# ethz-asl/ethzasl_brisk

Hardware: AMD Instinct MI355X
Metric: frames/sec detect+describe @1080p (1/2/4/8 GPU); % HBM roofline (higher is better)
Workload: dtype u8

## Files before the change

ethzasl_brisk_amd/csrc/brisk_capi.hip:

```cpp
#include <hip/hip_runtime.h>
#include <math.h>
#include <stdio.h>
#include <stdlib.h>
#include <string.h>

#include <sched.h>
#include <unistd.h>

#include <atomic>
#include <chrono>
#include <mutex>
#include <thread>
#include <string>
#include <vector>

#include "../../include/brisk_hip.h"
#include "../../include/brisk_hip_debug.h"
#include "brisk_common.h"
#include "brisk_kernels.h"
#include "brisk_pattern.h"
#include "brisk_device_describe.h"
#include "brisk_hostmem.h"
#include "brisk_slab_layout.h"
#include "brisk_transfer.h"
// ... 264 lines not shown
  HIPCHK(c, w.pyr.grow((size_t)slots * pyr + 256));
  HIPCHK(c, w.smap.grow(((size_t)slots * pyr + 256) * sizeof(uint16_t)));
  HIPCHK(c, w.cand.grow((size_t)slots * c->cand_cap * sizeof(BriskCand)));
  HIPCHK(c, w.blocks.grow((size_t)slots * c->cand_cap * 64));
  HIPCHK(c, w.tie_idx.grow((size_t)slots * BRISK_MAX_LAYERS * c->tie_cap * sizeof(int)));
  HIPCHK(c, w.keys.grow((size_t)slots * c->cand_cap * 2 * sizeof(unsigned)));
  HIPCHK(c, w.counters.grow((size_t)slots * sizeof(BriskFrameCounters)));
  HIPCHK(c, w.kp_out.grow((size_t)slots * c->kp_cap * sizeof(BriskKeyPoint)));
  HIPCHK(c, w.integral.grow((size_t)slots * ifr * sizeof(uint32_t)));
  HIPCHK(c, w.bandsum.grow((size_t)slots * ((ifr / 64) + 4 * 8192 + 64) * sizeof(uint32_t)));
  HIPCHK(c, w.dkp.grow((size_t)slots * c->kp_cap * sizeof(BriskKeyPoint)));
  HIPCHK(c, w.dscale.grow((size_t)slots * c->kp_cap * sizeof(int)));
  HIPCHK(c, w.dperm.grow((size_t)slots * c->kp_cap * sizeof(int)));
  HIPCHK(c, w.drec.grow(((size_t)slots * c->kp_cap + 4) * sizeof(uint4)));
  c->D.dp_work_stride = brisk_dp_work_ints(c->kp_cap);
  HIPCHK(c, w.dp_work.grow((size_t)slots * c->D.dp_work_stride * sizeof(int)));
  c->D.desc_pitch = c->desc_pitch;
  HIPCHK(c, w.desc.grow((size_t)slots * c->kp_cap * c->D.desc_pitch));
  HIPCHK(c, c->d_kp_in.grow((size_t)slots * c->kp_cap * sizeof(BriskKeyPoint)));
  HIPCHK(c, c->d_n_in.grow((size_t)slots * sizeof(int)));
  c->B.pyr = w.pyr.as<uint8_t>(); c->B.smap = w.smap.as<uint16_t>(); c->B.cand = w.cand.as<BriskCand>(); c->B.blocks = w.blocks.as<uint8_t>();
  c->B.tie_idx = w.tie_idx.as<int>(); c->B.keys = w.keys.as<unsigned>(); c->B.counters = w.counters.as<BriskFrameCounters>();
  c->B.kp_out = w.kp_out.as<BriskKeyPoint>(); c->B.bandsum = w.bandsum.as<uint32_t>();
  c->D.integral = w.integral.as<uint32_t>(); c->D.dkp = w.dkp.as<BriskKeyPoint>(); c->D.dscale = w.dscale.as<int>(); c->D.dperm = w.dperm.as<int>();
  c->D.drec = w.drec.as<uint4>(); c->D.dp_work = w.dp_work.as<int>(); c->D.desc = w.desc.as<uint8_t>();
  HIPCHK(c, hipMemset(c->B.pyr, 0, (size_t)slots * pyr + 256));
  HIPCHK(c, hipMemset(c->B.smap, 0, ((size_t)slots * pyr + 256) * sizeof(uint16_t)));
  HIPCHK(c, hipDeviceSynchronize());
  c->dirty_frames = 0;
  c->slots = slots; c->pyr_elems_alloc = pyr; c->iframe_elems_alloc = ifr;
  c->D.istride = istride;
  c->B.istride = istride;
  c->D.iframe_elems = iframe;
  c->D.ibits = 32;
  return BRISK_HIP_OK;
}

static int ensure_stage(brisk_hip_ctx* c, size_t bytes) {
  if (bytes <= c->d_stage.cap) return BRISK_HIP_OK;
  HIPCHK(c, hipStreamSynchronize(c->stream));
  c->img_cache.valid = false;
  HIPCHK(c, c->d_stage.grow(bytes, 256));
  return BRISK_HIP_OK;
}

static void integral_format(const brisk_hip_ctx* ctx, const brisk_hip_pattern* pat, bool batch_with_detect, int* ibits) {
  static const int env = tuning_env("BRISK_INTEGRAL_BITS") ? atoi(tuning_env("BRISK_INTEGRAL_BITS")) : 0;
  *ibits = 32;
  if (!pat || !pat->dev.int24_ok) return;
  if (env == 32 || (dbg_flags(ctx) & (1 << 18))) return;
  if (env == 24 || (dbg_flags(ctx) & (1 << 24))) { *ibits = 24; return; }
  if (ctx->integral_fmt == BRISK_HIP_INTEGRAL_U32) return;
  if (ctx->integral_fmt == BRISK_HIP_INTEGRAL_U24) { *ibits = 24; return; }
  if (!batch_with_detect) return;
  double density = 0.0;
  if (ctx->h_density.p && ctx->density_mpx > 0.0) {
    const long long wv = __atomic_load_n(ctx->h_density.as<long long>(), __ATOMIC_RELAXED);
    const long long frames = wv >> 40, cands = wv & 0xFFFFFFFFFFll;
    if (frames > 0) density = (double)cands / ((double)frames * ctx->density_mpx);
  }
  if (density <= 3000.0) *ibits = 24;
}
static int check_pattern_device(brisk_hip_ctx* ctx, const brisk_hip_pattern* pat) {
  if (pat && pat->device != ctx->device) {
    char msg[160];
    snprintf(msg, sizeof msg, "pattern handle was created on device %d, the context runs on device %d: create one extractor per GPU",
             pat->device, ctx->device);
    return fail(ctx, BRISK_HIP_ERR_ARG, msg);
  }
  return BRISK_HIP_OK;
}

static hipError_t upload_rows(uint8_t* dst, int pitch, const uint8_t* src, int stride, int w, int h, hipStream_t s) {
  if (pitch == w && stride == w) return hipMemcpyAsync(dst, src, (size_t)w * h, hipMemcpyHostToDevice, s);
  return hipMemcpy2DAsync(dst, pitch, src, stride, w, h, hipMemcpyHostToDevice, s);
}

static int check_detect_args(brisk_hip_ctx* ctx, int w, int h, int threshold, int octaves) {
  if (w <= 0 || h <= 0 || w > 8191 || h > 8191) return fail(ctx, BRISK_HIP_ERR_ARG, "image size must be in [1, 8191]");
  if (octaves < 0 || 2 * octaves > BRISK_MAX_LAYERS) return fail(ctx, BRISK_HIP_ERR_ARG, "octaves must be in [0, 8]");
  if (threshold < 1 || threshold > 255)
    return fail(ctx, BRISK_HIP_ERR_THRESHOLD, "AGAST threshold must be in [1, 255]");
  return BRISK_HIP_OK;
}

static int usable_cpus();

extern "C" {

int brisk_hip_device_count(void) {
  int n = 0;
  if (hipGetDeviceCount(&n) != hipSuccess) return 0;
  return n;
}

int brisk_hip_usable_cpus(void) { return usable_cpus(); }

int brisk_hip_host_register(void* ptr, size_t bytes) {
  if (!ptr || !bytes) return BRISK_HIP_ERR_ARG;
  int n = 0;
  if (hipGetDeviceCount(&n) != hipSuccess || n <= 0) return BRISK_HIP_ERR_NO_DEVICE;
  const hipError_t e = hipHostRegister(ptr, bytes, hipHostRegisterDefault);
  if (e == hipSuccess) return BRISK_HIP_OK;
  (void)hipGetLastError();
  return e == hipErrorHostMemoryAlreadyRegistered ? BRISK_HIP_ERR_ARG : BRISK_HIP_ERR_HIP;
}

int brisk_hip_host_unregister(void* ptr) {
  if (!ptr) return BRISK_HIP_ERR_ARG;
  if (hipHostUnregister(ptr) == hipSuccess) return BRISK_HIP_OK;
  (void)hipGetLastError();
  return BRISK_HIP_ERR_ARG;
}

int brisk_hip_create(int device, brisk_hip_ctx** out) {
  if (!out) return BRISK_HIP_ERR_ARG;
  *out = nullptr;
  int n = 0;
  if (hipGetDeviceCount(&n) != hipSuccess || n <= 0 || device < 0 || device >= n) return BRISK_HIP_ERR_NO_DEVICE;
  if (hipSetDevice(device) != hipSuccess) return BRISK_HIP_ERR_NO_DEVICE;
  brisk_hip_ctx* c = new brisk_hip_ctx();
  c->device = device;
  c->B.band_h = 96;
  if (hipStreamCreateWithFlags(&c->stream, hipStreamNonBlocking) != hipSuccess) {
    delete c;
    return BRISK_HIP_ERR_HIP;
  }
  *out = c;
  return BRISK_HIP_OK;
}

void brisk_hip_destroy(brisk_hip_ctx* c) {
  if (!c) return;
  hipSetDevice(c->device);
  hipDeviceSynchronize();
  if (c->done_ev) hipEventDestroy(c->done_ev);
  if (c->block_ev) hipEventDestroy(c->block_ev);
  for (int i = 0; i < 2; ++i) {
    if (c->copied_ev[i]) hipEventDestroy(c->copied_ev[i]);
    if (c->consumed_ev[i]) hipEventDestroy(c->consumed_ev[i]);
    if (c->pin_ev[i]) hipEventDestroy(c->pin_ev[i]);
  }
  if (c->kin_pin_ev) hipEventDestroy(c->kin_pin_ev);
  if (c->copy_stream) hipStreamDestroy(c->copy_stream);
  c->ex.destroy_events();
  c->mx.destroy_events();
  c->tx.destroy_events();
  if (c->egress) hipStreamDestroy(c->egress);
  brisk_prof_destroy(&c->prof);
  if (c->side) { hipStreamDestroy(c->side); hipEventDestroy(c->side_fork); hipEventDestroy(c->side_join); }
  if (c->sub_created) {
    for (int i = 0; i < 8; ++i) { hipStreamDestroy(c->sub[i]); hipEventDestroy(c->join_ev[i]); }
    hipEventDestroy(c->fork_ev);
  }
  hipStreamDestroy(c->stream);
  delete c;
}

const char* brisk_hip_last_error(const brisk_hip_ctx* ctx) { return ctx ? ctx->err.c_str() : "null context"; }

int brisk_hip_set_capacity(brisk_hip_ctx* ctx, int max_candidates, int max_keypoints) {
  if (!ctx) return BRISK_HIP_ERR_ARG;
  if (max_candidates < 256 || max_keypoints < 16) return fail(ctx, BRISK_HIP_ERR_ARG, "capacity too small");
  if (max_keypoints >= (1 << 23)) return fail(ctx, BRISK_HIP_ERR_ARG, "keypoint capacity must be below 2^23");
  std::lock_guard<std::mutex> lk(ctx->mu);
  ctx->cand_cap = max_candidates;
  ctx->kp_cap = max_keypoints;
  ctx->tie_cap = max_candidates / 4 > 1024 ? max_candidates / 4 : 1024;
  return BRISK_HIP_OK;
}

int brisk_hip_reserve(brisk_hip_ctx* ctx, int min_candidates, int min_keypoints) {
  if (!ctx) return BRISK_HIP_ERR_ARG;
  std::lock_guard<std::mutex> lk(ctx->mu);
  if (min_keypoints >= (1 << 23)) return fail(ctx, BRISK_HIP_ERR_ARG, "keypoint capacity must be below 2^23");
  if (min_candidates > ctx->cand_cap) {
    ctx->cand_cap = min_candidates;
    if (min_candidates / 4 > ctx->tie_cap) ctx->tie_cap = min_candidates / 4;
  }
  if (min_keypoints > ctx->kp_cap) ctx->kp_cap = min_keypoints;
  return BRISK_HIP_OK;
}

static int upload_pattern(brisk_hip_ctx* ctx, brisk_hip_pattern* p) {
  const BriskPatternHost& H = p->host;
  const size_t n = (size_t)H.npoints;
  size_t off = 0;
  auto take = [&](size_t bytes) { size_t o = off; off += (bytes + 255) / 256 * 256; return o; };
  const size_t o_mult = take(64 * n * 4), o_sigma = take(64 * n * 4), o_uv = take((size_t)BRISK_NROT * n * 16);
  const size_t o_scl = take(64 * n * 8), o_tab = take(64 * n * 16);
  const size_t o_thr = take(64 * 4), o_size = take(64 * 4), o_sp = take((size_t)H.nshort * 4), o_lp = take((size_t)H.nlong * 16);
  HIPCHK(ctx, hipSetDevice(ctx->device));
  HIPCHK(ctx, hipMalloc(&p->blob, off));
  char* b = (char*)p->blob;
  HIPCHK(ctx, hipMemcpy(b + o_mult, H.mult.data(), 64 * n * 4, hipMemcpyHostToDevice));
  HIPCHK(ctx, hipMemcpy(b + o_sigma, H.sigma.data(), 64 * n * 4, hipMemcpyHostToDevice));
  HIPCHK(ctx, hipMemcpy(b + o_scl, H.scaling.data(), 64 * n * 8, hipMemcpyHostToDevice));
  {
    std::vector<int> tab(64 * n * 4);
    for (size_t i = 0; i < 64 * n; ++i) {
      memcpy(&tab[4 * i], &H.mult[i], 4);
      memcpy(&tab[4 * i + 1], &H.sigma[i], 4);
      brisk_pack_tab(H.scaling[2 * i], H.scaling[2 * i + 1], &tab[4 * i + 2], &tab[4 * i + 3]);
    }
    HIPCHK(ctx, hipMemcpy(b + o_tab, tab.data(), 64 * n * 16, hipMemcpyHostToDevice));
  }
  HIPCHK(ctx, hipMemcpy(b + o_uv, H.uv.data(), (size_t)BRISK_NROT * n * 16, hipMemcpyHostToDevice));
  HIPCHK(ctx, hipMemcpy(b + o_thr, H.size_thresh.data(), 64 * 4, hipMemcpyHostToDevice));
  HIPCHK(ctx, hipMemcpy(b + o_size, H.size_list.data(), 64 * 4, hipMemcpyHostToDevice));
  HIPCHK(ctx, hipMemcpy(b + o_sp, H.short_pairs.data(), (size_t)H.nshort * 4, hipMemcpyHostToDevice));
  HIPCHK(ctx, hipMemcpy(b + o_lp, H.long_pairs.data(), (size_t)H.nlong * 16, hipMemcpyHostToDevice));
  BriskPatternDev& d = p->dev;
  d.npoints = H.npoints; d.nshort = H.nshort; d.nlong = H.nlong; d.strings = H.strings;
  d.rotation_invariant = 1; d.scale_invariant = 1; d.basicscale = H.basicscale;
  d.has_bilinear = 0;
  d.reg_tables = (H.nlong <= 896 && H.nshort <= 512 && H.npoints <= 128) ? 1 : 0;
  for (int i = 0; i < H.nlong; ++i)
    if (H.long_pairs[4 * i + 2] < -32768 || H.long_pairs[4 * i + 2] > 32767 || H.long_pairs[4 * i + 3] < -32768 || H.long_pairs[4 * i + 3] > 32767) d.reg_tables = 0;
  float sigma_max = 0.f;
  for (float sg : H.sigma) { d.has_bilinear |= (sg < 0.5f) ? 1 : 0; sigma_max = sg > sigma_max ? sg : sigma_max; }
  d.int24_ok = (!d.has_bilinear && sigma_max < 120.0f) ? 1 : 0;
  d.mult = (const float*)(b + o_mult); d.sigma = (const float*)(b + o_sigma); d.uv = (const double*)(b + o_uv);
  d.scaling = (const int*)(b + o_scl);
  d.tab = (const int*)(b + o_tab);
  d.size_thresh = (const float*)(b + o_thr); d.size_list = (const int*)(b + o_size);
  d.short_pairs = (const uint16_t*)(b + o_sp); d.long_pairs = (const int*)(b + o_lp);
  return BRISK_HIP_OK;
}

static int pattern_finish(brisk_hip_ctx* ctx, brisk_hip_pattern* p, bool ok, const std::string& err,
                          brisk_hip_pattern** out) {
  if (!ok) {
    ctx->err = err;
    delete p;
    return BRISK_HIP_ERR_PATTERN;
  }
  p->device = p->true_device = ctx->device;
  p->blob = nullptr;
  const int rc = upload_pattern(ctx, p);
  if (rc != BRISK_HIP_OK) {
    if (p->blob) hipFree(p->blob);
    delete p;
    return rc;
  }
  *out = p;
  return BRISK_HIP_OK;
}

int brisk_hip_pattern_create(brisk_hip_ctx* ctx, int version, float pattern_scale, brisk_hip_pattern** out) {
  if (!ctx || !out) return BRISK_HIP_ERR_ARG;
  *out = nullptr;
  std::lock_guard<std::mutex> lk(ctx->mu);
  brisk_hip_pattern* p = new brisk_hip_pattern();
  std::string err;
  const bool ok = brisk_pattern_build_default(version, pattern_scale, &p->host, &err);
  return pattern_finish(ctx, p, ok, err, out);
}

int brisk_hip_pattern_create_from_text(brisk_hip_ctx* ctx, const char* ptn_text, float pattern_scale,
                                       brisk_hip_pattern** out) {
  if (!ctx || !out || !ptn_text) return BRISK_HIP_ERR_ARG;
  *out = nullptr;
  std::lock_guard<std::mutex> lk(ctx->mu);
  brisk_hip_pattern* p = new brisk_hip_pattern();
  std::string err;
  const bool ok = brisk_pattern_build_from_text(ptn_text, pattern_scale, &p->host, &err);
  return pattern_finish(ctx, p, ok, err, out);
}

void brisk_hip_pattern_destroy(brisk_hip_pattern* p) {
  if (!p) return;
  hipSetDevice(p->true_device);
  if (p->blob) hipFree(p->blob);
  delete p;
}

int brisk_hip_pattern_descriptor_size(const brisk_hip_pattern* p) { return p ? p->host.strings : 0; }
int brisk_hip_pattern_points(const brisk_hip_pattern* p) { return p ? p->host.npoints : 0; }

int brisk_hip_pattern_tables(const brisk_hip_pattern* p, float* scale_list, int* size_list, float* size_thresh) {
  if (!p) return BRISK_HIP_ERR_ARG;
  if (scale_list) memcpy(scale_list, p->host.scale_list.data(), 64 * 4);
  if (size_list) memcpy(size_list, p->host.size_list.data(), 64 * 4);
  if (size_thresh) memcpy(size_thresh, p->host.size_thresh.data(), 64 * 4);
  return BRISK_HIP_OK;
}

struct BatchArgs {
  const brisk_hip_pattern* pat;
  int w, h, threshold, octaves;
  long frame_pitch;
  int row_pitch;
  const uint8_t* d_mask;
  long mask_frame_pitch;
  int mask_row_pitch;
  bool do_detect, do_describe;
  double uni_radius;
  int uni_max;
  int bk_u = 0, bk_v = 0, bk_max = 0;
  bool no_scale_nms = false;
  int lower_threshold = BRISK_LOWER_THRESHOLD;
  bool format_as_full_batch = false;
  bool inplace_ok = true;
};

static int ensure_filter_buffers(brisk_hip_ctx* ctx, int w, int h, int nframes, double uni_radius) {
  size_t need = 0;
  if (uni_radius > 0.0) {
    const float scaling = (float)(15.0 / (float)uni_radius);
    const int oh = (int)(h * ceil(scaling) + 32), ow = (int)(w * ceil(scaling) + 32);
    need = (size_t)(((long)oh * ow + 255) / 256 * 256) * nframes + 64;
  }
  const size_t items = (size_t)ctx->slots * ctx->kp_cap;
  if (need > ctx->d_occ.cap || items * sizeof(BriskKeyPoint) > ctx->d_uni_tmp.cap || items * sizeof(int) > ctx->d_uni_order.cap) {
    HIPCHK(ctx, hipDeviceSynchronize());
    HIPCHK(ctx, ctx->d_occ.grow(need));
    HIPCHK(ctx, ctx->d_uni_tmp.grow(items * sizeof(BriskKeyPoint)));
    HIPCHK(ctx, ctx->d_uni_order.grow(items * sizeof(int)));
  }
  return BRISK_HIP_OK;
}

static int batch_begin(brisk_hip_ctx* ctx, const BatchArgs& A, int nframes, hipStream_t s) {
  int rc = check_detect_args(ctx, A.w, A.h, A.threshold, A.octaves);
  if (rc) return rc;
  HIPCHK(ctx, hipSetDevice(ctx->device));
  make_geometry(A.w, A.h, A.threshold, A.octaves, &ctx->G, &ctx->T);
  ctx->G.debug_flags = dbg_flags(ctx);
  ctx->G.no_scale_nms = (A.no_scale_nms && A.octaves != 0) ? 1 : 0;
  ctx->G.lower_threshold = A.lower_threshold;
  if (A.do_describe && A.pat && A.pat->host.strings > ctx->desc_pitch) ctx->desc_pitch = brisk_align_up(A.pat->host.strings, 16);
  rc = ensure_buffers(ctx, nframes, ctx->G);
  if (rc) return rc;
  integral_format(ctx, A.pat, A.format_as_full_batch || (A.do_detect && A.do_describe), &ctx->D.ibits);
  const bool bucketing = A.do_detect && !(A.uni_radius > 0.0) && A.bk_u > 0;
  if ((A.do_detect && A.uni_radius > 0.0) || bucketing) {
    rc = ensure_filter_buffers(ctx, A.w, A.h, nframes, bucketing ? 0.0 : A.uni_radius);
    if (rc) return rc;
  }
  if (bucketing && (A.bk_u >= A.w || A.bk_v >= A.h))
    return fail(ctx, BRISK_HIP_ERR_ARG, "bucketing: more buckets than pixels (key-point-bucketing-inl.h:82-83)");
  rc = workspace_acquire(ctx, s);
  if (rc) return fail(ctx, rc, "hipStreamWaitEvent failed");
  ctx->img_cache.valid = false;
  brisk_prof_begin_call(&ctx->prof);
  if (A.do_detect) {
    if (ctx->dirty_frames > 0) brisk_launch_smap_clear(ctx->dirtyG, ctx->B, ctx->dirty_frames, s);
    ctx->dirtyG = ctx->G;
    ctx->dirty_frames = nframes;
  }
  return BRISK_HIP_OK;
}

static int batch_slice(brisk_hip_ctx* ctx, const BatchArgs& A, const uint8_t* d_frames, long f0, int nf, hipStream_t si,
                       BriskProfiler* prof, bool overlap_integral) {
  const int nbands = (A.h + ctx->B.band_h - 1) / ctx->B.band_h;
  BriskDetectBuffers Bi = ctx->B;
  Bi.pyr += f0 * ctx->G.pyr_elems;
  Bi.smap += f0 * ctx->G.pyr_elems;
  Bi.cand += f0 * Bi.cand_cap;
  Bi.blocks += f0 * Bi.cand_cap * 64;
  Bi.tie_idx += f0 * BRISK_MAX_LAYERS * Bi.tie_cap;
  Bi.keys += f0 * Bi.cand_cap * 2;
  Bi.counters += f0;
  Bi.kp_out += f0 * Bi.kp_cap;
  Bi.bandsum += f0 * nbands * Bi.istride;
  BriskDescribeBuffers Di = ctx->D;
  Di.ibits = ctx->D.ibits;
  Di.integral += f0 * Di.iframe_elems;
  Di.dkp += f0 * Bi.kp_cap;
  Di.dscale += f0 * Bi.kp_cap;
  Di.dperm += f0 * Bi.kp_cap;
  Di.drec += f0 * Bi.kp_cap;
  Di.dp_work += f0 * Di.dp_work_stride;
  Di.desc += f0 * Bi.kp_cap * Di.desc_pitch;
  BriskOverlap ov{};
  const BriskOverlap* ovp = nullptr;
  if (A.do_detect && A.do_describe && overlap_integral && ctx->overlap && !(dbg_flags(ctx) & 0x10000)) {
    if (!ctx->side) {
      int least = 0, greatest = 0;
      HIPCHK(ctx, hipDeviceGetStreamPriorityRange(&least, &greatest));
      const char* pe = tuning_env("BRISK_SIDE_PRIO");
      HIPCHK(ctx, hipStreamCreateWithPriority(&ctx->side, hipStreamNonBlocking, (pe && atoi(pe) == 0) ? 0 : least));
      HIPCHK(ctx, hipEventCreateWithFlags(&ctx->side_fork, hipEventDisableTiming));
      HIPCHK(ctx, hipEventCreateWithFlags(&ctx->side_join, hipEventDisableTiming));
    }
    ov.side = ctx->side; ov.fork = ctx->side_fork; ov.join = ctx->side_join; ov.Dd = &Di;
    ovp = &ov;
  }
  BriskGeom Gs = ctx->G;
  {
    static const bool inplace_on = !(tuning_env("BRISK_L0_INPLACE") && atoi(tuning_env("BRISK_L0_INPLACE")) == 0);
    const bool ordered = Gs.threshold < BRISK_FAST_PATH_MIN_THRESHOLD || Gs.no_scale_nms || Gs.lower_threshold != BRISK_LOWER_THRESHOLD;
    if (A.do_detect && A.inplace_ok && inplace_on && !ordered && A.row_pitch == Gs.L[0].stride && A.w == Gs.L[0].stride &&
        ((((uintptr_t)d_frames) | (uintptr_t)A.frame_pitch) & 15) == 0) {
      Gs.l0_ext = d_frames;
      Gs.l0_pitch = A.frame_pitch;
      if (f0 == 0) { ctx->last_l0_ext = d_frames; ctx->last_l0_pitch = A.frame_pitch; }
    } else if (f0 == 0) {
      ctx->last_l0_ext = nullptr;
    }
  }
  if (A.do_detect) {
    brisk_launch_detect(Gs, ctx->T, Bi, nf, d_frames, A.frame_pitch, A.row_pitch,
                        A.d_mask ? A.d_mask + f0 * A.mask_frame_pitch : nullptr, A.mask_frame_pitch, A.mask_row_pitch, si, prof, ovp);
  }
  int* const uni_order = ctx->d_uni_order.as<int>();
  BriskKeyPoint* const uni_tmp = ctx->d_uni_tmp.as<BriskKeyPoint>();
  if (A.do_detect && A.uni_radius > 0.0) {
    const float scaling = (float)(15.0 / (float)A.uni_radius);
    const int oh = (int)(A.h * ceil(scaling) + 32), ow = (int)(A.w * ceil(scaling) + 32);
    const long occ_frame = ((long)oh * ow + 255) / 256 * 256;
    brisk_launch_uniformity(Bi.kp_out, Bi.counters, uni_order + f0 * Bi.kp_cap, uni_tmp + f0 * Bi.kp_cap,
                            ctx->d_occ.as<uint8_t>() + f0 * occ_frame, occ_frame, ow, Bi.kp_cap, scaling, A.uni_max, nf, si);
  }
  if (A.do_detect && !(A.uni_radius > 0.0) && A.bk_u > 0) {
    brisk_launch_bucketing(Bi.kp_out, Bi.counters, uni_order + f0 * Bi.kp_cap, uni_tmp + f0 * Bi.kp_cap, Bi.kp_cap,
                           A.h, A.w, A.bk_u, A.bk_v, A.bk_max, nf, si);
  }
  if (A.do_detect) brisk_prof_mark(prof, BRISK_STG_INTEGRAL, si);
  if (A.do_describe) {
    BriskPatternDev P = A.pat->dev;
    brisk_launch_describe(Gs, P, Bi, Di, nf, Bi.kp_out, &Bi.counters[0].nkp, sizeof(BriskFrameCounters), si, prof, ovp);
  }
  return BRISK_HIP_OK;
}

static int batch_end(brisk_hip_ctx* ctx, const BatchArgs& A, int nframes, hipStream_t s) {
  if (A.do_detect && A.do_describe) {
    if (!ctx->h_density.p) {
      HIPCHK(ctx, ctx->h_density.grow(sizeof(long long), 0, hipHostMallocMapped));
      *ctx->h_density.as<long long>() = 0;
    }
    ctx->density_mpx = (double)A.w * (double)A.h / 1e6;
    brisk_launch_batch_density(ctx->B.counters, nframes, ctx->B.cand_cap, ctx->h_density.as<long long>(), s);
  }
  if (ctx->prof.on) ctx->prof.calls++;
  HIPCHK(ctx, hipGetLastError());
  ctx->last_nframes = nframes;
  ctx->last_has_desc = A.do_describe;
  ctx->last_desc_pitch = ctx->D.desc_pitch;
  if (A.do_describe && A.pat) ctx->last_strings = A.pat->host.strings;
  const int rc = workspace_release(ctx, s);
  if (rc) return fail(ctx, rc, "hipEventRecord failed");
  return BRISK_HIP_OK;
}

static int run_batch(brisk_hip_ctx* ctx, const brisk_hip_pattern* pat, const uint8_t* d_frames, int nframes, int w, int h,
                     long frame_pitch, int row_pitch, int threshold, int octaves, const uint8_t* d_mask,
                     long mask_frame_pitch, int mask_row_pitch, hipStream_t s, bool do_detect, bool do_describe,
                     double uni_radius = -1.0, int uni_max = 0, bool no_scale_nms = false,
                     int lower_threshold = BRISK_LOWER_THRESHOLD, const int* bucketing = nullptr) {
  if (!d_frames || nframes <= 0 || row_pitch < w || frame_pitch < (long)row_pitch * (h - 1) + w)
    return fail(ctx, BRISK_HIP_ERR_ARG, "bad frame buffer description");
  if (int rcp = check_pattern_device(ctx, pat)) return rcp;
  const bool full_batch = do_detect && do_describe;
  if (do_detect && do_describe && (dbg_flags(ctx) & (1 << 27)) && ctx->last_nframes >= nframes) do_detect = false;
  BatchArgs A{pat, w, h, threshold, octaves, frame_pitch, row_pitch, d_mask, mask_frame_pitch, mask_row_pitch, do_detect,
              do_describe, uni_radius < 0.0 ? ctx->uni_radius : uni_radius, uni_radius < 0.0 ? ctx->uni_max : uni_max};
  A.no_scale_nms = no_scale_nms;
  A.lower_threshold = lower_threshold;
  A.format_as_full_batch = full_batch;
  if (bucketing) { A.bk_u = bucketing[0]; A.bk_v = bucketing[1]; A.bk_max = bucketing[2]; }
  else if (uni_radius < 0.0) { A.bk_u = ctx->bk_u; A.bk_v = ctx->bk_v; A.bk_max = ctx->bk_max; }
  int rc = batch_begin(ctx, A, nframes, s);
  if (rc) return rc;
  WorkspaceGuard guard(ctx, s);
  int nsub = ctx->nsub;
  if (nsub > 8) nsub = 8;
  if (nframes < 16 * nsub) nsub = nframes >= 32 ? 2 : 1;
  if (nsub > 1 && !ctx->sub_created) {
    for (int i = 0; i < 8; ++i) {
      HIPCHK(ctx, hipStreamCreateWithFlags(&ctx->sub[i], hipStreamNonBlocking));
      HIPCHK(ctx, hipEventCreateWithFlags(&ctx->join_ev[i], hipEventDisableTiming));
    }
    HIPCHK(ctx, hipEventCreateWithFlags(&ctx->fork_ev, hipEventDisableTiming));
    ctx->sub_created = true;
  }
  const int grp = 8 * ((dbg_flags(ctx) >> 20) & 0xF);
  if (grp > 0 && !do_detect && do_describe) {
    if (dbg_flags(ctx) & (1 << 19))
      brisk_launch_integral(ctx->G, ctx->B.pyr, ctx->B.bandsum, ctx->D.integral, ctx->D.istride, ctx->D.iframe_elems, ctx->B.band_h, nframes, s);
    for (long f0 = 0; f0 < nframes; f0 += grp) {
      const int nf = (int)((nframes - f0) < grp ? (nframes - f0) : grp);
      if (f0 == 0) ctx->last_frames_per_launch = nf;
      rc = batch_slice(ctx, A, d_frames + f0 * frame_pitch, f0, nf, s, (f0 == 0) ? &ctx->prof : nullptr, false);
      if (rc) return rc;
    }
    guard.armed = false;
    return batch_end(ctx, A, nframes, s);
  }
  if (nsub > 1) HIPCHK(ctx, hipEventRecord(ctx->fork_ev, s));
  for (int i = 0; i < nsub; ++i) {
    const long f0 = (long)nframes * i / nsub, f1 = (long)nframes * (i + 1) / nsub;
    const int nf = (int)(f1 - f0);
    if (nf <= 0) continue;
    hipStream_t si = s;
    if (nsub > 1) {
      si = ctx->sub[i];
      HIPCHK(ctx, hipStreamWaitEvent(si, ctx->fork_ev, 0));
    }
    if (i == 0) ctx->last_frames_per_launch = nf;
    rc = batch_slice(ctx, A, d_frames + f0 * frame_pitch, f0, nf, si, (i == 0) ? &ctx->prof : nullptr, nsub == 1);
    if (rc) return rc;
    if (nsub > 1) {
      HIPCHK(ctx, hipEventRecord(ctx->join_ev[i], si));
      HIPCHK(ctx, hipStreamWaitEvent(s, ctx->join_ev[i], 0));
    }
  }
  guard.armed = false;
  return batch_end(ctx, A, nframes, s);
}

static int host_slice_frames() {
  static const int v = [] { const char* e = tuning_env("BRISK_HOST_SLICE"); const int n = e ? atoi(e) : 0; return n > 0 ? n : 64; }();
  return v;
}

#define BRISK_STAGED_SLICE 32
static int copy_threads() {
  static const int n = [] {
    const char* e = tuning_env("BRISK_COPY_THREADS");
    int t = e ? atoi(e) : usable_cpus() / 2;
    return t < 1 ? 1 : (t > 8 ? 8 : t);
  }();
  return n;
}
static int upload_frames(brisk_hip_ctx* ctx, uint8_t* d_dst, size_t dframe, int dpitch, const uint8_t* const* ptrs, int nf, int w, int h, int stride,
                         bool staged, int b, hipStream_t cs) {
  if (!staged) {
    for (int f = 0; f < nf; ++f)
      HIPCHK(ctx, hipMemcpy2DAsync(d_dst + (size_t)f * dframe, dpitch, ptrs[f], stride, w, h, hipMemcpyHostToDevice, cs));
    return BRISK_HIP_OK;
  }
  if (ctx->h_pin[0].cap < dframe * BRISK_STAGED_SLICE || ctx->h_pin[1].cap < dframe * BRISK_STAGED_SLICE) {
    for (int i = 0; i < 2; ++i) {
      if (ctx->pin_used[i]) HIPCHK(ctx, hipEventSynchronize(ctx->pin_ev[i]));
      ctx->pin_used[i] = false;
      ctx->h_pin[i].reset();
    }
    for (int i = 0; i < 2; ++i) {
      HIPCHK(ctx, ctx->h_pin[i].grow(dframe * BRISK_STAGED_SLICE, 256));
      if (!ctx->pin_ev[i]) HIPCHK(ctx, hipEventCreateWithFlags(&ctx->pin_ev[i], hipEventDisableTiming));
    }
  }
  if (ctx->pin_used[b]) HIPCHK(ctx, hipEventSynchronize(ctx->pin_ev[b]));
  uint8_t* const pin = ctx->h_pin[b].as<uint8_t>();
  std::atomic<int> next{0};
  const int items = nf * 4;
  auto work = [&]() {
    for (;;) {
      const int i = next.fetch_add(1, std::memory_order_relaxed);
      if (i >= items) break;
      const int f = i >> 2, part = i & 3;
      const int y0 = (int)((long)h * part / 4), y1 = (int)((long)h * (part + 1) / 4);
      if (y1 <= y0) continue;
      uint8_t* d = pin + (size_t)f * dframe;
      const uint8_t* sp = ptrs[f];
      if (stride == dpitch) memcpy(d + (size_t)y0 * dpitch, sp + (size_t)y0 * stride, (size_t)(y1 - y0 - 1) * dpitch + (size_t)w);
      else for (int y = y0; y < y1; ++y) memcpy(d + (size_t)y * dpitch, sp + (size_t)y * stride, (size_t)w);
    }
  };
  const int T = copy_threads() < items ? copy_threads() : items;
  std::vector<std::thread> helpers;
  for (int t = 1; t < T; ++t) helpers.emplace_back(work);
  work();
  for (std::thread& t : helpers) t.join();
  HIPCHK(ctx, hipMemcpyAsync(d_dst, pin, dframe * (size_t)nf, hipMemcpyHostToDevice, cs));
  HIPCHK(ctx, hipEventRecord(ctx->pin_ev[b], cs));
  ctx->pin_used[b] = true;
  return BRISK_HIP_OK;
}
static bool is_pageable(const void* p) {
  void* dev = nullptr;
  return !device_can_write(p, &dev);
}

static int batch_host_locked(brisk_hip_ctx* ctx, const brisk_hip_pattern* pat, const uint8_t* h_frames, int nframes, int w, int h,
                             long frame_pitch, int row_pitch, int threshold, int octaves, const uint8_t* const* frame_ptrs = nullptr,
                             uint8_t* d_resident = nullptr ) {
  if ((!h_frames && !frame_ptrs) || nframes <= 0 || row_pitch < w || (!frame_ptrs && frame_pitch < (long)row_pitch * (h - 1) + w))
    return fail(ctx, BRISK_HIP_ERR_ARG, "bad frame buffer description");
  if (frame_ptrs)
    for (int f = 0; f < nframes; ++f)
      if (!frame_ptrs[f]) return fail(ctx, BRISK_HIP_ERR_ARG, "null image in the list");
  if (int rcp = check_pattern_device(ctx, pat)) return rcp;
  BatchArgs A{pat, w, h, threshold, octaves, 0, 0, nullptr, 0, 0, true, pat != nullptr, ctx->uni_radius, ctx->uni_max};
  A.bk_u = ctx->bk_u; A.bk_v = ctx->bk_v; A.bk_max = ctx->bk_max;
  A.inplace_ok = d_resident != nullptr;
  hipStream_t s = ctx->stream;
  int rc = batch_begin(ctx, A, nframes, s);
  if (rc) return rc;
  WorkspaceGuard guard(ctx, s);
  const bool staged = frame_ptrs && is_pageable(frame_ptrs[0]);
  const int slice_max = staged ? BRISK_STAGED_SLICE : host_slice_frames();
  const int slice = slice_max < nframes ? slice_max : nframes;
  const int dpitch = brisk_align_up(w, 64);
  const size_t dframe = (size_t)dpitch * h;
  bool fresh = false;
  if (!ctx->copy_stream) {
    HIPCHK(ctx, hipStreamCreateWithFlags(&ctx->copy_stream, hipStreamNonBlocking));
    for (int i = 0; i < 2; ++i) {
      HIPCHK(ctx, hipEventCreateWithFlags(&ctx->copied_ev[i], hipEventDisableTiming));
      HIPCHK(ctx, hipEventCreateWithFlags(&ctx->consumed_ev[i], hipEventDisableTiming));
    }
    fresh = true;
  }
  if (!d_resident && (ctx->d_hstage[0].cap < dframe * slice || ctx->d_hstage[1].cap < dframe * slice)) {
    HIPCHK(ctx, hipDeviceSynchronize());
    for (int i = 0; i < 2; ++i) ctx->d_hstage[i].reset();
    for (int i = 0; i < 2; ++i) HIPCHK(ctx, ctx->d_hstage[i].grow(dframe * slice, 256));
    fresh = true;
  }
  A.frame_pitch = (long)dframe;
  A.row_pitch = dpitch;
  if (fresh) {
    HIPCHK(ctx, hipEventRecord(ctx->consumed_ev[0], s));
    HIPCHK(ctx, hipEventRecord(ctx->consumed_ev[1], s));
  }
  int k = 0;
  for (long f0 = 0; f0 < nframes; f0 += slice, ++k) {
    const int nf = (int)((nframes - f0 < slice) ? nframes - f0 : slice);
    const int b = k & 1;
    uint8_t* const dslice = d_resident ? d_resident + (size_t)f0 * dframe : ctx->d_hstage[b].as<uint8_t>();
    if (!d_resident) HIPCHK(ctx, hipStreamWaitEvent(ctx->copy_stream, ctx->consumed_ev[b], 0));
    else if (k == 0 && ctx->done_valid && !ensure_done_event(ctx)) HIPCHK(ctx, hipStreamWaitEvent(ctx->copy_stream, ctx->done_ev, 0));
    const uint8_t* src = frame_ptrs ? nullptr : h_frames + f0 * frame_pitch;
    if (frame_ptrs) {
      rc = upload_frames(ctx, dslice, dframe, dpitch, frame_ptrs + f0, nf, w, h, row_pitch, staged, b, ctx->copy_stream);
      if (rc) return rc;
    } else if (frame_pitch == (long)row_pitch * h) {
      HIPCHK(ctx, hipMemcpy2DAsync(dslice, dpitch, src, row_pitch, w, (size_t)h * nf, hipMemcpyHostToDevice,
                                   ctx->copy_stream));
    } else {
      for (int f = 0; f < nf; ++f)
        HIPCHK(ctx, hipMemcpy2DAsync(dslice + (size_t)f * dframe, dpitch, src + (long)f * frame_pitch, row_pitch, w,
                                     h, hipMemcpyHostToDevice, ctx->copy_stream));
    }
    HIPCHK(ctx, hipEventRecord(ctx->copied_ev[b], ctx->copy_stream));
    HIPCHK(ctx, hipStreamWaitEvent(s, ctx->copied_ev[b], 0));
    if (k == 0) ctx->last_frames_per_launch = nf;
    rc = batch_slice(ctx, A, dslice, f0, nf, s, (k == 0) ? &ctx->prof : nullptr, true);
    if (rc) return rc;
    if (!d_resident) HIPCHK(ctx, hipEventRecord(ctx->consumed_ev[b], s));
  }
  guard.armed = false;
  return batch_end(ctx, A, nframes, s);
}

int brisk_hip_detect_describe_batch_host(brisk_hip_ctx* ctx, const brisk_hip_pattern* pat, const uint8_t* h_frames,
                                         int nframes, int w, int h, long frame_pitch, int row_pitch, int threshold,
                                         int octaves) {
  if (!ctx || !pat) return BRISK_HIP_ERR_ARG;
  std::lock_guard<std::mutex> lk(ctx->mu);
  return batch_host_locked(ctx, pat, h_frames, nframes, w, h, frame_pitch, row_pitch, threshold, octaves);
}

int brisk_hip_detect_describe_batch(brisk_hip_ctx* ctx, const brisk_hip_pattern* pat, const uint8_t* d_frames, int nframes,
                                    int w, int h, long frame_pitch, int row_pitch, int threshold, int octaves,
                                    void* stream) {
  if (!ctx || !pat) return BRISK_HIP_ERR_ARG;
  std::lock_guard<std::mutex> lk(ctx->mu);
  hipStream_t s = stream ? (hipStream_t)stream : ctx->stream;
  return run_batch(ctx, pat, d_frames, nframes, w, h, frame_pitch, row_pitch, threshold, octaves, nullptr, 0, 0, s, true,
                   true);
}

int brisk_hip_detect_batch(brisk_hip_ctx* ctx, const uint8_t* d_frames, int nframes, int w, int h, long frame_pitch,
                           int row_pitch, int threshold, int octaves, void* stream) {
  if (!ctx) return BRISK_HIP_ERR_ARG;
  std::lock_guard<std::mutex> lk(ctx->mu);
  hipStream_t s = stream ? (hipStream_t)stream : ctx->stream;
  return run_batch(ctx, nullptr, d_frames, nframes, w, h, frame_pitch, row_pitch, threshold, octaves, nullptr, 0, 0, s, true,
                   false);
}

int brisk_hip_batch_results(brisk_hip_ctx* ctx, const int** d_detected, const int** d_described, int* count_stride,
                            const brisk_hip_keypoint** d_detected_kps, const brisk_hip_keypoint** d_described_kps,
                            const uint8_t** d_desc, int* kp_cap, int* desc_pitch) {
  if (!ctx) return BRISK_HIP_ERR_ARG;
  std::lock_guard<std::mutex> lk(ctx->mu);
  if (!ctx->B.counters) return fail(ctx, BRISK_HIP_ERR_ARG, "no batch has run");
  if (d_detected) *d_detected = &ctx->B.counters[0].nkp;
  if (d_described) *d_described = &ctx->B.counters[0].ndesc;
  if (count_stride) *count_stride = (int)sizeof(BriskFrameCounters);
  if (d_detected_kps) *d_detected_kps = (const brisk_hip_keypoint*)ctx->B.kp_out;
  if (d_described_kps) *d_described_kps = (const brisk_hip_keypoint*)ctx->D.dkp;
  if (d_desc) *d_desc = ctx->D.desc;
  if (kp_cap) *kp_cap = ctx->B.kp_cap;
  if (desc_pitch) *desc_pitch = ctx->last_desc_pitch ? ctx->last_desc_pitch : ctx->D.desc_pitch;
  return BRISK_HIP_OK;
}

static int overflow_to_rc(brisk_hip_ctx* ctx, int flags) {
  if (flags & 1) return fail(ctx, BRISK_HIP_ERR_CAPACITY, "candidate capacity exceeded (brisk_hip_set_capacity)");
  if (flags & 2) return fail(ctx, BRISK_HIP_ERR_CAPACITY, "tie-candidate capacity exceeded (brisk_hip_set_capacity)");
  if (flags & 4) return fail(ctx, BRISK_HIP_ERR_CAPACITY, "keypoint capacity exceeded (brisk_hip_set_capacity)");
  if (flags & 8) {
    static const char* const site[8] = {"", " (the layer below)", " (a pending tie outside its chunk)", " (a neighbour's decision)",
                                        " (the writer wave)", " (the sorted tie list of the layer below)", "", ""};
    char msg[128];
    snprintf(msg, sizeof(msg), "tie resolution gave up waiting for a decision%s (internal error)", site[(flags >> 8) & 7]);
    return fail(ctx, BRISK_HIP_ERR_HIP, msg);
  }
  if (flags & 16)
    return fail(ctx, BRISK_HIP_ERR_UNSUPPORTED,
                "no defined result in the reference on this input: suppressScaleNonmaxima=false indexes layer 0's point list "
                "past its end or reads outside a score matrix (brisk-scale-space.cc:137), or ComputeScale addresses the maps of "
                "a point in a layer's last rows beyond the image (brisk-layer.cc:110-115)");
  return BRISK_HIP_OK;
}

int brisk_hip_batch_status(brisk_hip_ctx* ctx, int nframes, int* overflow_flags) {
  if (!ctx) return BRISK_HIP_ERR_ARG;
  std::lock_guard<std::mutex> lk(ctx->mu);
  if (nframes <= 0 || nframes > ctx->slots) return fail(ctx, BRISK_HIP_ERR_ARG, "bad frame count");
  HIPCHK(ctx, hipSetDevice(ctx->device));
  HIPCHK(ctx, wait_own_work(ctx));
  std::vector<BriskFrameCounters> c(nframes);
  HIPCHK(ctx, hipMemcpy(c.data(), ctx->B.counters, sizeof(BriskFrameCounters) * nframes, hipMemcpyDeviceToHost));
  int f = 0;
  for (auto& x : c) f |= x.overflow;
  if (overflow_flags) *overflow_flags = f;
  return overflow_to_rc(ctx, f);
}

static int download_locked(brisk_hip_ctx* ctx, int frame, int which, brisk_hip_keypoint* kps, int cap, int* n,
                           uint8_t* desc, int desc_stride, int strings, int dev_pitch = 0) {
  if (!dev_pitch) dev_pitch = ctx->D.desc_pitch;
  if (frame < 0 || frame >= ctx->slots) return fail(ctx, BRISK_HIP_ERR_ARG, "bad frame index");
  HIPCHK(ctx, wait_own_work(ctx));
  BriskFrameCounters c;
  HIPCHK(ctx, hipMemcpy(&c, ctx->B.counters + frame, sizeof(c), hipMemcpyDeviceToHost));
  int rc = overflow_to_rc(ctx, c.overflow);
  if (rc) return rc;
  const int cnt = which ? c.ndesc : c.nkp;
  if (n) *n = cnt;
  if (kps) {
    if (cnt > cap) return fail(ctx, BRISK_HIP_ERR_CAPACITY, "output keypoint buffer too small");
    const BriskKeyPoint* src = (which ? ctx->D.dkp : ctx->B.kp_out) + (size_t)frame * ctx->B.kp_cap;
    if (cnt) HIPCHK(ctx, hipMemcpy(kps, src, sizeof(BriskKeyPoint) * (size_t)cnt, hipMemcpyDeviceToHost));
  }
  if (desc && which && cnt) {
    if (cnt > cap) return fail(ctx, BRISK_HIP_ERR_CAPACITY, "output descriptor buffer too small");
    const uint8_t* src = ctx->D.desc + (size_t)frame * ctx->B.kp_cap * ctx->D.desc_pitch;
    if (dev_pitch == desc_stride && strings == desc_stride)
      HIPCHK(ctx, hipMemcpy(desc, src, (size_t)cnt * strings, hipMemcpyDeviceToHost));
    else
      HIPCHK(ctx, hipMemcpy2D(desc, desc_stride, src, dev_pitch, strings, cnt, hipMemcpyDeviceToHost));
  }
  return BRISK_HIP_OK;
}

static int usable_cpus() {
  static const int n = [] {
    int c = 0;
    cpu_set_t set;
    if (sched_getaffinity(0, sizeof set, &set) == 0) c = CPU_COUNT(&set);
    if (c <= 0) c = (int)sysconf(_SC_NPROCESSORS_ONLN);
    long quota = -1, period = -1;
    if (FILE* f = fopen("/sys/fs/cgroup/cpu.max", "r")) {
      char q[64];
      if (fscanf(f, "%63s %ld", q, &period) == 2 && strcmp(q, "max") != 0) quota = atol(q);
      fclose(f);
    } else {
      if (FILE* g = fopen("/sys/fs/cgroup/cpu/cpu.cfs_quota_us", "r")) { if (fscanf(g, "%ld", &quota) != 1) quota = -1; fclose(g); }
      if (FILE* g = fopen("/sys/fs/cgroup/cpu/cpu.cfs_period_us", "r")) { if (fscanf(g, "%ld", &period) != 1) period = -1; fclose(g); }
    }
    if (quota > 0 && period > 0) {
      const int lim = (int)((quota + period - 1) / period);
      if (lim > 0 && lim < c) c = lim;
    }
    return c > 0 ? c : 1;
// ... 1858 lines not shown
```

ethzasl_brisk_amd/csrc/brisk_describe.hip:

```cpp
#include <hip/hip_runtime.h>
#include <stdlib.h>

#include "brisk_common.h"
#include "brisk_device_describe.h"
#include "brisk_kernels.h"

#define DP_MAXSORT 2048
#ifndef DP_THREADS
#define DP_THREADS 1024
#endif
#define DP_SMALL_N 2048
#define DP_SB DP_THREADS
#define DP_MAXBUCKETS 4096
#define DP_W_HIST 16
#define DP_W_BLK (DP_W_HIST + DP_MAXBUCKETS + 16)
__device__ __forceinline__ unsigned dp_order_key(int x, int y, int sc, int j, int mode) {
  const unsigned low = (unsigned)(j & 0x7FF);
  if (mode == 1) {
    unsigned tx = (unsigned)x >> 6, ty = (unsigned)y >> 6, d = 0;
    for (unsigned s = 64; s > 0; s >>= 1) {
      const unsigned rx = (tx & s) ? 1u : 0u, ry = (ty & s) ? 1u : 0u;
      d += s * s * ((3u * rx) ^ ry);
      if (ry == 0) {
        if (rx == 1) { tx = 127u - tx; ty = 127u - ty; }
        const unsigned t = tx; tx = ty; ty = t;
      }
    }
    return (d << 18) | (((unsigned)x & 63u) << 12) | low;
  }
  if (mode == 2) return ((unsigned)(y >> 7) << 24) | (((unsigned)x & 0x1FFFu) << 11) | low;
  if (mode == 3) return ((unsigned)(y >> 5) << 24) | (((unsigned)x & 0x1FFFu) << 11) | low;
  if (mode == 4) return ((unsigned)(sc >> 4) << 30) | (((unsigned)(y >> 6) & 0x7Fu) << 23) | ((((unsigned)x >> 1) & 0xFFFu) << 11) | low;
  return ((unsigned)(y >> 6) << 24) | (((unsigned)x & 0x1FFFu) << 11) | low;
}

__global__ void __launch_bounds__(DP_THREADS) k_desc_prepare(BriskGeom G, BriskPatternDev P, const BriskKeyPoint* kp_in,
                                                       const int* n_in_ptr, long n_in_stride, BriskFrameCounters* counters,
                                                       BriskKeyPoint* dkp, int* dscale, int* dperm, uint4* drec, int kp_cap,
                                                       int* work, long work_stride) {
  __shared__ int wtot[DP_THREADS / 64];
  __shared__ int base, nest;
  __shared__ __attribute__((aligned(16))) unsigned pkey[DP_MAXSORT + 4];
  BRISK_CHAIN_SETPRIO();
  const int frame = blockIdx.x, tid = threadIdx.x, wave = tid >> 6, lane = tid & 63;
  const int n = min(*(const int*)((const char*)n_in_ptr + (long)frame * n_in_stride), kp_cap);
  const BriskKeyPoint* K = kp_in + (long)frame * kp_cap;
  if (n > DP_SMALL_N) {
    int* wk = work + (long)frame * work_stride;
    for (int q = tid; q < DP_W_BLK; q += DP_THREADS) wk[q] = 0;
    return;
  }
  __shared__ uint4 srec[DP_SMALL_N];
  __shared__ int sborder[BRISK_SCALES];
  __shared__ float sthr[BRISK_SCALES];
  if (tid == 0) { base = 0; nest = 0; }
  if (tid < BRISK_SCALES) { sborder[tid] = P.size_list[tid]; sthr[tid] = P.size_thresh[tid]; }
  __syncthreads();
  for (int i0 = 0; i0 < n; i0 += DP_THREADS) {
    const int i = i0 + tid;
    bool keep = false;
    int sc = 0;
    BriskKeyPoint kp;
    if (i < n) {
      kp = K[i];
      if (!P.scale_invariant) sc = P.basicscale;
      else {
#pragma unroll 8
        for (int q = 1; q < BRISK_SCALES; ++q) sc += (kp.size >= sthr[q]) ? 1 : 0;
      }
      const int border = sborder[sc];
      keep = !((kp.x < (float)border) || (kp.x >= (float)(G.L[0].w - border)) || (kp.y < (float)border) || (kp.y >= (float)(G.L[0].h - border)));
    }
    const unsigned long long bal = __ballot(keep);
    const int before = __popcll(bal & ((1ull << lane) - 1ull));
    if (lane == 0) wtot[wave] = __popcll(bal);
    const unsigned long long bal_e = __ballot(keep && kp.angle == -1.0f);
    if (lane == 0 && bal_e) atomicAdd(&nest, __popcll(bal_e));
    __syncthreads();
    int wbase = 0, total = 0;
#pragma unroll
    for (int k = 0; k < DP_THREADS / 64; ++k) {
      const int t = wtot[k];
      wbase += (k < wave) ? t : 0;
      total += t;
    }
    if (keep) {
      const int j = base + wbase + before;
      dkp[(long)frame * kp_cap + j] = kp;
      if (j < DP_MAXSORT) pkey[j] = dp_order_key((int)kp.x, (int)kp.y, sc, j, (BRISK_DBG_FLAGS(G) >> 4) & 0xF);
      srec[j] = make_uint4(__float_as_uint(kp.x), __float_as_uint(kp.y), __float_as_uint(kp.angle), (unsigned)sc | ((unsigned)j << 8));
    }
    __syncthreads();
    if (tid == 0) base += total;
    __syncthreads();
  }
  if (tid == 0) { counters[frame].ndesc = base; counters[frame].nestimate = nest; counters[frame].desc_ticket = 0; counters[frame].orient_ticket = 0; }
  const int m = base;
  if (tid < 4) pkey[m + tid] = 0xFFFFFFFFu;
  __syncthreads();
  if (((BRISK_DBG_FLAGS(G) >> 4) & 0xF) != 0) {
    for (int j = tid; j < m; j += DP_THREADS) {
      const unsigned kj = pkey[j];
      int r = 0;
      for (int q = 0; q < m; q += 4) {
        const uint4 kk = *reinterpret_cast<const uint4*>(&pkey[q]);
        r += (kk.x < kj ? 1 : 0) + (kk.y < kj ? 1 : 0) + (kk.z < kj ? 1 : 0) + (kk.w < kj ? 1 : 0);
      }
      drec[(long)frame * kp_cap + r] = srec[j];
    }
    return;
  }
  {
    __shared__ int bhead[DP_SB], bstart[DP_SB];
    __shared__ int bnext[DP_SMALL_N];
    const int nbands = ((G.L[0].h - 1) >> 6) + 1;
    int xs = 6;
    while (nbands * (((G.L[0].w - 1) >> xs) + 1) > DP_SB) ++xs;
    const int nbx = ((G.L[0].w - 1) >> xs) + 1;
    auto bucket_of = [&](unsigned key) { return (int)(key >> 24) * nbx + (int)(((key >> 11) & 0x1FFFu) >> xs); };
    for (int b = tid; b < DP_SB; b += DP_THREADS) { bhead[b] = -1; bstart[b] = 0; }
    __syncthreads();
    for (int j = tid; j < m; j += DP_THREADS) {
      const int b = bucket_of(pkey[j]);
      atomicAdd(&bstart[b], 1);
      bnext[j] = atomicExch(&bhead[b], j);
    }
    __syncthreads();
    {
      static_assert(DP_SB == DP_THREADS, "one bucket per thread");
      const int v = bstart[tid];
      int incl = v;
#pragma unroll
      for (int off = 1; off < 64; off <<= 1) {
        const int t = __shfl_up(incl, off, 64);
        if (lane >= off) incl += t;
      }
      __syncthreads();
      if (lane == 63) wtot[wave] = incl;
      __syncthreads();
      int woff = 0;
#pragma unroll
      for (int k = 0; k < DP_THREADS / 64; ++k) woff += (k < wave) ? wtot[k] : 0;
      bstart[tid] = woff + incl - v;
    }
    __syncthreads();
    for (int j = tid; j < m; j += DP_THREADS) {
      const unsigned kj = pkey[j];
      const int b = bucket_of(kj);
      int r = bstart[b];
      for (int q = bhead[b]; q >= 0; q = bnext[q]) r += (pkey[q] < kj) ? 1 : 0;
      drec[(long)frame * kp_cap + r] = srec[j];
    }
  }
}

struct DpTiles { int shift, tiles_x, w, h; };
__device__ __forceinline__ int dp_bucket(const DpTiles& T, float x, float y) {
  const int xi = min(max((int)x, 0), T.w - 1), yi = min(max((int)y, 0), T.h - 1);
  return (yi >> T.shift) * T.tiles_x + (xi >> T.shift);
}
struct DpItem { bool keep; int sc; BriskKeyPoint kp; };
__device__ __forceinline__ DpItem dp_item(const BriskGeom& G, const BriskPatternDev& P, const BriskKeyPoint* K, int i, int n) {
  DpItem it;
  it.keep = false; it.sc = 0;
  if (i < n) {
    it.kp = K[i];
    it.sc = brisk_scale_index(P, it.kp.size);
    it.keep = brisk_inside_border(P, it.sc, it.kp.x, it.kp.y, G.L[0].w, G.L[0].h);
  }
  return it;
}

__global__ void __launch_bounds__(DP_THREADS) k_dp_count(BriskGeom G, BriskPatternDev P, DpTiles T, const BriskKeyPoint* kp_in,
                                                          const int* n_in_ptr, long n_in_stride, int kp_cap, int* work, long work_stride) {
  __shared__ int wtot[DP_THREADS / 64];
  const int frame = blockIdx.y, tid = threadIdx.x, wave = tid >> 6, lane = tid & 63;
  const int n = min(*(const int*)((const char*)n_in_ptr + (long)frame * n_in_stride), kp_cap);
  if (n <= DP_SMALL_N) return;
  int* wk = work + (long)frame * work_stride;
  for (int blk = blockIdx.x; blk * DP_THREADS < n; blk += gridDim.x) {
    const DpItem it = dp_item(G, P, kp_in + (long)frame * kp_cap, blk * DP_THREADS + tid, n);
    const unsigned long long bal = __ballot(it.keep);
    if (lane == 0) wtot[wave] = __popcll(bal);
    const unsigned long long bal_e = __ballot(it.keep && it.kp.angle == -1.0f);
    if (lane == 0 && bal_e) atomicAdd(&wk[0], __popcll(bal_e));
    if (it.keep) atomicAdd(&wk[DP_W_HIST + dp_bucket(T, it.kp.x, it.kp.y)], 1);
    __syncthreads();
    if (tid == 0) {
      int t = 0;
#pragma unroll
      for (int k = 0; k < DP_THREADS / 64; ++k) t += wtot[k];
      wk[DP_W_BLK + blk] = t;
    }
    __syncthreads();
  }
}

__device__ __forceinline__ int dp_scan_inplace(int* v, int n, int* sh) {
  const int tid = threadIdx.x, wave = tid >> 6, lane = tid & 63;
  int carry = 0;
  for (int i0 = 0; i0 < n; i0 += DP_THREADS) {
    const int i = i0 + tid;
    const int x = i < n ? v[i] : 0;
    int incl = x;
#pragma unroll
    for (int off = 1; off < 64; off <<= 1) {
      const int t = __shfl_up(incl, off, 64);
      if (lane >= off) incl += t;
    }
    if (lane == 63) sh[wave] = incl;
    __syncthreads();
    int woff = 0, tot = 0;
#pragma unroll
    for (int k = 0; k < DP_THREADS / 64; ++k) { const int t = sh[k]; woff += (k < wave) ? t : 0; tot += t; }
    if (i < n) v[i] = carry + woff + incl - x;
    carry += tot;
    __syncthreads();
  }
  return carry;
}

__global__ void __launch_bounds__(DP_THREADS) k_dp_scan(const int* n_in_ptr, long n_in_stride, int kp_cap, int nbuckets,
                                                         BriskFrameCounters* counters, int* work, long work_stride) {
  __shared__ int sh[DP_THREADS / 64 + 1];
  const int frame = blockIdx.x;
  const int n = min(*(const int*)((const char*)n_in_ptr + (long)frame * n_in_stride), kp_cap);
  if (n <= DP_SMALL_N) return;
  int* wk = work + (long)frame * work_stride;
  const int m = dp_scan_inplace(wk + DP_W_BLK, (n + DP_THREADS - 1) / DP_THREADS, sh);
  (void)dp_scan_inplace(wk + DP_W_HIST, nbuckets, sh);
  if (threadIdx.x == 0) {
    counters[frame].ndesc = m; counters[frame].nestimate = wk[0]; counters[frame].desc_ticket = 0; counters[frame].orient_ticket = 0;
  }
}

__global__ void __launch_bounds__(DP_THREADS) k_dp_scatter(BriskGeom G, BriskPatternDev P, DpTiles T, const BriskKeyPoint* kp_in,
                                                            const int* n_in_ptr, long n_in_stride, int kp_cap, int* work,
                                                            long work_stride, BriskKeyPoint* dkp, uint4* drec) {
  __shared__ int wtot[DP_THREADS / 64];
  const int frame = blockIdx.y, tid = threadIdx.x, wave = tid >> 6, lane = tid & 63;
  const int n = min(*(const int*)((const char*)n_in_ptr + (long)frame * n_in_stride), kp_cap);
  if (n <= DP_SMALL_N) return;
  int* wk = work + (long)frame * work_stride;
  for (int blk = blockIdx.x; blk * DP_THREADS < n; blk += gridDim.x) {
    const DpItem it = dp_item(G, P, kp_in + (long)frame * kp_cap, blk * DP_THREADS + tid, n);
    const unsigned long long bal = __ballot(it.keep);
    if (lane == 0) wtot[wave] = __popcll(bal);
    __syncthreads();
    if (it.keep) {
      int j = wk[DP_W_BLK + blk] + __popcll(bal & ((1ull << lane) - 1ull));
#pragma unroll
      for (int k = 0; k < DP_THREADS / 64; ++k) j += (k < wave) ? wtot[k] : 0;
      dkp[(long)frame * kp_cap + j] = it.kp;
      const int pos = atomicAdd(&wk[DP_W_HIST + dp_bucket(T, it.kp.x, it.kp.y)], 1);
      drec[(long)frame * kp_cap + pos] = make_uint4(__float_as_uint(it.kp.x), __float_as_uint(it.kp.y), __float_as_uint(it.kp.angle),
                                                    (unsigned)it.sc | ((unsigned)j << 8));
    }
    __syncthreads();
  }
}

#ifndef DS_WAVES
#define DS_WAVES 2
#endif
#define DS_MAXRUN 8
#define DS_MAXQ 256
#ifndef DS_BLOCKS_PER_CU
#define DS_BLOCKS_PER_CU 3
#endif
#define DS_LP_LDS 1024
#define DS_REG_LONG 14
#define DS_REG_SHORT 8
#define DS_GETREG_XCC_ID (20 | (3 << 11))

typedef uint32_t __attribute__((ext_vector_type(2))) ds_u32x2;

__device__ __forceinline__ int ds_wave_sum(int v) {
  v += __builtin_amdgcn_update_dpp(0, v, 0x111, 0xf, 0xf, false);
  v += __builtin_amdgcn_update_dpp(0, v, 0x112, 0xf, 0xf, false);
  v += __builtin_amdgcn_update_dpp(0, v, 0x114, 0xf, 0xf, false);
  v += __builtin_amdgcn_update_dpp(0, v, 0x118, 0xf, 0xf, false);
  v += __builtin_amdgcn_update_dpp(0, v, 0x142, 0xa, 0xf, false);
  v += __builtin_amdgcn_update_dpp(0, v, 0x143, 0xc, 0xf, false);
  return __builtin_amdgcn_readlane(v, 63);
}

struct DsLane {
  float kx, ky;
  int4 tab;
  int ti;
  double2 uv;
  int slot;
};
typedef BriskBoxPrep DsPrep;
typedef uint32_t __attribute__((ext_vector_type(3))) ds_u32x3;
struct DsRaw {
  ds_u32x2 p00, p02, p10, p12, p30, p32, ql, qr;
  ds_u32x3 p20, p22;
  unsigned br, bl;
};
__device__ __forceinline__ DsPrep ds_prep(float xf, float yf, float sigma_half, int tab_z, int tab_w) {
  return brisk_box_prep(xf, yf, sigma_half, tab_z, tab_w);
}
template <bool I24>
__device__ __forceinline__ void ds_load(DsRaw& r, const DsPrep& p, __amdgpu_buffer_rsrc_t rs_img, int stride, int cols,
                                        __amdgpu_buffer_rsrc_t rs_int, int istride) {
  constexpr int ES = I24 ? 3 : 4;
  const int rowb = istride * ES;
  const int o_t = p.y_top * rowb, o_b = p.y_bottom * rowb;
  const int o_tl = o_t + p.x_left * ES, o_tr = o_t + p.x_right * ES, o_bl = o_b + p.x_left * ES, o_br = o_b + p.x_right * ES;
  r.p00 = __builtin_amdgcn_raw_buffer_load_b64(rs_int, o_tl, 0, 0);
  r.p02 = __builtin_amdgcn_raw_buffer_load_b64(rs_int, o_tr, 0, 0);
  r.p10 = __builtin_amdgcn_raw_buffer_load_b64(rs_int, o_tl, rowb, 0);
  r.p12 = __builtin_amdgcn_raw_buffer_load_b64(rs_int, o_tr, rowb, 0);
  r.ql = __builtin_amdgcn_raw_buffer_load_b64(rs_int, o_bl - rowb + ES, 0, 0);
  r.qr = __builtin_amdgcn_raw_buffer_load_b64(rs_int, o_br - rowb + ES, 0, 0);
  r.p20 = __builtin_amdgcn_raw_buffer_load_b96(rs_int, o_bl, 0, 0);
  r.p22 = __builtin_amdgcn_raw_buffer_load_b96(rs_int, o_br, 0, 0);
  r.p30 = __builtin_amdgcn_raw_buffer_load_b64(rs_int, o_bl, rowb, 0);
  r.p32 = __builtin_amdgcn_raw_buffer_load_b64(rs_int, o_br, rowb, 0);
  r.br = 0; r.bl = 0;
  const bool wrap = p.quirk && (p.x_right + 1 >= cols || p.x_left + 1 >= cols);
  if (__builtin_expect(wrap, 0)) {
    const int qy = max(p.y_bottom - 1, 0), xr = p.x_right + 1, xl = p.x_left + 1, o_q = qy * stride, wr = stride - cols;
    r.br = __builtin_amdgcn_raw_buffer_load_b8(rs_img, o_q + xr + (xr >= cols ? wr : 0), 0, 0);
    r.bl = __builtin_amdgcn_raw_buffer_load_b8(rs_img, o_q + xl + (xl >= cols ? wr : 0), 0, 0);
    r.br |= 0x100u; r.bl |= 0x100u;
  }
}
__device__ __forceinline__ void ds_unpack2(ds_u32x2 v, uint32_t& a, uint32_t& b) {
  a = v.x;
  b = __builtin_amdgcn_alignbit(v.y, v.x, 24);
}
template <bool I24>
__device__ __forceinline__ int ds_combine(const DsPrep& p, const DsRaw& r) {
  uint32_t i00, i01, i02, i03, i10, i11, i12, i13, i20, i21, i2x, i22, i23, i2y, i30, i31, i32, i33, ql0, ql1, qr0, qr1;
  if (I24) {
    ds_unpack2(r.p00, i00, i01); ds_unpack2(r.p02, i02, i03); ds_unpack2(r.p10, i10, i11); ds_unpack2(r.p12, i12, i13);
    ds_unpack2(ds_u32x2{r.p20.x, r.p20.y}, i20, i21); i2x = __builtin_amdgcn_alignbit(r.p20.z, r.p20.y, 16);
    ds_unpack2(ds_u32x2{r.p22.x, r.p22.y}, i22, i23); i2y = __builtin_amdgcn_alignbit(r.p22.z, r.p22.y, 16);
    ds_unpack2(r.p30, i30, i31); ds_unpack2(r.p32, i32, i33); ds_unpack2(r.ql, ql0, ql1); ds_unpack2(r.qr, qr0, qr1);
  } else {
    i00 = r.p00.x; i01 = r.p00.y; i02 = r.p02.x; i03 = r.p02.y; i10 = r.p10.x; i11 = r.p10.y; i12 = r.p12.x; i13 = r.p12.y;
    i20 = r.p20.x; i21 = r.p20.y; i2x = r.p20.z; i22 = r.p22.x; i23 = r.p22.y; i2y = r.p22.z;
    i30 = r.p30.x; i31 = r.p30.y; i32 = r.p32.x; i33 = r.p32.y; ql0 = r.ql.x; ql1 = r.ql.y; qr0 = r.qr.x; qr1 = r.qr.y;
  }
  constexpr uint32_t mask = I24 ? 0xFFFFFFu : 0xFFFFFFFFu;
  unsigned qbr = (i2y - i23 - qr1 + qr0) & mask;
  unsigned qbl = (i2x - i21 - ql1 + ql0) & mask;
  if (r.br & 0x100u) { qbr = r.br & 0xFFu; qbl = r.bl & 0xFFu; }
  const uint32_t acc = brisk_box_acc(p, i00, i01, i02, i03, i10, i11, i12, i13, i20, i21, i22, i23, i30, i31, i32, i33, qbr, qbl, mask);
  if (__any(p.shift < 0)) return brisk_box_divide(p, acc);
  return brisk_div_by_magic((int)acc, p.magic, p.shift);
}
__device__ __forceinline__ int ds_dpp_even(int v) { return __builtin_amdgcn_update_dpp(0, v, 0xA0, 0xf, 0xf, false); }
__device__ __forceinline__ int ds_dpp_odd(int v) { return __builtin_amdgcn_update_dpp(0, v, 0xF5, 0xf, 0xf, false); }
__device__ __forceinline__ int ds_dpp_partner(int v) { return __builtin_amdgcn_update_dpp(0, v, 0xB1, 0xf, 0xf, false); }
struct DsRawPair {
  ds_u32x2 at0, at1, aq, ab1, bt0, bt1, bq, bb1;
  ds_u32x3 ab0, bb0;
  unsigned br, bl;
  bool a_quirk, b_quirk;
};
template <bool I24>
__device__ __forceinline__ void ds_load_pair(DsRawPair& r, const DsPrep& p, bool odd, bool pair_valid, bool valid, __amdgpu_buffer_rsrc_t rs_img,
                                             int stride, int cols, __amdgpu_buffer_rsrc_t rs_int, int istride) {
  constexpr int ES = I24 ? 3 : 4;
  const int rowb = istride * ES;
  const int o_t = p.y_top * rowb, o_b = p.y_bottom * rowb;
  const int o_tl = o_t + p.x_left * ES, o_tr = o_t + p.x_right * ES, o_bl = o_b + p.x_left * ES, o_br = o_b + p.x_right * ES;
  const int e_tr = ds_dpp_even(o_tr), o_tl_ = ds_dpp_odd(o_tl), e_br = ds_dpp_even(o_br), o_bl_ = ds_dpp_odd(o_bl);
  const int qk = p.quirk ? 1 : 0;
  const int e_qk = ds_dpp_even(qk), o_qk = ds_dpp_odd(qk);
  r.a_quirk = e_qk != 0; r.b_quirk = o_qk != 0;
  const int a_top = odd ? e_tr : o_tl, b_top = odd ? o_tr : o_tl_;
  const int a_bot = odd ? e_br : o_bl, b_bot = odd ? o_br : o_bl_;
  if (pair_valid) {
    r.at0 = __builtin_amdgcn_raw_buffer_load_b64(rs_int, a_top, 0, 0);
    r.bt0 = __builtin_amdgcn_raw_buffer_load_b64(rs_int, b_top, 0, 0);
    r.at1 = __builtin_amdgcn_raw_buffer_load_b64(rs_int, a_top, rowb, 0);
    r.bt1 = __builtin_amdgcn_raw_buffer_load_b64(rs_int, b_top, rowb, 0);
    r.aq = __builtin_amdgcn_raw_buffer_load_b64(rs_int, a_bot - rowb + ES, 0, 0);
    r.bq = __builtin_amdgcn_raw_buffer_load_b64(rs_int, b_bot - rowb + ES, 0, 0);
    r.ab0 = __builtin_amdgcn_raw_buffer_load_b96(rs_int, a_bot, 0, 0);
    r.bb0 = __builtin_amdgcn_raw_buffer_load_b96(rs_int, b_bot, 0, 0);
    r.ab1 = __builtin_amdgcn_raw_buffer_load_b64(rs_int, a_bot, rowb, 0);
    r.bb1 = __builtin_amdgcn_raw_buffer_load_b64(rs_int, b_bot, rowb, 0);
  }
  r.br = 0; r.bl = 0;
  const bool wrap = valid && p.quirk && (p.x_right + 1 >= cols || p.x_left + 1 >= cols);
  if (__builtin_expect(wrap, 0)) {
    const int qy = max(p.y_bottom - 1, 0), xr = p.x_right + 1, xl = p.x_left + 1, o_q = qy * stride, wr = stride - cols;
    r.br = __builtin_amdgcn_raw_buffer_load_b8(rs_img, o_q + xr + (xr >= cols ? wr : 0), 0, 0);
    r.bl = __builtin_amdgcn_raw_buffer_load_b8(rs_img, o_q + xl + (xl >= cols ? wr : 0), 0, 0);
    r.br |= 0x100u; r.bl |= 0x100u;
  }
}
template <bool I24>
__device__ __forceinline__ BriskBoxSide ds_side(ds_u32x2 t0, ds_u32x2 t1, ds_u32x2 q, ds_u32x3 b0, ds_u32x2 b1, bool quirk, bool right) {
  uint32_t t0x, t0y, t1x, t1y, qx, qy, b0x, b0y, b0z, b1x, b1y;
  if (I24) {
    ds_unpack2(t0, t0x, t0y); ds_unpack2(t1, t1x, t1y); ds_unpack2(q, qx, qy); ds_unpack2(ds_u32x2{b0.x, b0.y}, b0x, b0y); ds_unpack2(b1, b1x, b1y);
    b0z = __builtin_amdgcn_alignbit(b0.z, b0.y, 16);
  } else {
    t0x = t0.x; t0y = t0.y; t1x = t1.x; t1y = t1.y; qx = q.x; qy = q.y; b0x = b0.x; b0y = b0.y; b0z = b0.z; b1x = b1.x; b1y = b1.y;
  }
  return brisk_box_side(t0x, t0y, t1x, t1y, qx, qy, b0x, b0y, b0z, b1x, b1y, quirk, right, I24 ? 0xFFFFFFu : 0xFFFFFFFFu);
}
template <bool I24>
__device__ __forceinline__ int ds_combine_pair(const DsPrep& p, const DsRawPair& r, bool odd) {
  constexpr uint32_t mask = I24 ? 0xFFFFFFu : 0xFFFFFFFFu;
  const BriskBoxSide sa = ds_side<I24>(r.at0, r.at1, r.aq, r.ab0, r.ab1, r.a_quirk, odd);
  const BriskBoxSide sb = ds_side<I24>(r.bt0, r.bt1, r.bq, r.bb0, r.bb1, r.b_quirk, odd);
  BriskBoxSide own, par;
#define DS_X(f) own.f = odd ? sb.f : sa.f; par.f = (uint32_t)ds_dpp_partner((int)(odd ? sa.f : sb.f));
  DS_X(ct) DS_X(cb) DS_X(st) DS_X(dt) DS_X(db) DS_X(dm)
#undef DS_X
  if (r.br & 0x100u) {
    const unsigned pbl = r.bl & 0xFFu, pbr = r.br & 0xFFu;
    own.cb = odd ? pbr : pbl;
    par.cb = odd ? pbl : pbr;
  }
  const uint32_t acc = brisk_box_acc_pair(p, own, par, odd, mask);
  if (__any(p.shift < 0)) return brisk_box_divide(p, acc);
  return brisk_div_by_magic((int)acc, p.magic, p.shift);
}
struct DsFrame {
  const uint8_t* img;
  const uint32_t* integ;
  __amdgpu_buffer_rsrc_t rs_img, rs_int;
};
struct DsSide {
  int t;
  uint4 rec;
};
struct DsTicket {
  int frame, k0, cnt, total;
  bool ok;
};

template <int RUN, bool GENERIC, bool REGTAB, bool I24>
__global__ void __launch_bounds__(DS_WAVES * 64) k_describe(BriskGeom G, BriskPatternDev P, const uint8_t* __restrict__ pyr,
                                                            const uint32_t* __restrict__ integral, int istride,
                                                            long iframe_elems, BriskFrameCounters* counters,
                                                            BriskKeyPoint* dkp, uint4* __restrict__ drec,
                                                            uint8_t* desc, int kp_cap, int desc_pitch, int nframes, int run_fixed) {
  extern __shared__ __attribute__((aligned(16))) unsigned char ds_lds[];
  const int np = P.npoints;
  const bool lp_in_lds = !REGTAB && P.nlong <= DS_LP_LDS;
  int4* lp_s = reinterpret_cast<int4*>(ds_lds);
  unsigned* sp_s = reinterpret_cast<unsigned*>(lp_s + (lp_in_lds ? P.nlong : 0));
  const int wave = threadIdx.x >> 6, lane = threadIdx.x & 63;
  const int table_bytes = REGTAB ? 0 : ((lp_in_lds ? P.nlong * 16 : 0) + ((P.nshort * 4 + 15) & ~15));
  const int vals_bytes = (RUN * np * 4 + 15) & ~15;
  const int per_wave = 2 * RUN * 16 + ((RUN * 4 + 15) & ~15) + vals_bytes + 2 * DS_MAXQ * 4;
  unsigned char* wbase = ds_lds + table_bytes + wave * per_wave;
  uint4* krec2 = reinterpret_cast<uint4*>(wbase);
  int* kth = reinterpret_cast<int*>(wbase + 2 * RUN * 16);
  int* vals = reinterpret_cast<int*>(wbase + 2 * RUN * 16 + ((RUN * 4 + 15) & ~15));
  int* cum = reinterpret_cast<int*>(reinterpret_cast<unsigned char*>(vals) + vals_bytes);
  int* cnt_q = cum + DS_MAXQ;
  unsigned lp_ij[DS_REG_LONG], lp_w[DS_REG_LONG], sp_ij[DS_REG_SHORT];
  if (REGTAB) {
#pragma unroll
    for (int t = 0; t < DS_REG_LONG; ++t) {
      const int p = t * 64 + lane;
      lp_ij[t] = 0; lp_w[t] = 0;
      if (p < P.nlong) {
        const int4 q = reinterpret_cast<const int4*>(P.long_pairs)[p];
        lp_ij[t] = (unsigned)q.x | ((unsigned)q.y << 8);
        lp_w[t] = ((unsigned)q.z & 0xFFFFu) | ((unsigned)q.w << 16);
      }
    }
#pragma unroll
    for (int t = 0; t < DS_REG_SHORT; ++t) {
      const int p = t * 64 + lane;
      sp_ij[t] = 0xFFFFFFFFu;
      if (p < P.nshort) sp_ij[t] = (unsigned)P.short_pairs[2 * p] | ((unsigned)P.short_pairs[2 * p + 1] << 16);
    }
  } else {
    if (lp_in_lds)
      for (int p = threadIdx.x; p < P.nlong; p += DS_WAVES * 64) lp_s[p] = reinterpret_cast<const int4*>(P.long_pairs)[p];
    for (int p = threadIdx.x; p < P.nshort; p += DS_WAVES * 64) sp_s[p] = (unsigned)P.short_pairs[2 * p] | ((unsigned)P.short_pairs[2 * p + 1] << 16);
    __syncthreads();
  }

  const int xcc = (int)(__builtin_amdgcn_s_getreg(DS_GETREG_XCC_ID) & 7);
#ifdef DS_TIMING
  unsigned dt_acc[6] = {0, 0, 0, 0, 0, 0};
  unsigned long long dt_last = 0;
#define DS_T0() do { dt_last = __builtin_amdgcn_s_memtime(); asm volatile("s_waitcnt lgkmcnt(0)" ::: "memory"); } while (0)
#define DS_T(i) do { const unsigned long long t_ = __builtin_amdgcn_s_memtime(); asm volatile("s_waitcnt lgkmcnt(0)" ::: "memory"); dt_acc[i] += (unsigned)(t_ - dt_last); dt_last = t_; } while (0)
#else
#define DS_T0() do { } while (0)
#define DS_T(i) do { } while (0)
#endif
  const int stride = G.L[0].stride, cols = G.L[0].w;
  const int img_bytes = (G.L[0].h - 1) * stride + cols;
  const unsigned inv20 = (1u << 20) / (unsigned)np + 1u;
  const int nwords = P.strings / 8;
  const int4* tab4 = reinterpret_cast<const int4*>(P.tab);
  const double2* uv2 = reinterpret_cast<const double2*>(P.uv);

  auto wave_sync = [&]() {
    __builtin_amdgcn_fence(__ATOMIC_RELEASE, "wavefront");
    __builtin_amdgcn_wave_barrier();
    __builtin_amdgcn_fence(__ATOMIC_ACQUIRE, "wavefront");
  };
  auto fetch = [&](const uint4* krec, int total, int s, bool rotated) {
    DsLane L;
    const int sc = min(s, total - 1);
    const int kq = (int)(((unsigned)sc * inv20) >> 20);
    const int pt = sc - kq * np;
    const uint4 rec = krec[kq];
    const int theta = rotated ? kth[kq] : 0;
    L.kx = __uint_as_float(rec.x); L.ky = __uint_as_float(rec.y);
    L.ti = (int)(rec.w & 0xFF) * np + pt;
    L.tab = tab4[L.ti];
    L.uv = uv2[theta * np + pt];
    L.slot = sc;
    return L;
  };
  auto pass = [&](const DsFrame& F, const uint4* krec, int total, bool rotated, bool use_first, DsLane first, bool side,
                  auto&& take_fn, const uint4* nsrc, int ncnt) {
    DsSide out;
    out.t = 0; out.rec = make_uint4(0, 0, 0, 0);
    DsLane Lc = first;
    if (!use_first) Lc = fetch(krec, total, lane, rotated);
    for (int s0 = 0; s0 < total; s0 += 64) {
      const bool valid = s0 + lane < total;
      DsLane Ln = Lc;
      if (s0 + 64 < total) Ln = fetch(krec, total, s0 + 64 + lane, rotated);
      const double mm = (double)__int_as_float(Lc.tab.x);
      const float sigma = __int_as_float(Lc.tab.y);
      const float xf = (float)(mm * Lc.uv.x) + Lc.kx, yf = (float)(mm * Lc.uv.y) + Lc.ky;
      int value;
      if (GENERIC) {
        BriskSamplePoint sp;
        sp.x = (float)(mm * Lc.uv.x); sp.y = (float)(mm * Lc.uv.y); sp.sigma = sigma;
        sp.scaling = P.scaling[2 * Lc.ti]; sp.scaling2 = P.scaling[2 * Lc.ti + 1];
        value = valid ? brisk_smoothed_intensity(F.img, stride, cols, F.integ, istride, Lc.kx, Lc.ky, sp) : 0;
      } else {
        const DsPrep pr = ds_prep(xf, yf, sigma, Lc.tab.z, Lc.tab.w);
        if (side && s0 == 0) {
          out.t = take_fn();
          if (lane < ncnt) out.rec = nsrc[lane];
        }
#ifdef DS_NO_PAIRS
        constexpr bool pairs = false;
#else
        constexpr bool pairs = I24;
#endif
        if (!pairs) {
          DsRaw raw;
          __builtin_amdgcn_s_setprio(1);
          if (valid) ds_load<I24>(raw, pr, F.rs_img, stride, cols, F.rs_int, istride);
          __builtin_amdgcn_s_setprio(0);
          value = ds_combine<I24>(pr, raw);
        } else {
          DsRawPair raw;
          const bool odd = lane & 1;
          __builtin_amdgcn_s_setprio(1);
          ds_load_pair<I24>(raw, pr, odd, s0 + (lane & ~1) < total, valid, F.rs_img, stride, cols, F.rs_int, istride);
          __builtin_amdgcn_s_setprio(0);
          value = ds_combine_pair<I24>(pr, raw, odd);
        }
      }
      if (valid) vals[Lc.slot] = value;
      Lc = Ln;
    }
    if (GENERIC && side) {
      out.t = take_fn();
      if (lane < ncnt) out.rec = nsrc[lane];
    }
    wave_sync();
    return out;
  };
  auto frame_of = [&](int frame) {
    DsFrame F;
    F.img = brisk_layer_img(G, pyr, frame, 0);
    F.integ = integral + (long)frame * iframe_elems;
    F.rs_img = __builtin_amdgcn_make_buffer_rsrc(const_cast<uint8_t*>(F.img), 0, (BRISK_DBG_FLAGS(G) & (1 << 30)) ? 0 : img_bytes, 0x00020000);
    F.rs_int = __builtin_amdgcn_make_buffer_rsrc(const_cast<uint32_t*>(F.integ), 0, (BRISK_DBG_FLAGS(G) & (1 << 29)) ? 0 : (int)(iframe_elems * 4), 0x00020000);
    return F;
  };

  const int ngroups = nframes < 8 ? 1 : (nframes <= 8 * DS_MAXQ ? 8 : (nframes + DS_MAXQ - 1) / DS_MAXQ);
  for (int gi = 0; gi < ngroups; ++gi) {
    const int g = (xcc + gi) % ngroups;
    if (g >= nframes) continue;
    const int m = (nframes - 1 - g) / ngroups + 1;
    __builtin_amdgcn_wave_barrier();
    int carry = 0;
    for (int j0 = 0; j0 < m; j0 += 64) {
      const int j = j0 + lane;
      const int nkp = j < m ? counters[g + (m - 1 - j) * ngroups].ndesc : 0;
      int runf = run_fixed;
      if (runf == 0) {
        const long density = (long)nkp * (1 << 20) / ((long)cols * G.L[0].h);
        runf = density < 1500 ? 3 : density < 6000 ? 4 : 8;
        const int waves_serving = (int)(gridDim.x * DS_WAVES) / ngroups;
        runf = min(runf, max(1, nkp / max(waves_serving, 1)));
      }
      runf = min(max(runf, 1), RUN);
      int r = (nkp + runf - 1) / runf;
      for (int off = 1; off < 64; off <<= 1) {
        const int t = __shfl_up(r, off, 64);
        if (lane >= off) r += t;
      }
      if (j < m) { cum[j] = carry + r; cnt_q[j] = nkp | (runf << 24); }
      carry += __shfl(r, 63, 64);
    }
    wave_sync();
    const int total_runs = __builtin_amdgcn_readfirstlane(carry);
    int* ticket = &counters[g].desc_ticket;
    int qj = 0;
    auto decode = [&](int tk) {
      DsTicket T;
      T.ok = tk < total_runs;
      T.frame = 0; T.k0 = 0; T.cnt = 0; T.total = 0;
      if (T.ok) {
        while (tk >= cum[qj]) ++qj;
        qj = __builtin_amdgcn_readfirstlane(qj);
        T.frame = g + (m - 1 - qj) * ngroups;
        const int run = __builtin_amdgcn_readfirstlane(tk - (qj ? cum[qj - 1] : 0));
        const int cq = __builtin_amdgcn_readfirstlane(cnt_q[qj]);
        const int runf = cq >> 24;
        T.k0 = run * runf;
        T.cnt = min(runf, (cq & 0xFFFFFF) - T.k0);
        T.total = T.cnt * np;
      }
      return T;
    };
    const bool static_deal = ngroups == 1;
    int static_next = (int)(blockIdx.x * DS_WAVES + wave);
    typedef __attribute__((address_space(1))) int* ds_gptr;
    ds_gptr ticket_opaque = (ds_gptr)ticket;
    asm volatile("" : "+v"(ticket_opaque));
    auto take = [&]() {
      int t = total_runs;
      if (static_deal) {
        t = min(static_next, total_runs);
        static_next += (int)(gridDim.x * DS_WAVES);
      } else if (lane == 0) {
        t = __hip_atomic_fetch_add(ticket_opaque, 1, __ATOMIC_RELAXED, __HIP_MEMORY_SCOPE_AGENT);
      }
      return t;
    };
    if (gi > 0 && __builtin_amdgcn_readfirstlane(__hip_atomic_load(ticket, __ATOMIC_RELAXED, __HIP_MEMORY_SCOPE_AGENT)) >= total_runs) continue;
    const int t1 = take();
    const int t2 = take();
    DsTicket cur = decode(__builtin_amdgcn_readfirstlane(t1));
    DsTicket nxt = decode(__builtin_amdgcn_readfirstlane(t2));
    int kb = 0;
    uint4 myrec = make_uint4(0, 0, 0, 0);
    if (lane < cur.cnt) myrec = (drec + (long)cur.frame * kp_cap)[cur.k0 + lane];
    if (lane < cur.cnt) krec2[lane] = myrec;
    bool have_first = false;
    DsLane first;
    first.kx = 0.f; first.ky = 0.f; first.tab = make_int4(0, 0, 0, 0); first.ti = 0; first.uv = make_double2(0., 0.); first.slot = 0;
    DS_T0();
    while (cur.ok) {
      uint4* krec = krec2 + kb * RUN;
      const uint4* nsrc = drec + (long)nxt.frame * kp_cap + nxt.k0;
      const DsFrame F = frame_of(cur.frame);
      const bool estimate = P.rotation_invariant && lane < cur.cnt && __uint_as_float(myrec.z) == -1.0f;
      int theta = 0;
      DsSide side;
      side.t = 0; side.rec = make_uint4(0, 0, 0, 0);
      const bool two_passes = __any(estimate);
      DS_T(0);
      if (two_passes) {
        wave_sync();
        side = pass(F, krec, cur.total, false, have_first, first, true, take, nsrc, nxt.cnt);
        DS_T(1);
        int md0 = 0, md1 = 0;
        for (int kq = 0; kq < cur.cnt; ++kq) {
          const int* v = vals + kq * np;
          int d0 = 0, d1 = 0;
          if (REGTAB) {
            int va[DS_REG_LONG], vb[DS_REG_LONG];
#pragma unroll
            for (int t = 0; t < DS_REG_LONG; ++t) { va[t] = v[lp_ij[t] & 0xFF]; vb[t] = v[(lp_ij[t] >> 8) & 0xFF]; }
#pragma unroll
            for (int t = 0; t < DS_REG_LONG; ++t) {
              const int delta_t = va[t] - vb[t];
              d0 += delta_t * (int)(short)(lp_w[t] & 0xFFFFu) / 1024;
              d1 += delta_t * ((int)lp_w[t] >> 16) / 1024;
            }
          } else if (lp_in_lds) {
            for (int p = lane; p < P.nlong; p += 64) {
              const int4 q = lp_s[p];
              const int delta_t = v[q.x] - v[q.y];
              d0 += delta_t * q.z / 1024;
              d1 += delta_t * q.w / 1024;
            }
          } else {
            for (int p = lane; p < P.nlong; p += 64) {
              int a, b;
              brisk_long_pair(v, P.long_pairs + 4 * p, &a, &b);
              d0 += a;
              d1 += b;
            }
          }
          d0 = ds_wave_sum(d0);
          d1 = ds_wave_sum(d1);
          if (lane == kq) { md0 = d0; md1 = d1; }
        }
        if (estimate) {
          const float ang = brisk_angle_from_direction(md0, md1);
          dkp[(long)cur.frame * kp_cap + (int)(myrec.w >> 8)].angle = ang;
          theta = brisk_theta_from_angle(ang, true);
        }
        __builtin_amdgcn_wave_barrier();
      }
      if (P.rotation_invariant && !estimate) theta = brisk_theta_from_angle(__uint_as_float(myrec.z), false);
      if (lane < cur.cnt) kth[lane] = theta;
      wave_sync();
      DS_T(2);
      {
        const DsSide s2 = pass(F, krec, cur.total, true, false, first, !two_passes, take, nsrc, nxt.cnt);
        if (!two_passes) side = s2;
      }
      DS_T(3);
      const int t3 = side.t;
      const uint4 nrec = side.rec;
      const DsTicket nn = decode(__builtin_amdgcn_readfirstlane(t3));
      uint4* krec_n = krec2 + (kb ^ 1) * RUN;
      if (lane < nxt.cnt) krec_n[lane] = nrec;
      const bool est_n = P.rotation_invariant && lane < nxt.cnt && __uint_as_float(nrec.z) == -1.0f;
      have_first = nxt.ok && __any(est_n);
      for (int kq = 0; kq < cur.cnt; ++kq) {
        const int* v = vals + kq * np;
        const int k = (int)((unsigned)__builtin_amdgcn_readfirstlane((int)krec[kq].w) >> 8);
        unsigned long long mine = 0;
        if (REGTAB) {
          int va[DS_REG_SHORT], vb[DS_REG_SHORT];
#pragma unroll
          for (int w = 0; w < DS_REG_SHORT; ++w) { va[w] = v[sp_ij[w] & 0xFF]; vb[w] = v[(sp_ij[w] >> 16) & 0xFF]; }
#pragma unroll
          for (int w = 0; w < DS_REG_SHORT; ++w) {
            const unsigned long long mk = __ballot(sp_ij[w] != 0xFFFFFFFFu && va[w] > vb[w]);
            if (lane == w) mine = mk;
          }
        } else {
          for (int w = 0; w < nwords; ++w) {
            const int p = w * 64 + lane;
            bool bit = false;
            if (p < P.nshort) { const unsigned q = sp_s[p]; bit = v[q & 0xFFFF] > v[q >> 16]; }
            const unsigned long long mk = __ballot(bit);
            if (lane == w) mine = mk;
          }
        }
        if (lane < nwords)
          *reinterpret_cast<unsigned long long*>(desc + ((long)cur.frame * kp_cap + k) * desc_pitch + lane * 8) = mine;
      }
      if (have_first) {
        wave_sync();
        first = fetch(krec_n, nxt.total, lane, false);
      }
      __builtin_amdgcn_wave_barrier();
      cur = nxt;
      nxt = nn;
      myrec = nrec;
      kb ^= 1;
      DS_T(4);
#ifdef DS_TIMING
      dt_acc[5] += 1;
#endif
    }
  }
#ifdef DS_TIMING
  if (lane == 0)
    for (int k = 0; k < 6; ++k) atomicAdd(&counters[0].dphase[k], (int)(dt_acc[k] >> (k < 5 ? 4 : 0)));
#endif
}

long brisk_dp_work_ints(int kp_cap) { return DP_W_BLK + (kp_cap + DP_THREADS - 1) / DP_THREADS + 16; }

static size_t describe_lds_bytes(const BriskPatternDev& P, int run, bool regtab) {
  const size_t table = regtab ? 0 : (P.nlong <= DS_LP_LDS ? (size_t)P.nlong * 16 : 0) + (((size_t)P.nshort * 4 + 15) & ~(size_t)15);
  const size_t per_wave = 2 * (size_t)run * 16 + (((size_t)run * 4 + 15) & ~(size_t)15) + (((size_t)run * P.npoints * 4 + 15) & ~(size_t)15) + 2 * DS_MAXQ * 4;
  return table + DS_WAVES * per_wave;
}

typedef void (*ds_kernel_t)(BriskGeom, BriskPatternDev, const uint8_t*, const uint32_t*, int, long, BriskFrameCounters*, BriskKeyPoint*, uint4*,
                            uint8_t*, int, int, int, int);

void brisk_launch_describe(const BriskGeom& G, const BriskPatternDev& P, const BriskDetectBuffers& B,
                           const BriskDescribeBuffers& Dd, int nframes, const BriskKeyPoint* kp_in, const int* n_in,
                           long n_in_stride, hipStream_t s, BriskProfiler* prof, const BriskOverlap* ov, int n_in_max) {
  brisk_prof_mark(prof, BRISK_STG_INTEGRAL, s);
  if (!ov && !((BRISK_DBG_FLAGS(G) & (1 << 19)) && (BRISK_DBG_FLAGS(G) & (1 << 27))))
    brisk_launch_integral(G, B.pyr, B.bandsum, Dd.integral, Dd.istride, Dd.iframe_elems, B.band_h, nframes, s, Dd.ibits, B.counters);
  brisk_prof_mark(prof, BRISK_STG_DESC_PREPARE, s);
  hipLaunchKernelGGL(k_desc_prepare, dim3(nframes), dim3(DP_THREADS), 0, s, G, P, kp_in, n_in, n_in_stride, B.counters, Dd.dkp,
                     Dd.dscale, Dd.dperm, Dd.drec, B.kp_cap, Dd.dp_work, Dd.dp_work_stride);
  if (B.kp_cap > DP_SMALL_N && (n_in_max < 0 || n_in_max > DP_SMALL_N)) {
    DpTiles T;
    T.w = G.L[0].w; T.h = G.L[0].h; T.shift = 6;
    while ((((T.w - 1) >> T.shift) + 1) * (((T.h - 1) >> T.shift) + 1) > DP_MAXBUCKETS) ++T.shift;
    T.tiles_x = ((T.w - 1) >> T.shift) + 1;
    const int nbuckets = T.tiles_x * (((T.h - 1) >> T.shift) + 1);
    const int dp_blocks = min((B.kp_cap + DP_THREADS - 1) / DP_THREADS, max(1, 512 / nframes));
    const dim3 grid(dp_blocks, nframes);
    hipLaunchKernelGGL(k_dp_count, grid, dim3(DP_THREADS), 0, s, G, P, T, kp_in, n_in, n_in_stride, B.kp_cap, Dd.dp_work, Dd.dp_work_stride);
    hipLaunchKernelGGL(k_dp_scan, dim3(nframes), dim3(DP_THREADS), 0, s, n_in, n_in_stride, B.kp_cap, nbuckets, B.counters, Dd.dp_work,
                       Dd.dp_work_stride);
    hipLaunchKernelGGL(k_dp_scatter, grid, dim3(DP_THREADS), 0, s, G, P, T, kp_in, n_in, n_in_stride, B.kp_cap, Dd.dp_work,
                       Dd.dp_work_stride, Dd.dkp, Dd.drec);
  }
  if (ov) (void)hipStreamWaitEvent(s, ov->join, 0);
  brisk_prof_mark(prof, BRISK_STG_DESCRIBE, s);
  {
    const int ncu = brisk_device_cus();
    int run_fixed = (BRISK_DBG_FLAGS(G) >> 8) & 0xF;
    if (P.has_bilinear) run_fixed = 1;
    if (run_fixed > DS_MAXRUN) run_fixed = DS_MAXRUN;
    int bpc = (BRISK_DBG_FLAGS(G) >> 12) & 0xF;
    if (!bpc) bpc = DS_BLOCKS_PER_CU;
    const bool regtab = P.reg_tables && !P.has_bilinear;
    const int run_max = P.has_bilinear ? 1 : DS_MAXRUN;
    size_t lds = describe_lds_bytes(P, run_max, regtab);
    const size_t lds_limit = 160 * 1024 / (size_t)(bpc + 1) + 512;
    if (lds < lds_limit && !(BRISK_DBG_FLAGS(G) & (1 << 28))) lds = lds_limit;
    const bool i24 = Dd.ibits == 24;
    ds_kernel_t fn = regtab ? (i24 ? k_describe<DS_MAXRUN, false, true, true> : k_describe<DS_MAXRUN, false, true, false>)
                            : (i24 ? k_describe<DS_MAXRUN, false, false, true> : k_describe<DS_MAXRUN, false, false, false>);
    if (P.has_bilinear) fn = k_describe<1, true, false, false>;
    (void)hipFuncSetAttribute((const void*)fn, hipFuncAttributeMaxDynamicSharedMemorySize, (int)lds);
    hipLaunchKernelGGL(fn, dim3(ncu * bpc), dim3(DS_WAVES * 64), lds, s, G, P, B.pyr, Dd.integral, Dd.istride, Dd.iframe_elems,
                       B.counters, Dd.dkp, Dd.drec, Dd.desc, B.kp_cap, Dd.desc_pitch, nframes, run_fixed);
  }
  brisk_prof_mark(prof, BRISK_STG_DESCRIBE + 1, s);
}
```

ethzasl_brisk_amd/csrc/brisk_kernels.h:

```cpp
#pragma once
#include <hip/hip_runtime.h>

#include "brisk_common.h"
#include "brisk_match_gate.h"
#include "brisk_match_epiline.h"
#include "brisk_match_guide.h"
#include "brisk_match_select.h"
#include "brisk_pair_verify.h"
#include "brisk_pair_refit.h"
#include "brisk_pair_epipolar.h"
#include "brisk_pair_epipolar_refit.h"
#include "brisk_track_link.h"
#include "brisk_track_points.h"

#define BRISK_DETECT_TILE_W 64
#ifndef BRISK_DETECT_ROWS_PER_THREAD
#define BRISK_DETECT_ROWS_PER_THREAD 4
#endif
#define BRISK_DETECT_TILE_H (16 * BRISK_DETECT_ROWS_PER_THREAD)

struct BriskTileTable {
  int first_tile[BRISK_MAX_LAYERS + 1];
  int tiles_x[BRISK_MAX_LAYERS];
  int total_tiles;
};

struct BriskDetectBuffers {
  uint8_t* pyr;
  uint16_t* smap;
  BriskCand* cand;
  uint8_t* blocks;
  int* tie_idx;
  unsigned* keys;
  BriskFrameCounters* counters;
  BriskKeyPoint* kp_out;
  uint32_t* bandsum;
  int band_h;
  int istride;
  int cand_cap, tie_cap, kp_cap;
};

struct BriskDescribeBuffers {
  uint32_t* integral;
  int istride;
  int ibits;
  long iframe_elems;
  BriskKeyPoint* dkp;
  int* dscale;
  int* dperm;
  uint4* drec;
  uint8_t* desc;
  int desc_pitch;
  int* dp_work;
  long dp_work_stride;
};
long brisk_dp_work_ints(int kp_cap);

#define BRISK_PROF_STAGES 9
#define BRISK_PROF_MAX_CALLS 64
struct BriskProfiler {
  bool on = false;
  int calls = 0;
  hipEvent_t ev[BRISK_PROF_MAX_CALLS][BRISK_PROF_STAGES + 1] = {};
  bool used[BRISK_PROF_MAX_CALLS][BRISK_PROF_STAGES + 1] = {};
  hipEvent_t side_ev[BRISK_PROF_MAX_CALLS][2] = {};
  bool side_used[BRISK_PROF_MAX_CALLS] = {};
  bool created = false;
};
enum { BRISK_STG_PYRAMID = 0, BRISK_STG_DETECT, BRISK_STG_CLASSIFY, BRISK_STG_TIES, BRISK_STG_FINALIZE,
       BRISK_STG_POSTFILTER ,
       BRISK_STG_INTEGRAL, BRISK_STG_DESC_PREPARE, BRISK_STG_DESCRIBE };
const char* brisk_stage_name(int i);
void brisk_prof_begin_call(BriskProfiler* P);
void brisk_prof_mark(BriskProfiler* P, int slot, hipStream_t s);
void brisk_prof_mark_side(BriskProfiler* P, int which, hipStream_t side);
void brisk_prof_destroy(BriskProfiler* P);

struct BriskOverlap {
  hipStream_t side;
  hipEvent_t fork, join;
  const BriskDescribeBuffers* Dd;
};
int brisk_device_cus();
void brisk_launch_detect(const BriskGeom& G, const BriskTileTable& T, const BriskDetectBuffers& B, int nframes,
                         const uint8_t* frames, long frame_pitch, int row_pitch, const uint8_t* mask,
                         long mask_frame_pitch, int mask_row_pitch, hipStream_t s, BriskProfiler* prof,
                         const BriskOverlap* ov = nullptr);
void brisk_launch_smap_clear(const BriskGeom& Gprev, const BriskDetectBuffers& B, int nframes, hipStream_t s);
void brisk_launch_compute_scale(const BriskGeom& G, const BriskDetectBuffers& B, const uint8_t* frame, int row_pitch,
                                const BriskKeyPoint* d_in, int n_in, int suppress, hipStream_t s);
void brisk_launch_layer0_only(const BriskGeom& G, const BriskDetectBuffers& B, int nframes, const uint8_t* frames,
                              long frame_pitch, int row_pitch, hipStream_t s);
void brisk_launch_integral(const BriskGeom& G, const uint8_t* pyr, const uint32_t* bandsum, uint32_t* integral, int istride,
                           long iframe_elems, int band_h, int nframes, hipStream_t s, int ibits = 32,
                           BriskFrameCounters* counters = nullptr);
void brisk_launch_publish_single(const BriskFrameCounters* counters, const BriskKeyPoint* kps, const uint8_t* desc, int which, int max_kp,
                                 int dev_pitch, int expect, uint8_t* host, unsigned o_cnt, unsigned o_kp, unsigned o_desc, int* done,
                                 unsigned seq, hipStream_t s);
void brisk_launch_batch_density(const BriskFrameCounters* counters, int nframes, int cand_cap, long long* host_word, hipStream_t s);
void brisk_launch_describe(const BriskGeom& G, const BriskPatternDev& P, const BriskDetectBuffers& B,
                           const BriskDescribeBuffers& Dd, int nframes, const BriskKeyPoint* kp_in, const int* n_in,
                           long n_in_stride, hipStream_t s, BriskProfiler* prof, const BriskOverlap* ov = nullptr,
                           int n_in_max = -1 );

struct BriskExportSlab {
  int* counts;
  int* flags;
  long long* offsets;
  uint32_t* kps;
  uint32_t* desc;
};
void brisk_launch_export_pack(const BriskFrameCounters* counters, const BriskKeyPoint* kps, const uint8_t* desc, int kp_cap, int dev_pitch,
                              int strings, int nframes, int which, long long rows_cap, int desc_stride, int cut_flag,
                              const BriskExportSlab& S, hipStream_t s);
void brisk_launch_export_egress(const BriskExportSlab& S, int nframes, int desc_stride, int* h_counts, int* h_flags, long long* h_offsets,
                                void* h_kps, void* h_desc, hipStream_t s);

void brisk_launch_stream_probe(const void* a, void* b, size_t bytes, int mode, hipStream_t s);

struct BriskDMatch {
  int queryIdx, trainIdx, imgIdx;
  float distance;
};
void brisk_launch_match_dist(const uint8_t* query, int q_pitch, int q0, int nqb, const uint8_t* train, int t_pitch, int nt,
                             int words, const uint8_t* mask, long mask_pitch, uint16_t* dist, long dist_pitch,
                             hipStream_t s);
void brisk_launch_match_masked_out(const uint8_t* mask, long mask_pitch, int q0, int nqb, const int* img_start,
                                   const int* has_mask, int nimg, int* masked, hipStream_t s);
void brisk_launch_match_knn(const uint16_t* dist, long dist_pitch, int q0, int nqb, int nt, const int* img_start, int nimg,
                            const int* masked, int k, BriskDMatch* out, int* out_count, hipStream_t s);
void brisk_launch_match_radius(const uint16_t* dist, long dist_pitch, int q0, int nqb, int nt, const int* img_start,
                               int nimg, const int* masked, float max_distance, int cap, BriskDMatch* out, int* out_count,
                               int dim_bytes, hipStream_t s);
bool brisk_launch_match_knn_fused(const uint8_t* query, int q_pitch, int nq, const uint8_t* train, int t_pitch, int nt,
                                  int words32, int k, BriskDMatch* out, int* out_count, hipStream_t s);

struct BriskDescSet {
  const uint8_t* desc;
  const int* counts;
  int count_stride;
  long frame_pitch;
  int row_pitch;
  int frames;
};
struct BriskPairSpec {
  int npairs, query_first, query_step, train_first, train_step;
  const int* pairs;
};
bool brisk_launch_match_knn_pairs(const BriskDescSet& Q, const BriskDescSet& T, const BriskPairSpec& P, int words32, int k, bool cross,
                                  int rows_cap, BriskDMatch* out, int* out_count, int* pair_rows, hipStream_t s);

bool brisk_launch_match_radius_pairs(const BriskDescSet& Q, const BriskDescSet& T, const BriskPairSpec& P, int words32, float max_distance,
                                     int cap, int rows_cap, BriskDMatch* out, int* out_count, int* pair_rows, hipStream_t s);
bool brisk_launch_match_radius_fused(const uint8_t* query, int q_pitch, int nq, const uint8_t* train, int t_pitch, int nt, int words32,
                                     float max_distance, int cap, BriskDMatch* out, int* out_count, hipStream_t s);

struct BriskKpSet {
  const char* kps;
  long frame_pitch;
};
bool brisk_launch_match_knn_pairs_gated(const BriskDescSet& Q, const BriskDescSet& T, const BriskKpSet& QK, const BriskKpSet& TK,
                                        const BriskMatchGate& gate, const BriskPairSpec& P, int words32, int k, bool cross, int rows_cap,
                                        BriskDMatch* out, int* out_count, int* pair_rows, hipStream_t s);
bool brisk_launch_match_radius_pairs_gated(const BriskDescSet& Q, const BriskDescSet& T, const BriskKpSet& QK, const BriskKpSet& TK,
                                           const BriskMatchGate& gate, const BriskPairSpec& P, int words32, float max_distance, int cap,
                                           int rows_cap, BriskDMatch* out, int* out_count, int* pair_rows, hipStream_t s);

bool brisk_launch_match_knn_pairs_guided(const BriskDescSet& Q, const BriskDescSet& T, const BriskKpSet& QK, const BriskKpSet& TK,
                                         const BriskPairModel* models, const BriskMatchGuide& guide, const BriskPairSpec& P, int words32, int k,
                                         int rows_cap, BriskDMatch* out, int* out_count, int* pair_rows, hipStream_t s);
bool brisk_launch_match_radius_pairs_guided(const BriskDescSet& Q, const BriskDescSet& T, const BriskKpSet& QK, const BriskKpSet& TK,
                                            const BriskPairModel* models, const BriskMatchGuide& guide, const BriskPairSpec& P, int words32,
                                            float max_distance, int cap, int rows_cap, BriskDMatch* out, int* out_count, int* pair_rows,
                                            hipStream_t s);

bool brisk_launch_match_knn_pairs_epiline(const BriskDescSet& Q, const BriskDescSet& T, const BriskKpSet& QK, const BriskKpSet& TK,
                                          const BriskPairEpipolarModel* models, const BriskMatchEpiGuide& guide, const BriskPairSpec& P,
                                          int words32, int k, int rows_cap, BriskDMatch* out, int* out_count, int* pair_rows, hipStream_t s);
bool brisk_launch_match_radius_pairs_epiline(const BriskDescSet& Q, const BriskDescSet& T, const BriskKpSet& QK, const BriskKpSet& TK,
                                             const BriskPairEpipolarModel* models, const BriskMatchEpiGuide& guide, const BriskPairSpec& P,
                                             int words32, float max_distance, int cap, int rows_cap, BriskDMatch* out, int* out_count,
                                             int* pair_rows, hipStream_t s);

bool brisk_launch_match_mutual_pairs_guided(const BriskDescSet& Q, const BriskDescSet& T, const BriskKpSet& QK, const BriskKpSet& TK,
                                            const BriskPairModel* models, const BriskMatchGuide& guide, const BriskPairSpec& P, int words32,
                                            int rows_cap, BriskDMatch* out, int* out_count, int* pair_rows, hipStream_t s);
bool brisk_launch_match_mutual_pairs_epiline(const BriskDescSet& Q, const BriskDescSet& T, const BriskKpSet& QK, const BriskKpSet& TK,
                                             const BriskPairEpipolarModel* models, const BriskMatchEpiGuide& guide, const BriskPairSpec& P,
                                             int words32, int rows_cap, BriskDMatch* out, int* out_count, int* pair_rows, hipStream_t s);

enum { BRISK_PAIR_ROWS_CUT = 1, BRISK_PAIR_BAD = 2, BRISK_PAIR_ENTRIES_CUT = 4, BRISK_PAIR_NO_MODEL = 8, BRISK_PAIR_REFIT = 0x10, BRISK_PAIR_MATCHES_CUT = 0x100 };
int brisk_match_export_blocks_per_pair(int rows_cap);
void brisk_launch_pair_select(const BriskDMatch* out, const int* out_count, const int* pair_rows, int npairs, int rows_cap, int per_row,
                              const BriskMatchSelect& sel, long long* blk, int* blk_over, long long matches_cap, int* counts, int* flags,
                              long long* offsets, BriskDMatch* matches, int* rows_copy, hipStream_t s);
void brisk_launch_pair_select_egress(const int* s_rows, const int* s_counts, const int* s_flags, const long long* s_offsets,
                                     const BriskDMatch* s_matches, int npairs, int* h_rows, int* h_counts, int* h_flags, long long* h_offsets,
                                     void* h_matches, hipStream_t s);

void brisk_launch_pair_verify(const BriskDescSet& Q, const BriskDescSet& T, const BriskKpSet& QK, const BriskKpSet& TK, const BriskPairSpec& P,
                              int rows_cap, const long long* offsets, const BriskDMatch* matches, long long in_cap, const BriskPairVerify& V,
                              unsigned char* keep, long long* kept, long long out_cap, BriskPairModel* models, int* counts, int* flags,
                              long long* out_offsets, BriskDMatch* out, hipStream_t s);
void brisk_launch_pair_epipolar(const BriskDescSet& Q, const BriskDescSet& T, const BriskKpSet& QK, const BriskKpSet& TK, const BriskPairSpec& P,
                                int rows_cap, const long long* offsets, const BriskDMatch* matches, long long in_cap, const BriskPairVerify& V,
                                unsigned char* keep, long long* kept, long long out_cap, BriskPairEpipolarModel* models, int* counts, int* flags,
                                long long* out_offsets, BriskDMatch* out, hipStream_t s);
void brisk_launch_pair_refit(const BriskDescSet& Q, const BriskDescSet& T, const BriskKpSet& QK, const BriskKpSet& TK, const BriskPairSpec& P,
                             int rows_cap, const long long* offsets, const BriskDMatch* matches, long long in_cap,
                             const BriskPairModel* in_models, const BriskPairRefit& R, unsigned char* keep, long long* kept, long long out_cap,
                             BriskPairModel* models, int* counts, int* flags, long long* out_offsets, BriskDMatch* out, hipStream_t s);
void brisk_launch_pair_epipolar_refit(const BriskDescSet& Q, const BriskDescSet& T, const BriskKpSet& QK, const BriskKpSet& TK,
                                      const BriskPairSpec& P, int rows_cap, const long long* offsets, const BriskDMatch* matches, long long in_cap,
                                      const BriskPairEpipolarModel* in_models, const BriskPairEpipolarRefit& R, unsigned char* keep,
                                      long long* kept, long long out_cap, BriskPairEpipolarModel* models, int* counts, int* flags,
                                      long long* out_offsets, BriskDMatch* out, hipStream_t s);

enum { BRISK_TRACK_C_LINKS = 0, BRISK_TRACK_C_LOST = 1, BRISK_TRACK_C_IGNORED = 2, BRISK_TRACK_COUNTERS = 4 };
enum { BRISK_TRACK_LIST_CUT = 1 };
int brisk_track_blocks_per_node(int rows_cap);
void brisk_launch_track_link(const int* node_rows, long long stride, int nodes, int rows_cap, const long long* offsets, const BriskDMatch* matches,
                             const long long* seed_track, const int* seed_age, long long first_new, const long long* d_first_new,
                             unsigned long long* claims, long long* blk, unsigned long long* counters, long long* words, int* prev,
                             long long* track, int* age, long long* summary, hipStream_t s);
void brisk_launch_track_list(const int* node_rows, long long stride, int nodes, int rows_cap, const int* prev, const long long* track,
                             const int* age, int min_len, long long tracks_cap, long long obs_cap, int* next, int* len, long long* piece,
                             long long* blk_pieces, long long* blk_obs, long long* words, long long* list_track, int* list_len,
                             long long* list_offsets, void* list_obs, long long* summary, hipStream_t s);

void brisk_launch_tracklist_points(const int* node_rows, long long stride, int nodes, int rows_cap, const long long* list_offsets,
                                   const void* list_obs, const long long* list_summary, long long obs_cap, const void* kps, long long frame_pitch,
                                   int kp_first, int kp_step, void* points, hipStream_t s);
void brisk_launch_tracklist_egress(const long long* s_summary, const long long* s_track, const int* s_len, const long long* s_offsets,
                                   const void* s_points, long long tracks_cap, long long points_cap, long long* h_summary, long long* h_track,
                                   int* h_len, long long* h_offsets, void* h_points, hipStream_t s);

void brisk_launch_bucketing(BriskKeyPoint* kp, BriskFrameCounters* counters, int* order, BriskKeyPoint* tmp, int kp_cap, int rows,
                            int cols, int nbu, int nbv, int max_keypoints, int nframes, hipStream_t s);
void brisk_launch_uniformity(BriskKeyPoint* kp, BriskFrameCounters* counters, int* order, BriskKeyPoint* tmp, uint8_t* occ,
                             long occ_frame, int ow, int kp_cap, float scaling, int max_keypoints, int nframes, hipStream_t s);

void brisk_launch_halfsample16(const uint16_t* src, int sstride, int w, int h, uint16_t* dst, int dstride, hipStream_t s);
void brisk_launch_twothirdsample16(const uint16_t* src, int sstride, int w, int h, uint16_t* dst, int dstride, hipStream_t s);
void brisk_launch_integral16(const uint16_t* src, int sstride, int w, int h, float* rowsum, float* out, int ostride, hipStream_t s);
```

ethzasl_brisk_amd/csrc/brisk_kernels.hip:

```cpp
#include <hip/hip_runtime.h>
#include <stdlib.h>

#include "brisk_common.h"
#include "brisk_device_detect.h"
#include "brisk_kernels.h"

#ifdef BRISK_HIP_TUNING
static int env_knob(const char* name, int dflt) {
  const char* v = getenv(name);
  return (v && *v) ? atoi(v) : dflt;
}
#else
#define env_knob(name, dflt) (dflt)
#endif


__device__ __forceinline__ BriskLayerView make_view(const BriskGeom& G, uint8_t* pyr, uint16_t* smap, int frame,
                                                    int l) {
  BriskLayerView v;
  const long base = (long)frame * G.pyr_elems + G.L[l].off;
  v.img = brisk_layer_img(G, pyr, frame, l);
  v.smap = smap + base;
  v.w = G.L[l].w;
  v.h = G.L[l].h;
// ... 736 lines not shown
                                                                BriskFrameCounters* counters, int* tie_idx, int cand_cap,
                                                                int tie_cap) {
  const int frame = blockIdx.y;
  if (counters[frame].nredo == 0 || counters[frame].low_score) return;
  const int n = min(counters[frame].ncand, cand_cap);
  for (int i = blockIdx.x * blockDim.x + threadIdx.x; i < n; i += gridDim.x * blockDim.x) {
    BriskCand* c = &cand[(long)frame * cand_cap + i];
    if (c->status != 0xFF) continue;
    const int l = c->layer, x = c->x, y = c->y, D = c->D;
    const bool has_above = !G.single_layer && (l + 1 < G.nlayers);
    const bool has_below = !G.single_layer && (l > 0);
    const BriskLayerView Lo = make_view(G, pyr, smap, frame, l);
    const BriskLayerView La = make_view(G, pyr, smap, frame, has_above ? l + 1 : l);
    const BriskLayerView Lb = make_view(G, pyr, smap, frame, has_below ? l - 1 : l);
    int nprobed = 0;
    unsigned flags = 0;
    BriskKeyPoint kp;
    kp.x = kp.y = kp.size = kp.response = 0.f;
    BriskTouch touch;
    touch.on = false; touch.mask = 0; touch.x0 = 0; touch.y0 = 0;
    bool e5 = false;
    const unsigned status = brisk_classify<true>(Lo, x, y, D, &nprobed);
    if (status != BRISK_ST_REJ && brisk_refine<true>(G, Lb, Lo, La, l, x, y, &kp, &e5, &touch)) flags |= 1;
    unsigned bits = ((unsigned)nprobed << 8) | (status << 12);
    if (e5) { flags |= 2; bits |= BRISK_SM_E5; }
    if (flags & 1) { c->kx = kp.x; c->ky = kp.y; c->ksize = kp.size; c->kresp = kp.response; }
    c->fp_x0 = (int16_t)touch.x0; c->fp_y0 = (int16_t)touch.y0; c->fp_mask = (uint16_t)touch.mask;
    c->status = (uint8_t)status;
    c->flags = (uint8_t)flags;
    if (status == BRISK_ST_PASS && touch.mask) {
      for (int b = 0; b < 16; ++b)
        if (touch.mask & (1u << b)) smap_or(La.smap, (long)(touch.y0 + (b >> 2)) * La.stride + touch.x0 + (b & 3), BRISK_SM_TOUCH);
    }
    if (status == BRISK_ST_TIE) {
      const int j = atomicAdd(&counters[frame].ntie[l], 1);
      if (j < tie_cap) tie_idx[((long)frame * BRISK_MAX_LAYERS + l) * tie_cap + j] = i;
      else atomicOr(&counters[frame].overflow, 2);
    }
    smap_or(Lo.smap, (long)y * Lo.stride + x, bits);
  }
}

#define OC_THREADS 256
__global__ void __launch_bounds__(OC_THREADS) k_order_candidates(BriskGeom G, const BriskCand* cand, BriskFrameCounters* counters,
                                                                 unsigned* order_scratch, int* row_scratch, long row_scratch_stride,
                                                                 int cand_cap, int only_flagged) {
  const int frame = blockIdx.x, tid = threadIdx.x;
  if (only_flagged && !counters[frame].low_score) return;
  const int n = min(counters[frame].ncand, cand_cap);
  const BriskCand* C = cand + (long)frame * cand_cap;
  unsigned* order = order_scratch + (long)frame * cand_cap * 2;
  int* rows = row_scratch + (long)frame * row_scratch_stride;
  __shared__ int rbase[BRISK_MAX_LAYERS + 1];
  if (tid == 0) {
    int acc = 0;
    for (int l = 0; l < G.nlayers; ++l) { rbase[l] = acc; acc += G.L[l].h; }
    rbase[G.nlayers] = acc;
  }
  __syncthreads();
  const int R = rbase[G.nlayers];
  if (2 * R + 2 > row_scratch_stride) {
    if (tid == 0) atomicOr(&counters[frame].overflow, 8);
    return;
  }
  for (int r = tid; r < 2 * R + 2; r += OC_THREADS) rows[r] = 0;
  __threadfence_block();
  __syncthreads();
  for (int i = tid; i < n; i += OC_THREADS) atomicAdd(&rows[rbase[C[i].layer] + C[i].y + 1], 1);
  __threadfence_block();
  __syncthreads();
  if (tid == 0) {
    int acc = 0;
    for (int r = 1; r <= R; ++r) { acc += rows[r]; rows[r] = acc; }
  }
  __threadfence_block();
  __syncthreads();
  int* fill = rows + R + 1;
  for (int i = tid; i < n; i += OC_THREADS) {
    const int b = rbase[C[i].layer] + C[i].y;
    order[rows[b] + atomicAdd(&fill[b], 1)] = (unsigned)i;
  }
  __threadfence_block();
  __syncthreads();
  for (int b = tid; b < R; b += OC_THREADS) {
    const int lo = rows[b], hi = rows[b + 1];
    for (int i = lo + 1; i < hi; ++i) {
      const unsigned v = order[i];
      const int xv = C[v].x;
      int j = i - 1;
      while (j >= lo && C[order[j]].x > xv) { order[j + 1] = order[j]; --j; }
      order[j + 1] = v;
    }
  }
}

__global__ void __launch_bounds__(64) k_ordered_keypoints(BriskGeom G, uint8_t* pyr, uint16_t* smap, const BriskCand* cand,
                                                           BriskFrameCounters* counters, const unsigned* order_scratch,
                                                           BriskKeyPoint* kp_out, int cand_cap, int kp_cap, const uint8_t* mask,
                                                           long mask_pitch_frame, int mask_row_pitch, int no_scale_nms, int only_flagged) {
  if (threadIdx.x != 0) return;
  const int frame = blockIdx.x;
  if (only_flagged && !counters[frame].low_score) return;
  const int n = min(counters[frame].ncand, cand_cap);
  counters[frame].full_clear = 1;
  if (counters[frame].overflow & 1) return;
  BriskOrderedOut out;
  out.kp = kp_out + (long)frame * kp_cap;
  out.cap = kp_cap;
  out.n = 0;
  out.mask = mask ? mask + (long)frame * mask_pitch_frame : nullptr;
  out.mask_row_pitch = mask_row_pitch;
  const bool undefined = brisk_ordered_walk(G, pyr + (long)frame * G.pyr_elems, smap + (long)frame * G.pyr_elems,
                                            cand + (long)frame * cand_cap, order_scratch + (long)frame * cand_cap * 2, n,
                                            no_scale_nms != 0, &out);
  if (undefined) atomicOr(&counters[frame].overflow, 16);
  counters[frame].nkp = min(out.n, kp_cap);
  if (out.n > kp_cap) atomicOr(&counters[frame].overflow, 4);
}

#define CS_THREADS 256
__global__ void __launch_bounds__(CS_THREADS) k_cs_admit(BriskGeom G, uint8_t* pyr, uint16_t* smap, const BriskKeyPoint* in, int n_in,
                                                          BriskFrameCounters* counters, int* adm) {
  __shared__ int wtot[CS_THREADS / 64];
  __shared__ int base;
  const int l = blockIdx.x, tid = threadIdx.x, wave = tid >> 6, lane = tid & 63;
  if (tid == 0) base = 0;
  __syncthreads();
  for (int k0 = 0; k0 < n_in; k0 += CS_THREADS) {
    const int k = k0 + tid;
    float kx = 0.f, ky = 0.f;
    const bool ok = k < n_in && brisk_provided_on_layer(G, l, in[k], &kx, &ky);
    const unsigned long long bal = __ballot(ok);
    if (lane == 0) wtot[wave] = __popcll(bal);
    __syncthreads();
    int wbase = 0, total = 0;
#pragma unroll
    for (int q = 0; q < CS_THREADS / 64; ++q) { wbase += (q < wave) ? wtot[q] : 0; total += wtot[q]; }
    if (ok) {
      adm[(long)l * n_in + base + wbase + __popcll(bal & ((1ull << lane) - 1ull))] = k;
      brisk_cs_touch(G, pyr, smap, l, kx, ky);
    }
    __syncthreads();
    if (tid == 0) base += total;
    __syncthreads();
  }
  if (tid == 0) {
    counters[0].ntie[l] = base;
    counters[0].full_clear = 1;
    if (base == 0) atomicOr(&counters[0].pad[0], 1);
  }
}

__global__ void __launch_bounds__(CS_THREADS) k_cs_scores(BriskGeom G, uint8_t* pyr, uint16_t* smap, const BriskKeyPoint* in, int n_in,
                                                           BriskFrameCounters* counters, const int* adm) {
  if (counters[0].pad[0]) return;
  const int l = blockIdx.y, j = blockIdx.x * CS_THREADS + threadIdx.x;
  if (j >= counters[0].ntie[l]) return;
  float kx, ky;
  (void)brisk_provided_on_layer(G, l, in[adm[(long)l * n_in + j]], &kx, &ky);
  if (brisk_cs_score(G, pyr, smap, l, kx, ky)) atomicOr(&counters[0].overflow, 16);
}

__global__ void __launch_bounds__(64) k_cs_refine(BriskGeom G, uint8_t* pyr, uint16_t* smap, const BriskKeyPoint* in, int n_in, int suppress,
                                                   BriskFrameCounters* counters, const int* adm, unsigned* tmp) {
  if (counters[0].pad[0] || (counters[0].overflow & 16)) return;
  const int l = blockIdx.y, j = blockIdx.x * 64 + threadIdx.x;
  const int cnt = counters[0].ntie[l];
  const bool flat = !suppress && !G.single_layer;
  if (flat && cnt > counters[0].ntie[0]) {
    if (j == 0) atomicOr(&counters[0].overflow, 16);
    return;
  }
  if (j >= cnt) return;
  BriskKeyPoint kp;
  bool valid = true;
  float kx, ky;
  if (flat) {
    const BriskKeyPoint src0 = in[adm[j]];
    (void)brisk_provided_on_layer(G, 0, src0, &kx, &ky);
    brisk_cs_flat(G, pyr, smap, l, src0, kx, ky, &kp);
  } else {
    const BriskKeyPoint src = in[adm[(long)l * n_in + j]];
    (void)brisk_provided_on_layer(G, l, src, &kx, &ky);
    valid = brisk_cs_refine(G, pyr, smap, l, src, kx, ky, &kp);
  }
  unsigned* t = tmp + ((long)l * n_in + j) * 8;
  t[7] = valid ? 1u : 0u;
  if (valid) {
    t[0] = __float_as_uint(kp.x); t[1] = __float_as_uint(kp.y); t[2] = __float_as_uint(kp.size); t[3] = __float_as_uint(kp.angle);
    t[4] = __float_as_uint(kp.response); t[5] = (unsigned)kp.octave; t[6] = (unsigned)kp.class_id;
  }
}

__global__ void __launch_bounds__(1024) k_cs_emit(BriskGeom G, BriskFrameCounters* counters, const unsigned* tmp, int n_in,
                                                   BriskKeyPoint* kp_out, int kp_cap) {
  if (counters[0].pad[0] || (counters[0].overflow & 16)) return;
  __shared__ int wtot[16];
  __shared__ int base;
  const int tid = threadIdx.x, wave = tid >> 6, lane = tid & 63;
  if (tid == 0) base = 0;
  __syncthreads();
  for (int l = 0; l < G.nlayers; ++l) {
    const int cnt = counters[0].ntie[l];
    for (int j0 = 0; j0 < cnt; j0 += 1024) {
      const int j = j0 + tid;
      const unsigned* t = tmp + ((long)l * n_in + j) * 8;
      const bool ok = j < cnt && t[7] != 0;
      const unsigned long long bal = __ballot(ok);
      if (lane == 0) wtot[wave] = __popcll(bal);
      __syncthreads();
      int wbase = 0, total = 0;
#pragma unroll
      for (int q = 0; q < 16; ++q) { wbase += (q < wave) ? wtot[q] : 0; total += wtot[q]; }
      const int pos = base + wbase + __popcll(bal & ((1ull << lane) - 1ull));
      if (ok && pos < kp_cap) {
        BriskKeyPoint kp;
        kp.x = __uint_as_float(t[0]); kp.y = __uint_as_float(t[1]); kp.size = __uint_as_float(t[2]); kp.angle = __uint_as_float(t[3]);
        kp.response = __uint_as_float(t[4]); kp.octave = (int)t[5]; kp.class_id = (int)t[6];
        kp_out[pos] = kp;
      }
      __syncthreads();
      if (tid == 0) base += total;
      __syncthreads();
    }
  }
  if (tid == 0) {
    counters[0].nkp = min(base, kp_cap);
    if (base > kp_cap) atomicOr(&counters[0].overflow, 4);
  }
}

__global__ void __launch_bounds__(64) k_compute_scale(BriskGeom G, uint8_t* pyr, uint16_t* smap, const BriskKeyPoint* in, int n_in,
                                                       int suppress, BriskFrameCounters* counters, unsigned* det_scratch,
                                                       int det_cap, BriskKeyPoint* kp_out, int kp_cap, int always) {
  if (threadIdx.x != 0 || blockIdx.x != 0) return;
  if (!always && !counters[0].pad[0]) return;
  counters[0].full_clear = 1;
  BriskOrderedOut out;
  out.kp = kp_out; out.cap = kp_cap; out.n = 0; out.mask = nullptr; out.mask_row_pitch = 0;
  bool cap_exceeded = false;
  const bool undefined = brisk_compute_scale_walk(G, pyr, smap, in, n_in, suppress != 0, det_scratch, det_cap, &out, &cap_exceeded);
  if (undefined) atomicOr(&counters[0].overflow, 16);
  if (cap_exceeded) atomicOr(&counters[0].overflow, 1);
  counters[0].nkp = min(out.n, kp_cap);
  if (out.n > kp_cap) atomicOr(&counters[0].overflow, 4);
}

#ifndef TR_WAVES
#define TR_WAVES 16
#endif
#define TR_THREADS (TR_WAVES * 64)
#define TR_WIN 9
#ifndef TR_CHUNK
#define TR_CHUNK 3072
#endif
#define TR_PROG_DONE 0x7FFFFFFF
#define TR_DONE_BIT 4
#define TR_BM_WORDS 512
#ifdef TR_TIMING
#define TR_T(i) { const long long now_ = (long long)wall_clock64(); tacc[i] += (int)(now_ - tlast); tlast = now_; }
#else
#define TR_T(i)
#endif
#ifdef TR_TIMELINE
#define TR_STAMP(c_, l_, k_) if (c_) counters[frame].tl[(l_) * 8 + (k_)] = (int)wall_clock64();
#else
#define TR_STAMP(c_, l_, k_)
#endif


static_assert(TR_WIN == BRISK_TIE_WIN, "brisk_state_static_list walks the tie kernel's window");
#define TR_KERNEL_NAME k_tie_resolve
#define TR_SORT_NAME tie_sort_large
#define TR_KERNEL_MASKS 0
#define TR_KERNEL_PAIR 0
#define TR_KERNEL_LIST 1
#include "brisk_tie_kernel.inc"
#undef TR_KERNEL_NAME
#undef TR_KERNEL_MASKS
#undef TR_KERNEL_LIST
#undef TR_SORT_NAME
#define TR_KERNEL_NAME k_tie_resolve_small
#define TR_SORT_NAME tie_sort_large_small
#define TR_KERNEL_MASKS 1
#define TR_KERNEL_LIST 0
#include "brisk_tie_kernel.inc"
#undef TR_KERNEL_NAME
#undef TR_SORT_NAME
#undef TR_KERNEL_PAIR
#define TR_KERNEL_NAME k_tie_resolve_pair
#define TR_SORT_NAME tie_sort_large_pair
#define TR_KERNEL_PAIR 1
#include "brisk_tie_kernel.inc"
#undef TR_KERNEL_NAME
#undef TR_KERNEL_PAIR
#undef TR_KERNEL_MASKS

#ifndef FN_THREADS
#define FN_THREADS 512
#endif
#define FN_BUCKETS 2048
#define FN_SMALL 3072
#define FN_SB 1024
__global__ void __launch_bounds__(FN_THREADS) k_finalize(BriskGeom G, const BriskCand* cand, BriskFrameCounters* counters,
                                                          unsigned* keys_scratch, BriskKeyPoint* kp_out, int cand_cap,
                                                          int kp_cap, const uint8_t* mask, long mask_pitch_frame,
                                                          int mask_row_pitch) {
  __shared__ int nvalid;
  __shared__ unsigned skey[FN_SMALL];
  __shared__ unsigned sidx[FN_SMALL];
  BRISK_CHAIN_SETPRIO();
  const int frame = blockIdx.x, tid = threadIdx.x;
  if (counters[frame].low_score) return;
  const int n = min(counters[frame].ncand, cand_cap);
  const BriskCand* C = cand + (long)frame * cand_cap;
  unsigned* keys = keys_scratch + (long)frame * cand_cap * 2;
  if (tid == 0) nvalid = 0;
  __syncthreads();
  constexpr int FN_U = 4;
  for (int i0 = tid; i0 < n; i0 += FN_U * FN_THREADS) {
    unsigned sw[FN_U], ck[FN_U];
#pragma unroll
    for (int u = 0; u < FN_U; ++u) {
      const int i = min(i0 + u * FN_THREADS, n - 1);
      sw[u] = *reinterpret_cast<const unsigned*>(reinterpret_cast<const uint8_t*>(&C[i]) + 4);
      ck[u] = C[i].key;
    }
#pragma unroll
    for (int u = 0; u < FN_U; ++u) {
      const int i = i0 + u * FN_THREADS;
      bool valid = i < n && ((sw[u] >> 16) & 0xFFu) == BRISK_ST_PASS && ((sw[u] >> 24) & 1u);
      if (valid && mask) {
        const BriskCand& c = C[i];
        const uint8_t* m = mask + (long)frame * mask_pitch_frame;
        valid = m[(long)(int)(c.ky + 0.5f) * mask_row_pitch + (int)(c.kx + 0.5f)] != 0;
      }
      if (valid) {
        const int j = atomicAdd(&nvalid, 1);
        keys[2 * j] = ck[u];
        keys[2 * j + 1] = (unsigned)i;
        if (j < FN_SMALL) { skey[j] = ck[u]; sidx[j] = (unsigned)i; }
      }
    }
  }
  __threadfence_block();
  __syncthreads();
  const int nv = nvalid;
  if (nv > FN_SMALL) {
    if (tid == 0) counters[frame].nvalid_large = nv;
    return;
  }
  {
    __shared__ int rbase[BRISK_MAX_LAYERS + 1];
    __shared__ int bhead[FN_SB];
    __shared__ int bstart[FN_SB];
    __shared__ int bnext[FN_SMALL];
    __shared__ int wsum[FN_THREADS / 64];
    if (tid == 0) {
      int acc = 0;
      for (int l = 0; l < G.nlayers; ++l) { rbase[l] = acc; acc += G.L[l].h; }
      rbase[G.nlayers] = acc;
    }
    for (int b = tid; b < FN_SB; b += FN_THREADS) { bhead[b] = -1; bstart[b] = 0; }
    __syncthreads();
    int shift = 0;
    while ((rbase[G.nlayers] >> shift) >= FN_SB) ++shift;
    auto bucket_of = [&](unsigned key) { return (rbase[key >> 26] + (int)((key >> 13) & 0x1FFF)) >> shift; };
    for (int j = tid; j < nv; j += FN_THREADS) {
      const int b = bucket_of(skey[j]);
      atomicAdd(&bstart[b], 1);
      bnext[j] = atomicExch(&bhead[b], j);
    }
    __syncthreads();
    {
      constexpr int PER = FN_SB / FN_THREADS;
      int loc[PER], sum = 0;
#pragma unroll
      for (int q = 0; q < PER; ++q) { loc[q] = bstart[tid * PER + q]; sum += loc[q]; }
      const int incl = wave_inclusive_scan(sum);
      const int lane = tid & 63, wave = tid >> 6;
      if (lane == 63) wsum[wave] = incl;
      __syncthreads();
      int woff = 0;
#pragma unroll
      for (int q = 0; q < FN_THREADS / 64; ++q) woff += (q < wave) ? wsum[q] : 0;
      int run = woff + incl - sum;
#pragma unroll
      for (int q = 0; q < PER; ++q) { bstart[tid * PER + q] = run; run += loc[q]; }
    }
    __syncthreads();
    for (int j = tid; j < nv; j += FN_THREADS) {
      const unsigned k = skey[j];
      const BriskCand& c = C[sidx[j]];
      const float4 r = *reinterpret_cast<const float4*>(&c.kx);
      const int lyr = c.layer;
      const int b = bucket_of(k);
      int rank = bstart[b];
      for (int q = bhead[b]; q >= 0; q = bnext[q]) rank += (skey[q] < k) ? 1 : 0;
      if (rank < kp_cap) {
        BriskKeyPoint kp;
        kp.x = r.x; kp.y = r.y; kp.size = r.z; kp.angle = -1.0f; kp.response = r.w;
        kp.octave = G.single_layer ? 0 : lyr; kp.class_id = -1;
        kp_out[(long)frame * kp_cap + rank] = kp;
      }
    }
  }
  if (tid == 0) {
    counters[frame].nkp = min(nv, kp_cap);
    if (nv > kp_cap) atomicOr(&counters[frame].overflow, 4);
  }
}

__global__ void __launch_bounds__(FN_THREADS) k_finalize_large(BriskGeom G, const BriskCand* cand, BriskFrameCounters* counters,
                                                                const unsigned* keys_scratch, unsigned* scratch2,
                                                                long scratch2_stride, BriskKeyPoint* kp_out, int cand_cap,
                                                                int kp_cap) {
  const int frame = blockIdx.x, tid = threadIdx.x;
  const int nv = counters[frame].nvalid_large;
  if (nv <= 0) return;
  __shared__ int bstart[FN_BUCKETS + 1];
  __shared__ int bfill[FN_BUCKETS];
  __shared__ int rbase[BRISK_MAX_LAYERS + 1];
  __shared__ int wsum[FN_THREADS / 64];
  const BriskCand* C = cand + (long)frame * cand_cap;
  const unsigned* keys = keys_scratch + (long)frame * cand_cap * 2;
  unsigned* tmp = scratch2 + (long)frame * scratch2_stride;
  if (tid == 0) {
    int acc = 0;
    for (int l = 0; l < G.nlayers; ++l) { rbase[l] = acc; acc += G.L[l].h; }
    rbase[G.nlayers] = acc;
  }
  for (int b = tid; b < FN_BUCKETS; b += FN_THREADS) { bstart[b] = 0; bfill[b] = 0; }
  __syncthreads();
  int shift = 0;
  while ((rbase[G.nlayers] >> shift) >= FN_BUCKETS) ++shift;
  for (int j = tid; j < nv; j += FN_THREADS) {
    const unsigned key = keys[2 * j];
    atomicAdd(&bstart[(rbase[key >> 26] + (int)((key >> 13) & 0x1FFF)) >> shift], 1);
  }
  __syncthreads();
  {
    constexpr int PER = FN_BUCKETS / FN_THREADS;
    int loc[PER], sum = 0;
#pragma unroll
    for (int q = 0; q < PER; ++q) { loc[q] = bstart[tid * PER + q]; sum += loc[q]; }
    int incl = sum;
    const int lane = tid & 63, wave = tid >> 6;
#pragma unroll
    for (int off = 1; off < 64; off <<= 1) {
      const int v = __shfl_up(incl, off, 64);
      if (lane >= off) incl += v;
    }
    if (lane == 63) wsum[wave] = incl;
    __syncthreads();
    int woff = 0;
#pragma unroll
    for (int q = 0; q < FN_THREADS / 64; ++q) woff += (q < wave) ? wsum[q] : 0;
    int run = woff + incl - sum;
#pragma unroll
    for (int q = 0; q < PER; ++q) { bstart[tid * PER + q] = run; run += loc[q]; }
    if (tid == FN_THREADS - 1) bstart[FN_BUCKETS] = run;
  }
  __syncthreads();
  for (int j = tid; j < nv; j += FN_THREADS) {
    const unsigned key = keys[2 * j];
    const int b = (rbase[key >> 26] + (int)((key >> 13) & 0x1FFF)) >> shift;
    const int pos = bstart[b] + atomicAdd(&bfill[b], 1);
    tmp[2 * pos] = key;
    tmp[2 * pos + 1] = keys[2 * j + 1];
  }
  __threadfence();
  __syncthreads();
  for (int pos = tid; pos < nv; pos += FN_THREADS) {
    const unsigned key = tmp[2 * pos];
    const int b = (rbase[key >> 26] + (int)((key >> 13) & 0x1FFF)) >> shift;
    int rank = bstart[b];
    for (int q = bstart[b]; q < bstart[b + 1]; ++q) rank += (tmp[2 * q] < key) ? 1 : 0;
    if (rank < kp_cap) {
      const BriskCand& c = C[tmp[2 * pos + 1]];
      BriskKeyPoint kp;
      kp.x = c.kx; kp.y = c.ky; kp.size = c.ksize; kp.angle = -1.0f; kp.response = c.kresp;
      kp.octave = G.single_layer ? 0 : c.layer; kp.class_id = -1;
      kp_out[(long)frame * kp_cap + rank] = kp;
    }
  }
  if (tid == 0) {
    counters[frame].nkp = min(nv, kp_cap);
    if (nv > kp_cap) atomicOr(&counters[frame].overflow, 4);
  }
}

#define II_THREADS 512
#define II_BAND 64
#define II_CHUNK (II_THREADS * 4)

__device__ __forceinline__ unsigned ii_wg_scan(unsigned total, unsigned (*wave_tot)[II_THREADS / 64], int buf, unsigned* wg_total) {
  const int lane = threadIdx.x & 63, wave = threadIdx.x >> 6;
  const unsigned incl = (unsigned)wave_inclusive_scan((int)total);
  if (lane == 63) wave_tot[buf][wave] = incl;
  __syncthreads();
  unsigned woff = 0, tot = 0;
#pragma unroll
  for (int q = 0; q < II_THREADS / 64; ++q) {
    const unsigned v = wave_tot[buf][q];
    woff += (q < wave) ? v : 0;
    tot += v;
  }
  *wg_total = tot;
  return woff + incl - total;
}

#ifndef II_ROWS
#define II_ROWS 3
#endif
#define II_MAXCHUNKS 4
__device__ __forceinline__ uint2 ii_fetch(const uint8_t* row, int stride, int c0 ) {
  const int a = min(max(c0 - 4, 0), stride - 4), b = min(c0, stride - 4);
  return make_uint2(*reinterpret_cast<const unsigned*>(row + a), *reinterpret_cast<const unsigned*>(row + b));
}
__device__ __forceinline__ void ii_unpack(uint2 raw, int stride, int w, int c0, unsigned* px) {
  const unsigned prev = (c0 >= 4 && c0 - 4 < stride) ? raw.x : 0u, cur = (c0 < stride) ? raw.y : 0u;
  px[0] = (c0 - 1 >= 0 && c0 - 1 < w) ? (prev >> 24) : 0;
  px[1] = (c0 < w) ? (cur & 0xFF) : 0;
  px[2] = (c0 + 1 < w) ? ((cur >> 8) & 0xFF) : 0;
  px[3] = (c0 + 2 < w) ? ((cur >> 16) & 0xFF) : 0;
}

typedef uint32_t __attribute__((ext_vector_type(3))) ii_u32x3;
__device__ __forceinline__ void ii_store4(bool b24, uint32_t* out, long row, int istride, int c0, unsigned a0, unsigned a1, unsigned a2, unsigned a3) {
  if (b24) {
    ii_u32x3 v;
    v.x = (a0 & 0xFFFFFFu) | (a1 << 24);
    v.y = ((a1 >> 8) & 0xFFFFu) | (a2 << 16);
    v.z = ((a2 >> 16) & 0xFFu) | (a3 << 8);
    *reinterpret_cast<ii_u32x3*>(reinterpret_cast<uint8_t*>(out) + (row * istride + c0) * 3) = v;
  } else {
    *reinterpret_cast<uint4*>(out + row * istride + c0) = make_uint4(a0, a1, a2, a3);
  }
}
template <int NCH, bool B24, bool SUB>
__global__ void __launch_bounds__(II_THREADS) k_integral_final(BriskGeom G, const uint8_t* __restrict__ pyr,
                                                               const uint32_t* __restrict__ bandsum,
                                                               uint32_t* __restrict__ integral, int istride, long iframe_elems,
                                                               int nbands, int band_h, BriskFrameCounters* counters, int nsub, int sub_h) {
  __shared__ unsigned wave_tot[2][II_THREADS / 64];
  const int frame = blockIdx.y, band = SUB ? (int)blockIdx.x / nsub : (int)blockIdx.x;
  const int sub = SUB ? (int)blockIdx.x - band * nsub : 0;
  constexpr bool b24 = B24;
  if (counters && blockIdx.x == 0 && threadIdx.x == 0) counters[frame].i24 = b24 ? 1 : 0;
  const int w = G.L[0].w, h = G.L[0].h, stride = G.L[0].stride;
  const uint8_t* img = brisk_layer_img(G, pyr, frame, 0);
  uint32_t* out = integral + (long)frame * iframe_elems;
  const int yb = band * band_h;
  const int y0 = SUB ? yb + sub * sub_h : yb;
  const int y1 = SUB ? min(min(h, yb + band_h), y0 + sub_h) : min(h, y0 + band_h);
  if (SUB && y0 >= y1) return;
  int buf = 0;
  unsigned acc[NCH][4];
  uint2 raw[NCH];
#pragma unroll
  for (int ch = 0; ch < NCH; ++ch) raw[ch] = ii_fetch(img + (long)min(y0, h - 1) * stride, stride, ch * II_CHUNK + threadIdx.x * 4);
  {
    unsigned carry = 0;
#pragma unroll
    for (int ch = 0; ch < NCH; ++ch) {
      const int c0 = ch * II_CHUNK + threadIdx.x * 4;
      uint4 C = make_uint4(0, 0, 0, 0);
      if (c0 <= w)
        for (int b = 0; b < band; ++b) {
          const uint4 v = *reinterpret_cast<const uint4*>(bandsum + ((long)frame * nbands + b) * istride + c0);
          C.x += v.x; C.y += v.y; C.z += v.z; C.w += v.w;
        }
      if (SUB && c0 <= w) {
        for (int r0 = yb; r0 < y0; r0 += 6) {
          uint2 rr[6];
#pragma unroll
          for (int k = 0; k < 6; ++k) rr[k] = ii_fetch(img + (long)min(r0 + k, y0 - 1) * stride, stride, c0);
#pragma unroll
          for (int k = 0; k < 6; ++k) {
            unsigned px[4];
            ii_unpack(rr[k], stride, w, c0, px);
            if (r0 + k < y0) { C.x += px[0]; C.y += px[1]; C.z += px[2]; C.w += px[3]; }
          }
        }
      }
      if (c0 + 1 > w) C.y = 0;
      if (c0 + 2 > w) C.z = 0;
      if (c0 + 3 > w) C.w = 0;
      const unsigned s0 = C.x, s1 = s0 + C.y, s2 = s1 + C.z, s3 = s2 + C.w;
      unsigned tot;
      const unsigned o = ii_wg_scan(s3, wave_tot, buf, &tot) + carry;
      buf ^= 1;
      carry += tot;
      acc[ch][0] = o + s0; acc[ch][1] = o + s1; acc[ch][2] = o + s2; acc[ch][3] = o + s3;
      if (band == 0 && sub == 0 && c0 <= w) ii_store4(b24, out, 0, istride, c0, 0, 0, 0, 0);
    }
  }
  __shared__ unsigned wave_totr[2][II_THREADS / 64][II_ROWS];
  uint2 rawr[II_ROWS][NCH];
#pragma unroll
  for (int k = 0; k < II_ROWS; ++k)
#pragma unroll
    for (int ch = 0; ch < NCH; ++ch)
      rawr[k][ch] = (k == 0) ? raw[ch] : ii_fetch(img + (long)min(y0 + k, h - 1) * stride, stride, ch * II_CHUNK + threadIdx.x * 4);
  const int lane = threadIdx.x & 63, wave = threadIdx.x >> 6;
  for (int y = y0; y < y1; y += II_ROWS) {
    uint2 nxt[II_ROWS][NCH];
#pragma unroll
    for (int k = 0; k < II_ROWS; ++k) {
      const int yn = min(y + II_ROWS + k, y1 - 1);
#pragma unroll
      for (int ch = 0; ch < NCH; ++ch) nxt[k][ch] = ii_fetch(img + (long)yn * stride, stride, ch * II_CHUNK + threadIdx.x * 4);
    }
    unsigned carry[II_ROWS];
#pragma unroll
    for (int k = 0; k < II_ROWS; ++k) carry[k] = 0;
#pragma unroll
    for (int ch = 0; ch < NCH; ++ch) {
      const int c0 = ch * II_CHUNK + threadIdx.x * 4;
      unsigned s[II_ROWS][4], incl[II_ROWS];
#pragma unroll
      for (int k = 0; k < II_ROWS; ++k) {
        unsigned px[4] = {0, 0, 0, 0};
        if (c0 <= w && y + k < y1) ii_unpack(rawr[k][ch], stride, w, c0, px);
        s[k][0] = px[0]; s[k][1] = s[k][0] + px[1]; s[k][2] = s[k][1] + px[2]; s[k][3] = s[k][2] + px[3];
        incl[k] = (unsigned)wave_inclusive_scan((int)s[k][3]);
        if (lane == 63) wave_totr[buf][wave][k] = incl[k];
      }
      __syncthreads();
#pragma unroll
      for (int k = 0; k < II_ROWS; ++k) {
        unsigned wo = 0, tot = 0;
#pragma unroll
        for (int q = 0; q < II_THREADS / 64; ++q) {
          const unsigned v = wave_totr[buf][q][k];
          wo += (q < wave) ? v : 0;
          tot += v;
        }
        const unsigned o = wo + incl[k] - s[k][3] + carry[k];
        carry[k] += tot;
        acc[ch][0] += o + s[k][0]; acc[ch][1] += o + s[k][1]; acc[ch][2] += o + s[k][2]; acc[ch][3] += o + s[k][3];
        if (c0 <= w && y + k < y1) ii_store4(b24, out, (long)(y + k + 1), istride, c0, acc[ch][0], acc[ch][1], acc[ch][2], acc[ch][3]);
      }
      buf ^= 1;
    }
#pragma unroll
    for (int k = 0; k < II_ROWS; ++k)
#pragma unroll
      for (int ch = 0; ch < NCH; ++ch) rawr[k][ch] = nxt[k][ch];
  }
}

void brisk_launch_integral(const BriskGeom& G, const uint8_t* pyr, const uint32_t* bandsum, uint32_t* integral, int istride,
                            long iframe_elems, int band_h, int nframes, hipStream_t s, int ibits, BriskFrameCounters* counters) {
  const int nbands = (G.L[0].h + band_h - 1) / band_h;
  const int nchunks = (G.L[0].w + 1 + II_CHUNK - 1) / II_CHUNK;
  static const int sub_knob = env_knob("BRISK_II_SUB", -1);
  const int sub_h = ((sub_knob > 0 ? sub_knob : (band_h >= 96 ? 18 : 15)) + II_ROWS - 1) / II_ROWS * II_ROWS;
  const bool sub = sub_knob != 0 && nframes <= 4 && sub_h < band_h;
  const int nsub = sub ? (band_h + sub_h - 1) / sub_h : 1;
  const dim3 grid(nbands * nsub, nframes), block(II_THREADS);
  static const int pad_lds = env_knob("BRISK_II_LDS", 0);
  const bool b24 = ibits == 24 && counters;
#define II_LAUNCH1(NCH, LDS, B24_, SUB_)                                                                                                   \
  hipLaunchKernelGGL((k_integral_final<NCH, B24_, SUB_>), grid, block, LDS, s, G, pyr, bandsum, integral, istride, iframe_elems, nbands,   \
                     band_h, counters, nsub, sub_h);
#define II_LAUNCH(NCH, LDS)                                                                                                                  \
  if (b24) { if (sub) { II_LAUNCH1(NCH, LDS, true, true) } else { II_LAUNCH1(NCH, LDS, true, false) } }                                      \
  else { if (sub) { II_LAUNCH1(NCH, LDS, false, true) } else { II_LAUNCH1(NCH, LDS, false, false) } }
  if (nchunks <= 1) { II_LAUNCH(1, pad_lds) }
  else if (nchunks == 2) { II_LAUNCH(2, 0) }
  else { II_LAUNCH(II_MAXCHUNKS, 0) }
#undef II_LAUNCH
#undef II_LAUNCH1
}

__global__ void __launch_bounds__(256) k_batch_density(const BriskFrameCounters* __restrict__ counters, int nframes, int cand_cap,
                                                       long long* __restrict__ host_word) {
  __shared__ long long part[4];
  long long sum = 0;
  for (int f = threadIdx.x; f < nframes; f += 256) sum += min(counters[f].ncand, cand_cap);
  for (int off = 32; off > 0; off >>= 1) sum += __shfl_xor(sum, off, 64);
  if ((threadIdx.x & 63) == 0) part[threadIdx.x >> 6] = sum;
  __syncthreads();
  if (threadIdx.x == 0) {
    const long long total = part[0] + part[1] + part[2] + part[3];
    __hip_atomic_store(host_word, (total & 0xFFFFFFFFFFll) | ((long long)nframes << 40), __ATOMIC_RELAXED, __HIP_MEMORY_SCOPE_SYSTEM);
  }
}
void brisk_launch_batch_density(const BriskFrameCounters* counters, int nframes, int cand_cap, long long* host_word, hipStream_t s) {
  hipLaunchKernelGGL(k_batch_density, dim3(1), dim3(256), 0, s, counters, nframes, cand_cap, host_word);
}

__global__ void __launch_bounds__(256) k_publish_single(const BriskFrameCounters* __restrict__ counters, const BriskKeyPoint* __restrict__ kps,
                                                        const uint8_t* __restrict__ desc, int which, int max_kp, int dev_pitch,
                                                        uint8_t* host, unsigned o_cnt, unsigned o_kp, unsigned o_desc, int* done, unsigned seq) {
  const int tid = threadIdx.x, gt = blockIdx.x * blockDim.x + tid, gn = gridDim.x * blockDim.x;
  const int cnt = (counters[0].overflow & 7) ? 0 : (which ? counters[0].ndesc : counters[0].nkp);
  const bool fits = cnt <= max_kp;
  const int n = fits ? cnt : 0;
  if (blockIdx.x == 0)
    for (int i = tid; i < (int)(sizeof(BriskFrameCounters) / 4); i += blockDim.x)
      reinterpret_cast<int*>(host + o_cnt)[i] = reinterpret_cast<const int*>(counters)[i];
  {
    const int* src = reinterpret_cast<const int*>(kps);
    int* dst = reinterpret_cast<int*>(host + o_kp);
    const int nd = n * (int)(sizeof(BriskKeyPoint) / 4);
    for (int i = gt; i < nd; i += gn) dst[i] = src[i];
  }
  if (desc) {
    const uint2* src = reinterpret_cast<const uint2*>(desc);
    uint2* dst = reinterpret_cast<uint2*>(host + o_desc);
    const long nd = (long)n * dev_pitch / 8;
    for (long i = gt; i < nd; i += gn) dst[i] = src[i];
  }
  __threadfence_system();
  __syncthreads();
  if (tid == 0) {
    const int old = __hip_atomic_fetch_add(done, 1, __ATOMIC_ACQ_REL, __HIP_MEMORY_SCOPE_AGENT);
    if (old == (int)gridDim.x - 1) {
      __hip_atomic_store(done, 0, __ATOMIC_RELAXED, __HIP_MEMORY_SCOPE_AGENT);
      __threadfence_system();
      __hip_atomic_store(reinterpret_cast<unsigned*>(host), seq | (fits ? 0u : 0x80000000u), __ATOMIC_RELEASE, __HIP_MEMORY_SCOPE_SYSTEM);
    }
  }
}
void brisk_launch_publish_single(const BriskFrameCounters* counters, const BriskKeyPoint* kps, const uint8_t* desc, int which, int max_kp,
                                 int dev_pitch, int expect, uint8_t* host, unsigned o_cnt, unsigned o_kp, unsigned o_desc, int* done,
                                 unsigned seq, hipStream_t s) {
  const long bytes = (long)expect * ((long)sizeof(BriskKeyPoint) + (desc ? dev_pitch : 0));
  int grid = (int)((bytes + 16383) / 16384);
  grid = grid < 1 ? 1 : (grid > 32 ? 32 : grid);
  hipLaunchKernelGGL(k_publish_single, dim3(grid), dim3(256), 0, s, counters, kps, desc, which, max_kp, dev_pitch, host, o_cnt, o_kp, o_desc,
                     done, seq);
}

int brisk_device_cus() {
  static int cus[64] = {};
  int dev = 0;
  if (hipGetDevice(&dev) != hipSuccess || dev < 0 || dev >= 64) return 256;
  int v = __atomic_load_n(&cus[dev], __ATOMIC_RELAXED);
  if (!v) {
    hipDeviceProp_t prop;
    v = (hipGetDeviceProperties(&prop, dev) == hipSuccess && prop.multiProcessorCount > 0) ? prop.multiProcessorCount : 256;
    __atomic_store_n(&cus[dev], v, __ATOMIC_RELAXED);
  }
  return v;
}

static inline int grid_for(long items, int per_block, int cap) {
  long b = (items + per_block - 1) / per_block;
  if (b < 1) b = 1;
  if (b > cap) b = cap;
  return (int)b;
}

const char* brisk_stage_name(int i) {
  static const char* n[BRISK_PROF_STAGES] = {"k_pyramid", "k_detect", "k_classify_refine", "k_tie_resolve", "k_finalize",
                                             "k_postfilter", "k_integral_final", "k_desc_prepare", "k_describe"};
  return (i >= 0 && i < BRISK_PROF_STAGES) ? n[i] : "?";
}

void brisk_prof_begin_call(BriskProfiler* P) {
  if (!P || !P->on) return;
  if (!P->created) {
    for (int c = 0; c < BRISK_PROF_MAX_CALLS; ++c)
      for (int k = 0; k <= BRISK_PROF_STAGES; ++k) (void)hipEventCreate(&P->ev[c][k]);
    for (int c = 0; c < BRISK_PROF_MAX_CALLS; ++c)
      for (int k = 0; k < 2; ++k) (void)hipEventCreate(&P->side_ev[c][k]);
    P->created = true;
  }
  const int c = P->calls % BRISK_PROF_MAX_CALLS;
  for (int k = 0; k <= BRISK_PROF_STAGES; ++k) P->used[c][k] = false;
  P->side_used[c] = false;
}

void brisk_prof_mark_side(BriskProfiler* P, int which, hipStream_t side) {
  if (!P || !P->on) return;
  const int c = P->calls % BRISK_PROF_MAX_CALLS;
  (void)hipEventRecord(P->side_ev[c][which], side);
  if (which == 1) P->side_used[c] = true;
}

void brisk_prof_destroy(BriskProfiler* P) {
  if (!P || !P->created) return;
  for (int c = 0; c < BRISK_PROF_MAX_CALLS; ++c) {
    for (int k = 0; k <= BRISK_PROF_STAGES; ++k) (void)hipEventDestroy(P->ev[c][k]);
    for (int k = 0; k < 2; ++k) (void)hipEventDestroy(P->side_ev[c][k]);
  }
  P->created = false;
}

void brisk_prof_mark(BriskProfiler* P, int slot, hipStream_t s) {
  if (!P || !P->on) return;
  const int c = P->calls % BRISK_PROF_MAX_CALLS;
  (void)hipEventRecord(P->ev[c][slot], s);
  P->used[c][slot] = true;
}

__global__ void __launch_bounds__(256) k_stream_copy(const float4* __restrict__ in, float4* __restrict__ out, long n) {
  for (long i = (long)blockIdx.x * blockDim.x + threadIdx.x; i < n; i += (long)gridDim.x * blockDim.x) out[i] = in[i];
}
__global__ void __launch_bounds__(256) k_stream_read(const float4* __restrict__ in, float* __restrict__ out, long n) {
  float s = 0;
  for (long i = (long)blockIdx.x * blockDim.x + threadIdx.x; i < n; i += (long)gridDim.x * blockDim.x) {
    const float4 v = in[i];
    s += v.x + v.y + v.z + v.w;
  }
  if (s == 1.2345f) out[0] = s;
}
void brisk_launch_stream_probe(const void* a, void* b, size_t bytes, int mode, hipStream_t s) {
  const long n = (long)(bytes / 16);
  if (mode == 0) hipLaunchKernelGGL(k_stream_copy, dim3(4096), dim3(256), 0, s, (const float4*)a, (float4*)b, n);
  else hipLaunchKernelGGL(k_stream_read, dim3(4096), dim3(256), 0, s, (const float4*)a, (float*)b, n);
}

void brisk_launch_smap_clear(const BriskGeom& Gprev, const BriskDetectBuffers& B, int nframes, hipStream_t s) {
  if (nframes > 0) hipLaunchKernelGGL(k_smap_clear, dim3(16, nframes), dim3(256), 0, s, Gprev, B.smap, B.cand, B.counters, B.cand_cap);
}

static void launch_pyramid(const BriskGeom& G, const BriskDetectBuffers& B, int nframes, const uint8_t* frames, long frame_pitch,
                           int row_pitch, hipStream_t s) {
  {
    const int even_levels = G.nlayers >= 7 ? 3 : G.nlayers >= 5 ? 2 : G.nlayers >= 3 ? 1 : 0;
    const int odd_levels = G.nlayers >= 8 ? 3 : G.nlayers >= 6 ? 2 : G.nlayers >= 4 ? 1 : G.nlayers >= 2 ? 0 : -1;
    const int ftx = (G.L[0].stride + 95) / 96, fty = (G.L[0].h + PF_BAND - 1) / PF_BAND;
    hipLaunchKernelGGL(k_pyramid_fused, dim3(ftx * fty, nframes), dim3(256), 0, s, G, frames, frame_pitch, row_pitch, B.pyr,
                       even_levels, odd_levels, ftx, fty, B.bandsum, B.istride);
    for (int l = 8; l < G.nlayers; ++l) {
      const long items = (long)(G.L[l].stride / 4) * G.L[l].h;
      hipLaunchKernelGGL(k_pyramid_level, dim3(grid_for(items, 256, 2048), nframes), dim3(256), 0, s, G, B.pyr, l - 2, l, 0);
    }
  }
}

void brisk_launch_detect(const BriskGeom& G, const BriskTileTable& T, const BriskDetectBuffers& B, int nframes,
                         const uint8_t* frames, long frame_pitch, int row_pitch, const uint8_t* mask,
                         long mask_frame_pitch, int mask_row_pitch, hipStream_t s, BriskProfiler* prof,
                         const BriskOverlap* ov) {
  (void)hipMemsetAsync(B.counters, 0, sizeof(BriskFrameCounters) * (size_t)nframes, s);
  brisk_prof_mark(prof, BRISK_STG_PYRAMID, s);
  const int probe_stop = env_knob("BRISK_DETECT_PROBE", 0);
  if (probe_stop != 2) launch_pyramid(G, B, nframes, frames, frame_pitch, row_pitch, s);
  static const int fork_at = env_knob("BRISK_INTEGRAL_FORK", 0);
  auto fork_integral = [&]() {
    (void)hipEventRecord(ov->fork, s);
    (void)hipStreamWaitEvent(ov->side, ov->fork, 0);
    brisk_prof_mark_side(prof, 0, ov->side);
    brisk_launch_integral(G, B.pyr, B.bandsum, ov->Dd->integral, ov->Dd->istride, ov->Dd->iframe_elems, B.band_h, nframes, ov->side,
                          ov->Dd->ibits, B.counters);
    brisk_prof_mark_side(prof, 1, ov->side);
    (void)hipEventRecord(ov->join, ov->side);
  };
  if (ov && fork_at == 1) fork_integral();
  brisk_prof_mark(prof, BRISK_STG_DETECT, s);
  hipLaunchKernelGGL(k_detect, dim3((T.total_tiles + 7) / 8 * 8, nframes), dim3(256), 0, s, G, T, B.pyr, B.smap, B.cand, B.counters,
                     B.cand_cap);
  if (probe_stop) return;
  if (ov && fork_at == 2) fork_integral();
  brisk_prof_mark(prof, BRISK_STG_CLASSIFY, s);
  const bool ordered_all = G.no_scale_nms || G.lower_threshold != BRISK_LOWER_THRESHOLD;
  const bool ordered_some = !ordered_all && G.threshold < BRISK_FAST_PATH_MIN_THRESHOLD;
  auto launch_ordered = [&](int only_flagged) {
    const long row_stride = (long)BRISK_MAX_LAYERS * B.tie_cap;
    hipLaunchKernelGGL(k_order_candidates, dim3(nframes), dim3(OC_THREADS), 0, s, G, B.cand, B.counters, B.keys, B.tie_idx,
                       row_stride, B.cand_cap, only_flagged);
    hipLaunchKernelGGL(k_ordered_keypoints, dim3(nframes), dim3(64), 0, s, G, B.pyr, B.smap, B.cand, B.counters, B.keys, B.kp_out,
                       B.cand_cap, B.kp_cap, mask, mask_frame_pitch, mask_row_pitch, G.no_scale_nms, only_flagged);
  };
  if (ordered_all) {
    brisk_prof_mark(prof, BRISK_STG_TIES, s);
    if (ov && fork_at != 1 && fork_at != 2) fork_integral();
    launch_ordered(0);
    brisk_prof_mark(prof, BRISK_STG_FINALIZE, s);
    brisk_prof_mark(prof, BRISK_STG_POSTFILTER, s);
    return;
  }
  static const int sb_knob = env_knob("BRISK_SB_BLOCKS", 0), cr_knob = env_knob("BRISK_CR_BLOCKS", 0);
  const int sb_blocks = sb_knob ? sb_knob : (nframes > 64 ? (nframes >= 256 ? 32 : 64) : 256), cr_blocks = cr_knob ? cr_knob : (nframes >= 64 ? 24 : 64);
  {
    const int sb_bpf = grid_for(B.cand_cap, SB_WAVES * SB_PER_WAVE, sb_blocks), cr_bpf = grid_for(B.cand_cap, 64, cr_blocks);
    hipLaunchKernelGGL(k_score_blocks, dim3(xcd_grid(nframes, sb_bpf)), dim3(SB_WAVES * 64), 0, s, G, B.pyr, B.smap, B.cand,
                       B.counters, B.blocks, B.cand_cap, nframes, sb_bpf);
    hipLaunchKernelGGL(k_classify_refine, dim3(xcd_grid(nframes, cr_bpf)), dim3(64), 0, s, G, B.pyr, B.smap, B.cand, B.counters,
                       B.blocks, B.tie_idx, B.cand_cap, B.tie_cap, nframes, cr_bpf);
  }
  hipLaunchKernelGGL(k_classify_refine_direct, dim3(8, nframes), dim3(64), 0, s, G, B.pyr, B.smap, B.cand, B.counters,
                     B.tie_idx, B.cand_cap, B.tie_cap);
  brisk_prof_mark(prof, BRISK_STG_TIES, s);
  if (ov && fork_at == 0) fork_integral();
  {
    static const int lpw_knob = env_knob("BRISK_TR_LPW", 0);
    const int per_wg = G.nlayers > 8 ? 192 : 256;
    int lpw_auto = G.nlayers;
    for (int c = 1; c <= G.nlayers; ++c)
      if (nframes * ((G.nlayers + c - 1) / c) <= per_wg) { lpw_auto = c; break; }
    const int lpw = lpw_knob ? min(lpw_knob, G.nlayers) : (nframes * G.nlayers <= 512 ? 1 : lpw_auto);
    int tr_grid = (nframes >= 8 ? (nframes + 7) / 8 * 8 : nframes) * ((G.nlayers + lpw - 1) / lpw);
    static const int persist_knob = env_knob("BRISK_TR_PERSIST", -1), pgrid_env = env_knob("BRISK_TR_PGRID", 0);
    const int pgrid_knob = pgrid_env > 0 ? pgrid_env : brisk_device_cus();
    const int persist = persist_knob >= 0 ? persist_knob : (tr_grid > pgrid_knob ? 1 : 0);
    if (persist && tr_grid > pgrid_knob) tr_grid = pgrid_knob;
    static const int waves_knob = env_knob("BRISK_TR_WAVES", 0);
    const int tr_waves = waves_knob ? min(max(waves_knob, 2), TR_WAVES) : ((!persist && lpw >= G.nlayers && nframes >= 192) ? 12 : TR_WAVES);
    static const int pair_knob = env_knob("BRISK_TR_PAIR", 1);
    static const int pair_min_knob = env_knob("BRISK_TR_PAIR_MIN", 0);
    static const int pair_mode_knob = env_knob("BRISK_TR_PAIR_MODE", 1);
    const int pair_min = (pair_min_knob ? pair_min_knob : 4 * (tr_waves - 1)) | (pair_mode_knob << 16);
    static const int bands_knob = env_knob("BRISK_TR_BANDS", 0);
    int bands = 1;
    if (lpw == 1 && !persist) {
      bands = bands_knob ? min(max(bands_knob, 1), BRISK_TIE_MAX_BANDS) : (tr_grid * 8 <= pgrid_knob ? 8 : tr_grid * 4 <= pgrid_knob ? 4 : tr_grid * 2 <= pgrid_knob ? 2 : 1);
      if (tr_grid * bands > pgrid_knob) bands = 1;
    }
    if ((nframes <= 64 && pair_knob) || pair_knob == 2)
      hipLaunchKernelGGL(k_tie_resolve_pair, dim3(tr_grid * bands), dim3(tr_waves * 64), 0, s, G, B.pyr, B.smap, B.cand, B.counters, B.tie_idx,
                         B.blocks, B.keys, B.cand_cap, B.tie_cap, nframes, lpw, persist, pair_min, bands);
    else if (nframes < 32)
      hipLaunchKernelGGL(k_tie_resolve_small, dim3(tr_grid), dim3(tr_waves * 64), 0, s, G, B.pyr, B.smap, B.cand, B.counters, B.tie_idx,
                         B.blocks, B.keys, B.cand_cap, B.tie_cap, nframes, lpw, persist, 0, 1);
    else
      hipLaunchKernelGGL(k_tie_resolve, dim3(tr_grid), dim3(tr_waves * 64), 0, s, G, B.pyr, B.smap, B.cand, B.counters, B.tie_idx,
                         B.blocks, B.keys, B.cand_cap, B.tie_cap, nframes, lpw, persist, 0, 1);
  }
  brisk_prof_mark(prof, BRISK_STG_FINALIZE, s);
  hipLaunchKernelGGL(k_finalize, dim3(nframes), dim3(FN_THREADS), 0, s, G, B.cand, B.counters, B.keys, B.kp_out, B.cand_cap,
                     B.kp_cap, mask, mask_frame_pitch, mask_row_pitch);
  hipLaunchKernelGGL(k_finalize_large, dim3(nframes), dim3(FN_THREADS), 0, s, G, B.cand, B.counters, B.keys,
                     reinterpret_cast<unsigned*>(B.tie_idx), (long)BRISK_MAX_LAYERS * B.tie_cap, B.kp_out, B.cand_cap, B.kp_cap);
  if (ordered_some) launch_ordered(1);
  brisk_prof_mark(prof, BRISK_STG_POSTFILTER, s);
}

void brisk_launch_compute_scale(const BriskGeom& G, const BriskDetectBuffers& B, const uint8_t* frame, int row_pitch,
                                const BriskKeyPoint* d_in, int n_in, int suppress, hipStream_t s) {
  (void)hipMemsetAsync(B.counters, 0, sizeof(BriskFrameCounters), s);
  launch_pyramid(G, B, 1, frame, 0, row_pitch, s);
  static const int seq_knob = env_knob("BRISK_CS_SEQUENTIAL", 0);
  const bool parallel = !seq_knob && (long)G.nlayers * n_in <= 2L * B.cand_cap;
  if (parallel) {
    int* adm = reinterpret_cast<int*>(B.keys);
    unsigned* tmp = reinterpret_cast<unsigned*>(B.blocks);
    hipLaunchKernelGGL(k_cs_admit, dim3(G.nlayers), dim3(CS_THREADS), 0, s, G, B.pyr, B.smap, d_in, n_in, B.counters, adm);
    hipLaunchKernelGGL(k_cs_scores, dim3((n_in + CS_THREADS - 1) / CS_THREADS, G.nlayers), dim3(CS_THREADS), 0, s, G, B.pyr, B.smap, d_in,
                       n_in, B.counters, adm);
    hipLaunchKernelGGL(k_cs_refine, dim3((n_in + 63) / 64, G.nlayers), dim3(64), 0, s, G, B.pyr, B.smap, d_in, n_in, suppress, B.counters,
                       adm, tmp);
    hipLaunchKernelGGL(k_cs_emit, dim3(1), dim3(1024), 0, s, G, B.counters, tmp, n_in, B.kp_out, B.kp_cap);
  }
  hipLaunchKernelGGL(k_compute_scale, dim3(1), dim3(64), 0, s, G, B.pyr, B.smap, d_in, n_in, suppress, B.counters, B.keys,
                     2 * B.cand_cap, B.kp_out, B.kp_cap, parallel ? 0 : 1);
}

void brisk_launch_layer0_only(const BriskGeom& G, const BriskDetectBuffers& B, int nframes, const uint8_t* frames,
                              long frame_pitch, int row_pitch, hipStream_t s) {
  const int etx = (G.L[0].stride + 63) / 64, ety = (G.L[0].h + 63) / 64;
  hipLaunchKernelGGL(k_pyramid_even, dim3(etx * ety, nframes), dim3(256), 0, s, G, frames, frame_pitch, row_pitch, B.pyr, 0,
                     etx, ety, B.bandsum, B.istride);
}
```

Before: 80740.

## Fuse finalize_large into finalize, inline desc-prepare phases, overlap smap clear and density

Merges k_finalize_large into k_finalize so large-candidate frames are handled in the same launch. It adds a single-block path in k_desc_prepare that runs count, scan and scatter in one kernel when dp_alone is set. For single-slice batches, the smap clear moves into the detect launch and the batch density kernel moves onto the side stream after the integral, removing separate launches from the main stream. This cuts launch count and serialization on small batches, but the large-frame path now shares the finalize kernel's shared-memory footprint and a single block per frame.

```diff
diff --git a/ethzasl_brisk_amd/csrc/brisk_capi.hip b/ethzasl_brisk_amd/csrc/brisk_capi.hip
--- a/ethzasl_brisk_amd/csrc/brisk_capi.hip
+++ b/ethzasl_brisk_amd/csrc/brisk_capi.hip
@@ -590,7 +590,12 @@
   int lower_threshold = BRISK_LOWER_THRESHOLD;
   bool format_as_full_batch = false;
   bool inplace_ok = true;
+  bool one_slice = false;
 };
+
+static bool slice_overlaps(const brisk_hip_ctx* ctx, const BatchArgs& A, bool overlap_integral) {
+  return A.do_detect && A.do_describe && overlap_integral && ctx->overlap && !(dbg_flags(ctx) & 0x10000);
+}
 
 static int ensure_filter_buffers(brisk_hip_ctx* ctx, int w, int h, int nframes, double uni_radius) {
   size_t need = 0;
@@ -632,7 +637,7 @@
   if (rc) return fail(ctx, rc, "hipStreamWaitEvent failed");
   ctx->img_cache.valid = false;
   brisk_prof_begin_call(&ctx->prof);
-  if (A.do_detect) {
+  if (A.do_detect && !A.one_slice) {
     if (ctx->dirty_frames > 0) brisk_launch_smap_clear(ctx->dirtyG, ctx->B, ctx->dirty_frames, s);
     ctx->dirtyG = ctx->G;
     ctx->dirty_frames = nframes;
@@ -664,7 +669,7 @@
   Di.desc += f0 * Bi.kp_cap * Di.desc_pitch;
   BriskOverlap ov{};
   const BriskOverlap* ovp = nullptr;
-  if (A.do_detect && A.do_describe && overlap_integral && ctx->overlap && !(dbg_flags(ctx) & 0x10000)) {
+  if (slice_overlaps(ctx, A, overlap_integral)) {
     if (!ctx->side) {
       int least = 0, greatest = 0;
       HIPCHK(ctx, hipDeviceGetStreamPriorityRange(&least, &greatest));
@@ -675,6 +680,23 @@
     }
     ov.side = ctx->side; ov.fork = ctx->side_fork; ov.join = ctx->side_join; ov.Dd = &Di;
     ovp = &ov;
+  }
+  BriskGeom Gprev;
+  if (A.do_detect && A.one_slice) {
+    Gprev = ctx->dirtyG;
+    if (ovp) {
+      ov.clear_G = &Gprev;
+      ov.clear_frames = ctx->dirty_frames;
+      if (!ctx->h_density.p) {
+        HIPCHK(ctx, ctx->h_density.grow(sizeof(long long), 0, hipHostMallocMapped));
+        *ctx->h_density.as<long long>() = 0;
+      }
+      ov.density_word = ctx->h_density.as<long long>();
+    } else if (ctx->dirty_frames > 0) {
+      brisk_launch_smap_clear(Gprev, ctx->B, ctx->dirty_frames, si);
+    }
+    ctx->dirtyG = ctx->G;
+    ctx->dirty_frames = nf;
   }
   BriskGeom Gs = ctx->G;
   {
@@ -716,12 +738,14 @@
 
 static int batch_end(brisk_hip_ctx* ctx, const BatchArgs& A, int nframes, hipStream_t s) {
   if (A.do_detect && A.do_describe) {
-    if (!ctx->h_density.p) {
-      HIPCHK(ctx, ctx->h_density.grow(sizeof(long long), 0, hipHostMallocMapped));
-      *ctx->h_density.as<long long>() = 0;
+    ctx->density_mpx = (double)A.w * (double)A.h / 1e6;
+    if (!(A.one_slice && slice_overlaps(ctx, A, true))) {
+      if (!ctx->h_density.p) {
+        HIPCHK(ctx, ctx->h_density.grow(sizeof(long long), 0, hipHostMallocMapped));
+        *ctx->h_density.as<long long>() = 0;
+      }
+      brisk_launch_batch_density(ctx->B.counters, nframes, ctx->B.cand_cap, ctx->h_density.as<long long>(), s);
     }
-    ctx->density_mpx = (double)A.w * (double)A.h / 1e6;
-    brisk_launch_batch_density(ctx->B.counters, nframes, ctx->B.cand_cap, ctx->h_density.as<long long>(), s);
   }
   if (ctx->prof.on) ctx->prof.calls++;
   HIPCHK(ctx, hipGetLastError());
@@ -751,12 +775,13 @@
   A.format_as_full_batch = full_batch;
   if (bucketing) { A.bk_u = bucketing[0]; A.bk_v = bucketing[1]; A.bk_max = bucketing[2]; }
   else if (uni_radius < 0.0) { A.bk_u = ctx->bk_u; A.bk_v = ctx->bk_v; A.bk_max = ctx->bk_max; }
+  int nsub = ctx->nsub;
+  if (nsub > 8) nsub = 8;
+  if (nframes < 16 * nsub) nsub = nframes >= 32 ? 2 : 1;
+  A.one_slice = nsub == 1;
   int rc = batch_begin(ctx, A, nframes, s);
   if (rc) return rc;
   WorkspaceGuard guard(ctx, s);
-  int nsub = ctx->nsub;
-  if (nsub > 8) nsub = 8;
-  if (nframes < 16 * nsub) nsub = nframes >= 32 ? 2 : 1;
   if (nsub > 1 && !ctx->sub_created) {
     for (int i = 0; i < 8; ++i) {
       HIPCHK(ctx, hipStreamCreateWithFlags(&ctx->sub[i], hipStreamNonBlocking));
diff --git a/ethzasl_brisk_amd/csrc/brisk_describe.hip b/ethzasl_brisk_amd/csrc/brisk_describe.hip
--- a/ethzasl_brisk_amd/csrc/brisk_describe.hip
+++ b/ethzasl_brisk_amd/csrc/brisk_describe.hip
@@ -34,10 +34,139 @@
   return ((unsigned)(y >> 6) << 24) | (((unsigned)x & 0x1FFFu) << 11) | low;
 }
 
+struct DpTiles { int shift, tiles_x, w, h; };
+__device__ __forceinline__ int dp_bucket(const DpTiles& T, float x, float y) {
+  const int xi = min(max((int)x, 0), T.w - 1), yi = min(max((int)y, 0), T.h - 1);
+  return (yi >> T.shift) * T.tiles_x + (xi >> T.shift);
+}
+struct DpItem { bool keep; int sc; BriskKeyPoint kp; };
+__device__ __forceinline__ DpItem dp_item(const BriskGeom& G, const BriskPatternDev& P, const BriskKeyPoint* K, int i, int n) {
+  DpItem it;
+  it.keep = false; it.sc = 0;
+  if (i < n) {
+    it.kp = K[i];
+    it.sc = brisk_scale_index(P, it.kp.size);
+    it.keep = brisk_inside_border(P, it.sc, it.kp.x, it.kp.y, G.L[0].w, G.L[0].h);
+  }
+  return it;
+}
+
+__device__ __forceinline__ void dp_count(const BriskGeom& G, const BriskPatternDev& P, const DpTiles& T, const BriskKeyPoint* K, int n,
+                                         int* wk, int part, int nparts, int* wtot) {
+  const int tid = threadIdx.x, wave = tid >> 6, lane = tid & 63;
+  for (int blk = part; blk * DP_THREADS < n; blk += nparts) {
+    const DpItem it = dp_item(G, P, K, blk * DP_THREADS + tid, n);
+    const unsigned long long bal = __ballot(it.keep);
+    if (lane == 0) wtot[wave] = __popcll(bal);
+    const unsigned long long bal_e = __ballot(it.keep && it.kp.angle == -1.0f);
+    if (lane == 0 && bal_e) atomicAdd(&wk[0], __popcll(bal_e));
+    if (it.keep) atomicAdd(&wk[DP_W_HIST + dp_bucket(T, it.kp.x, it.kp.y)], 1);
+    __syncthreads();
+    if (tid == 0) {
+      int t = 0;
+#pragma unroll
+      for (int k = 0; k < DP_THREADS / 64; ++k) t += wtot[k];
+      wk[DP_W_BLK + blk] = t;
+    }
+    __syncthreads();
+  }
+}
+__global__ void __launch_bounds__(DP_THREADS) k_dp_count(BriskGeom G, BriskPatternDev P, DpTiles T, const BriskKeyPoint* kp_in,
+                                                          const int* n_in_ptr, long n_in_stride, int kp_cap, int* work, long work_stride) {
+  __shared__ int wtot[DP_THREADS / 64];
+  const int frame = blockIdx.y;
+  const int n = min(*(const int*)((const char*)n_in_ptr + (long)frame * n_in_stride), kp_cap);
+  if (n <= DP_SMALL_N) return;
+  dp_count(G, P, T, kp_in + (long)frame * kp_cap, n, work + (long)frame * work_stride, blockIdx.x, gridDim.x, wtot);
+}
+
+__device__ __forceinline__ int dp_scan_inplace(int* v, int n, int* sh) {
+  const int tid = threadIdx.x, wave = tid >> 6, lane = tid & 63;
+  int carry = 0;
+  for (int i0 = 0; i0 < n; i0 += DP_THREADS) {
+    const int i = i0 + tid;
+    const int x = i < n ? v[i] : 0;
+    int incl = x;
+#pragma unroll
+    for (int off = 1; off < 64; off <<= 1) {
+      const int t = __shfl_up(incl, off, 64);
+      if (lane >= off) incl += t;
+    }
+    if (lane == 63) sh[wave] = incl;
+    __syncthreads();
+    int woff = 0, tot = 0;
+#pragma unroll
+    for (int k = 0; k < DP_THREADS / 64; ++k) { const int t = sh[k]; woff += (k < wave) ? t : 0; tot += t; }
+    if (i < n) v[i] = carry + woff + incl - x;
+    carry += tot;
+    __syncthreads();
+  }
+  return carry;
+}
+
+__device__ __forceinline__ void dp_scan(int n, int nbuckets, BriskFrameCounters* fc, int* wk, int* sh) {
+  const int m = dp_scan_inplace(wk + DP_W_BLK, (n + DP_THREADS - 1) / DP_THREADS, sh);
+  (void)dp_scan_inplace(wk + DP_W_HIST, nbuckets, sh);
+  if (threadIdx.x == 0) { fc->ndesc = m; fc->nestimate = wk[0]; fc->desc_ticket = 0; fc->orient_ticket = 0; }
+}
+__global__ void __launch_bounds__(DP_THREADS) k_dp_scan(const int* n_in_ptr, long n_in_stride, int kp_cap, int nbuckets,
+                                                         BriskFrameCounters* counters, int* work, long work_stride) {
+  __shared__ int sh[DP_THREADS / 64 + 1];
+  const int frame = blockIdx.x;
+  const int n = min(*(const int*)((const char*)n_in_ptr + (long)frame * n_in_stride), kp_cap);
+  if (n <= DP_SMALL_N) return;
+  dp_scan(n, nbuckets, &counters[frame], work + (long)frame * work_stride, sh);
+}
+
+__device__ __forceinline__ void dp_scatter(const BriskGeom& G, const BriskPatternDev& P, const DpTiles& T, const BriskKeyPoint* K, int n,
+                                           int* wk, int part, int nparts, BriskKeyPoint* dkp, uint4* drec, int* wtot) {
+  const int tid = threadIdx.x, wave = tid >> 6, lane = tid & 63;
+  for (int blk = part; blk * DP_THREADS < n; blk += nparts) {
+    const DpItem it = dp_item(G, P, K, blk * DP_THREADS + tid, n);
+    const unsigned long long bal = __ballot(it.keep);
+    if (lane == 0) wtot[wave] = __popcll(bal);
+    __syncthreads();
+    if (it.keep) {
+      int j = wk[DP_W_BLK + blk] + __popcll(bal & ((1ull << lane) - 1ull));
+#pragma unroll
+      for (int k = 0; k < DP_THREADS / 64; ++k) j += (k < wave) ? wtot[k] : 0;
+      dkp[j] = it.kp;
+      const int pos = atomicAdd(&wk[DP_W_HIST + dp_bucket(T, it.kp.x, it.kp.y)], 1);
+      drec[pos] = make_uint4(__float_as_uint(it.kp.x), __float_as_uint(it.kp.y), __float_as_uint(it.kp.angle),
+                             (unsigned)it.sc | ((unsigned)j << 8));
+    }
+    __syncthreads();
+  }
+}
+__global__ void __launch_bounds__(DP_THREADS) k_dp_scatter(BriskGeom G, BriskPatternDev P, DpTiles T, const BriskKeyPoint* kp_in,
+                                                            const int* n_in_ptr, long n_in_stride, int kp_cap, int* work,
+                                                            long work_stride, BriskKeyPoint* dkp, uint4* drec) {
+  __shared__ int wtot[DP_THREADS / 64];
+  const int frame = blockIdx.y;
+  const int n = min(*(const int*)((const char*)n_in_ptr + (long)frame * n_in_stride), kp_cap);
+  if (n <= DP_SMALL_N) return;
+  dp_scatter(G, P, T, kp_in + (long)frame * kp_cap, n, work + (long)frame * work_stride, blockIdx.x, gridDim.x,
+             dkp + (long)frame * kp_cap, drec + (long)frame * kp_cap, wtot);
+}
+
+__device__ __forceinline__ void dp_frame_alone(const BriskGeom& G, const BriskPatternDev& P, const DpTiles& T, int nbuckets,
+                                               const BriskKeyPoint* K, int n, BriskFrameCounters* fc, int* wk, BriskKeyPoint* dkp,
+                                               uint4* drec, int* sh) {
+  __threadfence_block();
+  __syncthreads();
+  dp_count(G, P, T, K, n, wk, 0, 1, sh);
+  __threadfence_block();
+  __syncthreads();
+  dp_scan(n, nbuckets, fc, wk, sh);
+  __threadfence_block();
+  __syncthreads();
+  dp_scatter(G, P, T, K, n, wk, 0, 1, dkp, drec, sh);
+}
+
 __global__ void __launch_bounds__(DP_THREADS) k_desc_prepare(BriskGeom G, BriskPatternDev P, const BriskKeyPoint* kp_in,
                                                        const int* n_in_ptr, long n_in_stride, BriskFrameCounters* counters,
                                                        BriskKeyPoint* dkp, int* dscale, int* dperm, uint4* drec, int kp_cap,
-                                                       int* work, long work_stride) {
+                                                       int* work, long work_stride, DpTiles T, int nbuckets, int dp_alone) {
   __shared__ int wtot[DP_THREADS / 64];
   __shared__ int base, nest;
   __shared__ __attribute__((aligned(16))) unsigned pkey[DP_MAXSORT + 4];
@@ -48,6 +177,9 @@
   if (n > DP_SMALL_N) {
     int* wk = work + (long)frame * work_stride;
     for (int q = tid; q < DP_W_BLK; q += DP_THREADS) wk[q] = 0;
+    if (dp_alone)
+      dp_frame_alone(G, P, T, nbuckets, K, n, &counters[frame], wk, dkp + (long)frame * kp_cap, drec + (long)frame * kp_cap,
+                     reinterpret_cast<int*>(pkey));
     return;
   }
   __shared__ uint4 srec[DP_SMALL_N];
@@ -151,112 +283,6 @@
       for (int q = bhead[b]; q >= 0; q = bnext[q]) r += (pkey[q] < kj) ? 1 : 0;
       drec[(long)frame * kp_cap + r] = srec[j];
     }
-  }
-}
-
-struct DpTiles { int shift, tiles_x, w, h; };
-__device__ __forceinline__ int dp_bucket(const DpTiles& T, float x, float y) {
-  const int xi = min(max((int)x, 0), T.w - 1), yi = min(max((int)y, 0), T.h - 1);
-  return (yi >> T.shift) * T.tiles_x + (xi >> T.shift);
-}
-struct DpItem { bool keep; int sc; BriskKeyPoint kp; };
-__device__ __forceinline__ DpItem dp_item(const BriskGeom& G, const BriskPatternDev& P, const BriskKeyPoint* K, int i, int n) {
-  DpItem it;
-  it.keep = false; it.sc = 0;
-  if (i < n) {
-    it.kp = K[i];
-    it.sc = brisk_scale_index(P, it.kp.size);
-    it.keep = brisk_inside_border(P, it.sc, it.kp.x, it.kp.y, G.L[0].w, G.L[0].h);
-  }
-  return it;
-}
-
-__global__ void __launch_bounds__(DP_THREADS) k_dp_count(BriskGeom G, BriskPatternDev P, DpTiles T, const BriskKeyPoint* kp_in,
-                                                          const int* n_in_ptr, long n_in_stride, int kp_cap, int* work, long work_stride) {
-  __shared__ int wtot[DP_THREADS / 64];
-  const int frame = blockIdx.y, tid = threadIdx.x, wave = tid >> 6, lane = tid & 63;
-  const int n = min(*(const int*)((const char*)n_in_ptr + (long)frame * n_in_stride), kp_cap);
-  if (n <= DP_SMALL_N) return;
-  int* wk = work + (long)frame * work_stride;
-  for (int blk = blockIdx.x; blk * DP_THREADS < n; blk += gridDim.x) {
-    const DpItem it = dp_item(G, P, kp_in + (long)frame * kp_cap, blk * DP_THREADS + tid, n);
-    const unsigned long long bal = __ballot(it.keep);
-    if (lane == 0) wtot[wave] = __popcll(bal);
-    const unsigned long long bal_e = __ballot(it.keep && it.kp.angle == -1.0f);
-    if (lane == 0 && bal_e) atomicAdd(&wk[0], __popcll(bal_e));
-    if (it.keep) atomicAdd(&wk[DP_W_HIST + dp_bucket(T, it.kp.x, it.kp.y)], 1);
-    __syncthreads();
-    if (tid == 0) {
-      int t = 0;
-#pragma unroll
-      for (int k = 0; k < DP_THREADS / 64; ++k) t += wtot[k];
-      wk[DP_W_BLK + blk] = t;
-    }
-    __syncthreads();
-  }
-}
-
-__device__ __forceinline__ int dp_scan_inplace(int* v, int n, int* sh) {
-  const int tid = threadIdx.x, wave = tid >> 6, lane = tid & 63;
-  int carry = 0;
-  for (int i0 = 0; i0 < n; i0 += DP_THREADS) {
-    const int i = i0 + tid;
-    const int x = i < n ? v[i] : 0;
-    int incl = x;
-#pragma unroll
-    for (int off = 1; off < 64; off <<= 1) {
-      const int t = __shfl_up(incl, off, 64);
-      if (lane >= off) incl += t;
-    }
-    if (lane == 63) sh[wave] = incl;
-    __syncthreads();
-    int woff = 0, tot = 0;
-#pragma unroll
-    for (int k = 0; k < DP_THREADS / 64; ++k) { const int t = sh[k]; woff += (k < wave) ? t : 0; tot += t; }
-    if (i < n) v[i] = carry + woff + incl - x;
-    carry += tot;
-    __syncthreads();
-  }
-  return carry;
-}
-
-__global__ void __launch_bounds__(DP_THREADS) k_dp_scan(const int* n_in_ptr, long n_in_stride, int kp_cap, int nbuckets,
-                                                         BriskFrameCounters* counters, int* work, long work_stride) {
-  __shared__ int sh[DP_THREADS / 64 + 1];
-  const int frame = blockIdx.x;
-  const int n = min(*(const int*)((const char*)n_in_ptr + (long)frame * n_in_stride), kp_cap);
-  if (n <= DP_SMALL_N) return;
-  int* wk = work + (long)frame * work_stride;
-  const int m = dp_scan_inplace(wk + DP_W_BLK, (n + DP_THREADS - 1) / DP_THREADS, sh);
-  (void)dp_scan_inplace(wk + DP_W_HIST, nbuckets, sh);
-  if (threadIdx.x == 0) {
-    counters[frame].ndesc = m; counters[frame].nestimate = wk[0]; counters[frame].desc_ticket = 0; counters[frame].orient_ticket = 0;
-  }
-}
-
-__global__ void __launch_bounds__(DP_THREADS) k_dp_scatter(BriskGeom G, BriskPatternDev P, DpTiles T, const BriskKeyPoint* kp_in,
-                                                            const int* n_in_ptr, long n_in_stride, int kp_cap, int* work,
-                                                            long work_stride, BriskKeyPoint* dkp, uint4* drec) {
-  __shared__ int wtot[DP_THREADS / 64];
-  const int frame = blockIdx.y, tid = threadIdx.x, wave = tid >> 6, lane = tid & 63;
-  const int n = min(*(const int*)((const char*)n_in_ptr + (long)frame * n_in_stride), kp_cap);
-  if (n <= DP_SMALL_N) return;
-  int* wk = work + (long)frame * work_stride;
-  for (int blk = blockIdx.x; blk * DP_THREADS < n; blk += gridDim.x) {
-    const DpItem it = dp_item(G, P, kp_in + (long)frame * kp_cap, blk * DP_THREADS + tid, n);
-    const unsigned long long bal = __ballot(it.keep);
-    if (lane == 0) wtot[wave] = __popcll(bal);
-    __syncthreads();
-    if (it.keep) {
-      int j = wk[DP_W_BLK + blk] + __popcll(bal & ((1ull << lane) - 1ull));
-#pragma unroll
-      for (int k = 0; k < DP_THREADS / 64; ++k) j += (k < wave) ? wtot[k] : 0;
-      dkp[(long)frame * kp_cap + j] = it.kp;
-      const int pos = atomicAdd(&wk[DP_W_HIST + dp_bucket(T, it.kp.x, it.kp.y)], 1);
-      drec[(long)frame * kp_cap + pos] = make_uint4(__float_as_uint(it.kp.x), __float_as_uint(it.kp.y), __float_as_uint(it.kp.angle),
-                                                    (unsigned)it.sc | ((unsigned)j << 8));
-    }
-    __syncthreads();
   }
 }
 
@@ -794,15 +820,15 @@
   if (!ov && !((BRISK_DBG_FLAGS(G) & (1 << 19)) && (BRISK_DBG_FLAGS(G) & (1 << 27))))
     brisk_launch_integral(G, B.pyr, B.bandsum, Dd.integral, Dd.istride, Dd.iframe_elems, B.band_h, nframes, s, Dd.ibits, B.counters);
   brisk_prof_mark(prof, BRISK_STG_DESC_PREPARE, s);
+  DpTiles T;
+  T.w = G.L[0].w; T.h = G.L[0].h; T.shift = 6;
+  while ((((T.w - 1) >> T.shift) + 1) * (((T.h - 1) >> T.shift) + 1) > DP_MAXBUCKETS) ++T.shift;
+  T.tiles_x = ((T.w - 1) >> T.shift) + 1;
+  const int nbuckets = T.tiles_x * (((T.h - 1) >> T.shift) + 1);
+  const int dp_blocks = min((B.kp_cap + DP_THREADS - 1) / DP_THREADS, max(1, 512 / nframes));
   hipLaunchKernelGGL(k_desc_prepare, dim3(nframes), dim3(DP_THREADS), 0, s, G, P, kp_in, n_in, n_in_stride, B.counters, Dd.dkp,
-                     Dd.dscale, Dd.dperm, Dd.drec, B.kp_cap, Dd.dp_work, Dd.dp_work_stride);
-  if (B.kp_cap > DP_SMALL_N && (n_in_max < 0 || n_in_max > DP_SMALL_N)) {
-    DpTiles T;
-    T.w = G.L[0].w; T.h = G.L[0].h; T.shift = 6;
-    while ((((T.w - 1) >> T.shift) + 1) * (((T.h - 1) >> T.shift) + 1) > DP_MAXBUCKETS) ++T.shift;
-    T.tiles_x = ((T.w - 1) >> T.shift) + 1;
-    const int nbuckets = T.tiles_x * (((T.h - 1) >> T.shift) + 1);
-    const int dp_blocks = min((B.kp_cap + DP_THREADS - 1) / DP_THREADS, max(1, 512 / nframes));
+                     Dd.dscale, Dd.dperm, Dd.drec, B.kp_cap, Dd.dp_work, Dd.dp_work_stride, T, nbuckets, dp_blocks == 1 ? 1 : 0);
+  if (dp_blocks > 1 && B.kp_cap > DP_SMALL_N && (n_in_max < 0 || n_in_max > DP_SMALL_N)) {
     const dim3 grid(dp_blocks, nframes);
     hipLaunchKernelGGL(k_dp_count, grid, dim3(DP_THREADS), 0, s, G, P, T, kp_in, n_in, n_in_stride, B.kp_cap, Dd.dp_work, Dd.dp_work_stride);
     hipLaunchKernelGGL(k_dp_scan, dim3(nframes), dim3(DP_THREADS), 0, s, n_in, n_in_stride, B.kp_cap, nbuckets, B.counters, Dd.dp_work,
diff --git a/ethzasl_brisk_amd/csrc/brisk_kernels.h b/ethzasl_brisk_amd/csrc/brisk_kernels.h
--- a/ethzasl_brisk_amd/csrc/brisk_kernels.h
+++ b/ethzasl_brisk_amd/csrc/brisk_kernels.h
@@ -80,6 +80,9 @@
   hipStream_t side;
   hipEvent_t fork, join;
   const BriskDescribeBuffers* Dd;
+  const BriskGeom* clear_G;
+  int clear_frames;
+  long long* density_word;
 };
 int brisk_device_cus();
 void brisk_launch_detect(const BriskGeom& G, const BriskTileTable& T, const BriskDetectBuffers& B, int nframes,
diff --git a/ethzasl_brisk_amd/csrc/brisk_kernels.hip b/ethzasl_brisk_amd/csrc/brisk_kernels.hip
--- a/ethzasl_brisk_amd/csrc/brisk_kernels.hip
+++ b/ethzasl_brisk_amd/csrc/brisk_kernels.hip
@@ -1062,13 +1062,86 @@
 #define FN_BUCKETS 2048
 #define FN_SMALL 3072
 #define FN_SB 1024
+
+__device__ __forceinline__ void finalize_large(const BriskGeom& G, const BriskCand* C, BriskFrameCounters* fc, const unsigned* keys,
+                                               unsigned* tmp, BriskKeyPoint* kp_frame, int nv, int kp_cap, int* bstart, int* bfill,
+                                               int* rbase, int* wsum) {
+  const int tid = threadIdx.x;
+  if (tid == 0) {
+    int acc = 0;
+    for (int l = 0; l < G.nlayers; ++l) { rbase[l] = acc; acc += G.L[l].h; }
+    rbase[G.nlayers] = acc;
+  }
+  for (int b = tid; b < FN_BUCKETS; b += FN_THREADS) { bstart[b] = 0; bfill[b] = 0; }
+  __syncthreads();
+  int shift = 0;
+  while ((rbase[G.nlayers] >> shift) >= FN_BUCKETS) ++shift;
+  for (int j = tid; j < nv; j += FN_THREADS) {
+    const unsigned key = keys[2 * j];
+    atomicAdd(&bstart[(rbase[key >> 26] + (int)((key >> 13) & 0x1FFF)) >> shift], 1);
+  }
+  __syncthreads();
+  {
+    constexpr int PER = FN_BUCKETS / FN_THREADS;
+    int loc[PER], sum = 0;
+#pragma unroll
+    for (int q = 0; q < PER; ++q) { loc[q] = bstart[tid * PER + q]; sum += loc[q]; }
+    int incl = sum;
+    const int lane = tid & 63, wave = tid >> 6;
+#pragma unroll
+    for (int off = 1; off < 64; off <<= 1) {
+      const int v = __shfl_up(incl, off, 64);
+      if (lane >= off) incl += v;
+    }
+    if (lane == 63) wsum[wave] = incl;
+    __syncthreads();
+    int woff = 0;
+#pragma unroll
+    for (int q = 0; q < FN_THREADS / 64; ++q) woff += (q < wave) ? wsum[q] : 0;
+    int run = woff + incl - sum;
+#pragma unroll
+    for (int q = 0; q < PER; ++q) { bstart[tid * PER + q] = run; run += loc[q]; }
+    if (tid == FN_THREADS - 1) bstart[FN_BUCKETS] = run;
+  }
+  __syncthreads();
+  for (int j = tid; j < nv; j += FN_THREADS) {
+    const unsigned key = keys[2 * j];
+    const int b = (rbase[key >> 26] + (int)((key >> 13) & 0x1FFF)) >> shift;
+    const int pos = bstart[b] + atomicAdd(&bfill[b], 1);
+    tmp[2 * pos] = key;
+    tmp[2 * pos + 1] = keys[2 * j + 1];
+  }
+  __threadfence();
+  __syncthreads();
+  for (int pos = tid; pos < nv; pos += FN_THREADS) {
+    const unsigned key = tmp[2 * pos];
+    const int b = (rbase[key >> 26] + (int)((key >> 13) & 0x1FFF)) >> shift;
+    int rank = bstart[b];
+    for (int q = bstart[b]; q < bstart[b + 1]; ++q) rank += (tmp[2 * q] < key) ? 1 : 0;
+    if (rank < kp_cap) {
+      const BriskCand& c = C[tmp[2 * pos + 1]];
+      BriskKeyPoint kp;
+      kp.x = c.kx; kp.y = c.ky; kp.size = c.ksize; kp.angle = -1.0f; kp.response = c.kresp;
+      kp.octave = G.single_layer ? 0 : c.layer; kp.class_id = -1;
+      kp_frame[rank] = kp;
+    }
+  }
+  if (tid == 0) {
+    fc->nkp = min(nv, kp_cap);
+    if (nv > kp_cap) atomicOr(&fc->overflow, 4);
+  }
+}
+
 __global__ void __launch_bounds__(FN_THREADS) k_finalize(BriskGeom G, const BriskCand* cand, BriskFrameCounters* counters,
-                                                          unsigned* keys_scratch, BriskKeyPoint* kp_out, int cand_cap,
-                                                          int kp_cap, const uint8_t* mask, long mask_pitch_frame,
-                                                          int mask_row_pitch) {
+                                                          unsigned* keys_scratch, unsigned* scratch2, long scratch2_stride,
+                                                          BriskKeyPoint* kp_out, int cand_cap, int kp_cap, const uint8_t* mask,
+                                                          long mask_pitch_frame, int mask_row_pitch) {
   __shared__ int nvalid;
   __shared__ unsigned skey[FN_SMALL];
   __shared__ unsigned sidx[FN_SMALL];
+  __shared__ int rbase[BRISK_MAX_LAYERS + 1];
+  __shared__ int wsum[FN_THREADS / 64];
+  static_assert(FN_BUCKETS + 1 <= FN_SMALL, "finalize_large's bucket arrays take the place of skey / sidx");
   BRISK_CHAIN_SETPRIO();
   const int frame = blockIdx.x, tid = threadIdx.x;
   if (counters[frame].low_score) return;
@@ -1108,14 +1181,14 @@
   const int nv = nvalid;
   if (nv > FN_SMALL) {
     if (tid == 0) counters[frame].nvalid_large = nv;
+    finalize_large(G, C, &counters[frame], keys, scratch2 + (long)frame * scratch2_stride, kp_out + (long)frame * kp_cap, nv, kp_cap,
+                   reinterpret_cast<int*>(skey), reinterpret_cast<int*>(sidx), rbase, wsum);
     return;
   }
   {
-    __shared__ int rbase[BRISK_MAX_LAYERS + 1];
     __shared__ int bhead[FN_SB];
     __shared__ int bstart[FN_SB];
     __shared__ int bnext[FN_SMALL];
-    __shared__ int wsum[FN_THREADS / 64];
     if (tid == 0) {
       int acc = 0;
       for (int l = 0; l < G.nlayers; ++l) { rbase[l] = acc; acc += G.L[l].h; }
@@ -1163,85 +1236,6 @@
         kp.octave = G.single_layer ? 0 : lyr; kp.class_id = -1;
         kp_out[(long)frame * kp_cap + rank] = kp;
       }
-    }
-  }
-  if (tid == 0) {
-    counters[frame].nkp = min(nv, kp_cap);
-    if (nv > kp_cap) atomicOr(&counters[frame].overflow, 4);
-  }
-}
-
-__global__ void __launch_bounds__(FN_THREADS) k_finalize_large(BriskGeom G, const BriskCand* cand, BriskFrameCounters* counters,
-                                                                const unsigned* keys_scratch, unsigned* scratch2,
-                                                                long scratch2_stride, BriskKeyPoint* kp_out, int cand_cap,
-                                                                int kp_cap) {
-  const int frame = blockIdx.x, tid = threadIdx.x;
-  const int nv = counters[frame].nvalid_large;
-  if (nv <= 0) return;
-  __shared__ int bstart[FN_BUCKETS + 1];
-  __shared__ int bfill[FN_BUCKETS];
-  __shared__ int rbase[BRISK_MAX_LAYERS + 1];
-  __shared__ int wsum[FN_THREADS / 64];
-  const BriskCand* C = cand + (long)frame * cand_cap;
-  const unsigned* keys = keys_scratch + (long)frame * cand_cap * 2;
-  unsigned* tmp = scratch2 + (long)frame * scratch2_stride;
-  if (tid == 0) {
-    int acc = 0;
-    for (int l = 0; l < G.nlayers; ++l) { rbase[l] = acc; acc += G.L[l].h; }
-    rbase[G.nlayers] = acc;
-  }
-  for (int b = tid; b < FN_BUCKETS; b += FN_THREADS) { bstart[b] = 0; bfill[b] = 0; }
-  __syncthreads();
-  int shift = 0;
-  while ((rbase[G.nlayers] >> shift) >= FN_BUCKETS) ++shift;
-  for (int j = tid; j < nv; j += FN_THREADS) {
-    const unsigned key = keys[2 * j];
-    atomicAdd(&bstart[(rbase[key >> 26] + (int)((key >> 13) & 0x1FFF)) >> shift], 1);
-  }
-  __syncthreads();
-  {
-    constexpr int PER = FN_BUCKETS / FN_THREADS;
-    int loc[PER], sum = 0;
-#pragma unroll
-    for (int q = 0; q < PER; ++q) { loc[q] = bstart[tid * PER + q]; sum += loc[q]; }
-    int incl = sum;
-    const int lane = tid & 63, wave = tid >> 6;
-#pragma unroll
-    for (int off = 1; off < 64; off <<= 1) {
-      const int v = __shfl_up(incl, off, 64);
-      if (lane >= off) incl += v;
-    }
-    if (lane == 63) wsum[wave] = incl;
-    __syncthreads();
-    int woff = 0;
-#pragma unroll
-    for (int q = 0; q < FN_THREADS / 64; ++q) woff += (q < wave) ? wsum[q] : 0;
-    int run = woff + incl - sum;
-#pragma unroll
-    for (int q = 0; q < PER; ++q) { bstart[tid * PER + q] = run; run += loc[q]; }
-    if (tid == FN_THREADS - 1) bstart[FN_BUCKETS] = run;
-  }
-  __syncthreads();
-  for (int j = tid; j < nv; j += FN_THREADS) {
-    const unsigned key = keys[2 * j];
-    const int b = (rbase[key >> 26] + (int)((key >> 13) & 0x1FFF)) >> shift;
-    const int pos = bstart[b] + atomicAdd(&bfill[b], 1);
-    tmp[2 * pos] = key;
-    tmp[2 * pos + 1] = keys[2 * j + 1];
-  }
-  __threadfence();
-  __syncthreads();
-  for (int pos = tid; pos < nv; pos += FN_THREADS) {
-    const unsigned key = tmp[2 * pos];
-    const int b = (rbase[key >> 26] + (int)((key >> 13) & 0x1FFF)) >> shift;
-    int rank = bstart[b];
-    for (int q = bstart[b]; q < bstart[b + 1]; ++q) rank += (tmp[2 * q] < key) ? 1 : 0;
-    if (rank < kp_cap) {
-      const BriskCand& c = C[tmp[2 * pos + 1]];
-      BriskKeyPoint kp;
-      kp.x = c.kx; kp.y = c.ky; kp.size = c.ksize; kp.angle = -1.0f; kp.response = c.kresp;
-      kp.octave = G.single_layer ? 0 : c.layer; kp.class_id = -1;
-      kp_out[(long)frame * kp_cap + rank] = kp;
     }
   }
   if (tid == 0) {
@@ -1598,9 +1592,10 @@
                          const uint8_t* frames, long frame_pitch, int row_pitch, const uint8_t* mask,
                          long mask_frame_pitch, int mask_row_pitch, hipStream_t s, BriskProfiler* prof,
                          const BriskOverlap* ov) {
+  const int probe_stop = env_knob("BRISK_DETECT_PROBE", 0);
+  if (ov && ov->clear_frames > 0) brisk_launch_smap_clear(*ov->clear_G, B, ov->clear_frames, s);
   (void)hipMemsetAsync(B.counters, 0, sizeof(BriskFrameCounters) * (size_t)nframes, s);
   brisk_prof_mark(prof, BRISK_STG_PYRAMID, s);
-  const int probe_stop = env_knob("BRISK_DETECT_PROBE", 0);
   if (probe_stop != 2) launch_pyramid(G, B, nframes, frames, frame_pitch, row_pitch, s);
   static const int fork_at = env_knob("BRISK_INTEGRAL_FORK", 0);
   auto fork_integral = [&]() {
@@ -1610,12 +1605,14 @@
     brisk_launch_integral(G, B.pyr, B.bandsum, ov->Dd->integral, ov->Dd->istride, ov->Dd->iframe_elems, B.band_h, nframes, ov->side,
                           ov->Dd->ibits, B.counters);
     brisk_prof_mark_side(prof, 1, ov->side);
+    if (ov->density_word && fork_at != 1) brisk_launch_batch_density(B.counters, nframes, B.cand_cap, ov->density_word, ov->side);
     (void)hipEventRecord(ov->join, ov->side);
   };
   if (ov && fork_at == 1) fork_integral();
   brisk_prof_mark(prof, BRISK_STG_DETECT, s);
   hipLaunchKernelGGL(k_detect, dim3((T.total_tiles + 7) / 8 * 8, nframes), dim3(256), 0, s, G, T, B.pyr, B.smap, B.cand, B.counters,
                      B.cand_cap);
+  if (ov && ov->density_word && fork_at == 1) brisk_launch_batch_density(B.counters, nframes, B.cand_cap, ov->density_word, s);
   if (probe_stop) return;
   if (ov && fork_at == 2) fork_integral();
   brisk_prof_mark(prof, BRISK_STG_CLASSIFY, s);
@@ -1684,10 +1681,9 @@
                          B.blocks, B.keys, B.cand_cap, B.tie_cap, nframes, lpw, persist, 0, 1);
   }
   brisk_prof_mark(prof, BRISK_STG_FINALIZE, s);
-  hipLaunchKernelGGL(k_finalize, dim3(nframes), dim3(FN_THREADS), 0, s, G, B.cand, B.counters, B.keys, B.kp_out, B.cand_cap,
-                     B.kp_cap, mask, mask_frame_pitch, mask_row_pitch);
-  hipLaunchKernelGGL(k_finalize_large, dim3(nframes), dim3(FN_THREADS), 0, s, G, B.cand, B.counters, B.keys,
-                     reinterpret_cast<unsigned*>(B.tie_idx), (long)BRISK_MAX_LAYERS * B.tie_cap, B.kp_out, B.cand_cap, B.kp_cap);
+  hipLaunchKernelGGL(k_finalize, dim3(nframes), dim3(FN_THREADS), 0, s, G, B.cand, B.counters, B.keys,
+                     reinterpret_cast<unsigned*>(B.tie_idx), (long)BRISK_MAX_LAYERS * B.tie_cap, B.kp_out, B.cand_cap, B.kp_cap, mask,
+                     mask_frame_pitch, mask_row_pitch);
   if (ordered_some) launch_ordered(1);
   brisk_prof_mark(prof, BRISK_STG_POSTFILTER, s);
 }
```

Result: no change. 80760, median of 2 (+0.0%).
